# AlibabaResearch/recom

Hardware: AMD Instinct MI355X
Metric: inference QPS + p50 latency, 1000-col synth model, batch 512, 1×MI355X (higher is better)
Workload: dtype f32

## Files before the change

include/fcp_hip.h:

```cpp
#ifndef FCP_HIP_H_
#define FCP_HIP_H_

#include <stddef.h>
#include <stdint.h>

#ifdef __cplusplus
extern "C" {
#endif

#define FCP_ABI_VERSION 2

enum {
  FCP_OK = 0,
  FCP_ERR_INVALID_ARGUMENT = 1,
  FCP_ERR_SHAPE_MISMATCH = 2,
  FCP_ERR_ALLOC = 3,
  FCP_ERR_HIP = 4,
  FCP_ERR_UNSUPPORTED = 5,
  FCP_ERR_NO_DEVICE = 6
};

enum {
  FCP_FORM_GATHER = 1,
  FCP_FORM_SEGMENT_REDUCE = 2,
// ... 138 lines not shown
                            int64_t *blob_bytes, int32_t *rank_sum);
int fcp_concat_inputs(const fcp_host_tensor_t *inputs, int32_t n_inputs,
                      void *blob, int64_t blob_capacity, int32_t *offsets,
                      int32_t *shapes);

int fcp_plan_create(const fcp_plan_desc_t *desc, fcp_plan_t **plan);

#define FCP_SEG_MAP_MAX 4
typedef struct fcp_column_ext {
  int32_t seg_map_n;
  int32_t seg_map_sym;
  int32_t seg_map_sym_slot;
  int32_t weights_input1;
  int64_t seg_map_mul[FCP_SEG_MAP_MAX];
  int64_t seg_map_div;
  int32_t table_kind1;
  int32_t reserved0;
  int64_t reserved1[1];
} fcp_column_ext_t;
int fcp_plan_create_ex(const fcp_plan_desc_t *desc, const fcp_column_ext_t *ext, fcp_plan_t **plan);
int fcp_plan_create_from_file(const char *path, int32_t device, uint32_t flags,
                              fcp_plan_t **plan);
int fcp_plan_destroy(fcp_plan_t *plan);
int fcp_plan_counts(const fcp_plan_t *plan, int32_t *n_columns, int32_t *n_groups,
                    int32_t *n_host_inputs, int32_t *n_device_inputs,
                    int32_t *n_symbols);
int fcp_plan_output_columns(const fcp_plan_t *plan, int32_t *n, int32_t *indices,
                            int32_t capacity);
int fcp_plan_out_dtype(const fcp_plan_t *plan, int32_t *out);
int fcp_plan_table_dtype(const fcp_plan_t *plan, int32_t *out);
int fcp_plan_table_kinds(const fcp_plan_t *plan, int32_t *kinds, int32_t capacity, int32_t *n);
int fcp_plan_table_bytes(const fcp_plan_t *plan, int64_t *shard_bytes,
                         int64_t *max_table_bytes_unsharded);

int64_t fcp_table_row_bytes(int32_t kind, int32_t dim);
int fcp_table_convert(void *dst, int32_t dst_kind, int64_t dst_row0, const void *src, int32_t src_kind, int64_t rows,
                      int32_t dim, int32_t device, void *stream);
int fcp_table_update_rows(void *table, int32_t kind, int64_t table_rows, int32_t dim, const int64_t *row_ids, const float *rows,
                          int64_t n, int64_t *skipped, int32_t device, void *stream);
int fcp_table_read_rows(float *rows, const void *table, int32_t kind, int64_t table_rows, int32_t dim, const int64_t *row_ids,
                        int64_t n, int32_t device, void *stream);
typedef struct fcp_table_delta_report {
  int64_t n;
  int64_t distinct;
  int64_t duplicates;
  int64_t skipped;
} fcp_table_delta_report_t;
int64_t fcp_table_delta_workspace_bytes(int64_t n);
int fcp_table_delta_distinct(const void *row_ids, int32_t id_bytes, const float *rows, int32_t dim, int64_t n, int64_t table_rows,
                             int64_t *ids_out, float *rows_out, int64_t *pos_out, fcp_table_delta_report_t *report, void *workspace,
                             int32_t device, void *stream);
typedef struct fcp_table_audit_kind {
  int64_t rows_bad;
  int64_t first_bad_row;
  double sum_sq_err;
  float max_abs_err;
  int32_t reserved;
} fcp_table_audit_kind_t;
typedef struct fcp_table_audit {
  int64_t rows, rows_nonfinite, first_nonfinite_row;
  double sum_sq;
  fcp_table_audit_kind_t kind[4];
} fcp_table_audit_t;
int64_t fcp_table_audit_workspace_bytes(void);
int fcp_table_audit(const float *src, int64_t rows, int32_t dim, fcp_table_audit_t *out, void *workspace, int32_t device,
                    void *stream);
int fcp_table_audit_weighted(const float *src, int64_t rows, int32_t dim, const uint32_t *row_counts, fcp_table_audit_t *out,
                             void *workspace, int32_t device, void *stream);
int fcp_table_count_ids(uint32_t *counts, int64_t table_rows, const void *ids, int32_t id_bytes, int64_t n, int64_t *skipped,
                        int32_t device, void *stream);
int fcp_plan_table_rows(const fcp_plan_t *plan, int64_t *rows, int32_t capacity, int32_t *n);
int fcp_plan_traffic_bind(fcp_plan_t *plan, uint32_t *const *counts, int32_t n_counts, int64_t *skipped);
int fcp_plan_traffic_count(fcp_plan_t *plan, const fcp_process_args_t *args);
int fcp_table_formats_choose(const fcp_table_audit_t *audits, const int64_t *rows, const int32_t *dims, int32_t n_tables,
                             int64_t budget_bytes, uint32_t allowed_kinds, const double *table_weight, int32_t *kinds_out,
                             int64_t *bytes_out, double *error_out);
typedef struct fcp_table_digest {
  uint64_t sum;
  int64_t rows;
  int64_t skipped;
  int64_t reserved;
} fcp_table_digest_t;
int64_t fcp_table_digest_workspace_bytes(void);
int fcp_table_digest(const void *first_row, int32_t kind, int64_t rows, int32_t dim, int64_t row0, int64_t row_step,
                     fcp_table_digest_t *out, void *workspace, int32_t device, void *stream);
int fcp_table_digest_rows(const void *table, int32_t kind, int64_t table_rows, int32_t dim, int64_t row0, int64_t row_step,
                          const int64_t *row_ids, int64_t n, fcp_table_digest_t *out, void *workspace, int32_t device, void *stream);
uint64_t fcp_table_digest_host(const void *first_row, int32_t kind, int64_t rows, int32_t dim, int64_t row0, int64_t row_step);
typedef struct fcp_output_error {
  int64_t elems;
  int64_t differ;
  int64_t nonfinite;
  int64_t first_differ_row;
  double sum_sq_ref;
  double sum_sq_err;
  float max_abs_err;
  float max_abs_ref;
  int64_t reserved;
} fcp_output_error_t;
int64_t fcp_outputs_compare_workspace_bytes(int32_t n_columns);
int fcp_outputs_compare(const void *const *ptrs_a, const int64_t *row_strides_a, int32_t out_kind_a, const void *const *ptrs_b,
                        const int64_t *row_strides_b, int32_t out_kind_b,
                        const int32_t *shapes , int32_t n_columns,
                        fcp_output_error_t *out , void *workspace, int32_t device, void *stream);
enum {
  FCP_PLACE_REPLICATE = 0,
  FCP_PLACE_COLUMN_SHARD = 1,
  FCP_PLACE_ROW_SHARD = 2,
  FCP_PLACE_MIXED = 3
};
typedef struct fcp_placement {
  int32_t mode;
  int32_t min_world;
  int64_t bytes_per_gpu;
} fcp_placement_t;
int fcp_placement_decide(const int64_t *table_bytes, int32_t n_tables,
                         int64_t hbm_bytes, int64_t reserve_bytes, int32_t world,
                         int32_t prefer_mode, fcp_placement_t *out);
int fcp_placement_assign(const int64_t *table_bytes, int32_t n_tables,
                         int64_t hbm_bytes, int64_t reserve_bytes, int32_t world,
                         int32_t prefer_mode, int32_t *owner, fcp_placement_t *out);

int fcp_plan_group_width(const fcp_plan_t *plan, int32_t group, int32_t *width);
int fcp_plan_column_offset(const fcp_plan_t *plan, int32_t column,
                           int32_t *offset);
int fcp_plan_arena_bytes(fcp_plan_t *plan, const int32_t *concated_shapes,
                         const int32_t *symbols, int64_t *bytes);
int fcp_plan_read_bad_ids(fcp_plan_t *plan, void *stream, int64_t *count);

enum {
  FCP_LAUNCH_NONE = 0, FCP_LAUNCH_DENSE = 1, FCP_LAUNCH_RAGGED = 2, FCP_LAUNCH_HYBRID = 3,
  FCP_LAUNCH_RAGGED_WEIGHTED = 4,
  FCP_LAUNCH_DENSE_NARROW = 5, FCP_LAUNCH_RAGGED_NARROW = 6, FCP_LAUNCH_HYBRID_NARROW = 7,
  FCP_LAUNCH_DENSE_TAB16 = 8, FCP_LAUNCH_RAGGED_TAB16 = 9, FCP_LAUNCH_HYBRID_TAB16 = 10,
  FCP_LAUNCH_DENSE_TABQ8 = 11, FCP_LAUNCH_RAGGED_TABQ8 = 12, FCP_LAUNCH_HYBRID_TABQ8 = 13,
  FCP_LAUNCH_DENSE_TABMIX = 14, FCP_LAUNCH_RAGGED_TABMIX = 15, FCP_LAUNCH_HYBRID_TABMIX = 16
};
enum { FCP_LAUNCH_STORE_NT = 0, FCP_LAUNCH_STORE_SC1_NT = 1, FCP_LAUNCH_STORE_PLAIN = 4 };
enum { FCP_LAUNCH_SEG_NONE = 0, FCP_LAUNCH_SEG_PREPASS = 1, FCP_LAUNCH_SEG_SEARCH = 2 };
typedef struct fcp_launch_info {
  int32_t kernel;
  int32_t vec;
  int32_t rows_per_wave;
  int32_t store_policy;
  int32_t wide_rows;
  int32_t shard_world;
  int32_t dense_blocks;
  int32_t ragged_blocks;
  int32_t segment_offsets;
} fcp_launch_info_t;
int fcp_plan_last_launch(const fcp_plan_t *plan, fcp_launch_info_t *out);
enum { FCP_DENSE_FRONT_NONE = 0, FCP_DENSE_FRONT_GENERIC = 1, FCP_DENSE_FRONT_PLAIN = 2 };
int fcp_plan_last_dense_front(const fcp_plan_t *plan, int32_t *front);
int fcp_plan_last_csr(const fcp_plan_t *plan, int64_t *csr_arena_off, int32_t *csr_base, int32_t capacity);
enum {
  FCP_AUX_SEGMENT_OFFSETS = 0,
  FCP_AUX_SHARD_FINALIZE_V4 = 1, FCP_AUX_SHARD_FINALIZE_V2 = 2, FCP_AUX_SHARD_FINALIZE_V1 = 3,
  FCP_AUX_CONCAT_V4 = 4, FCP_AUX_CONCAT_V2 = 5, FCP_AUX_CONCAT_V1 = 6,
  FCP_AUX_UPLOAD = 7,
  FCP_AUX_H2D_COPY = 8,
  FCP_AUX_KERNELS = 9
};
int fcp_aux_launch_counts(int64_t *counts, int32_t capacity, int32_t reset);

int fcp_plan_release_captures(fcp_plan_t *plan);
int fcp_process_feature_columns(fcp_plan_t *plan,
                                const fcp_process_args_t *args,
                                fcp_process_result_t *result);

enum { FCP_PRIVATE_NO_CALLER_WAIT = 1u << 0, FCP_PRIVATE_ALWAYS = 1u << 1, FCP_PRIVATE_NO_VERIFY = 1u << 2 };
 int fcp_plan_set_private_streams(fcp_plan_t *plan, int32_t n_streams, uint32_t flags);

 int fcp_plan_probe_private_streams(fcp_plan_t *plan, void *stream, int32_t requests, int32_t spin_us, int32_t grid_blocks,
                                   double *serial_us, double *lanes_us);
 int fcp_plan_private_streams_verdict(fcp_plan_t *plan, void *stream, int32_t *verdict);
 int fcp_plan_verify_private_streams(fcp_plan_t *plan, void *stream, int32_t budget_ms, int32_t *verdict);
typedef struct fcp_private_streams_stats {
  void *supervised_stream;
  int64_t requests;
  int64_t lane_requests;
  int64_t evaluations;
  double stream_order_us_per_mib;
  double last_ratio;
  double worst_ratio;
  double keep_ratio;
  int32_t demoted;
  int32_t evaluation_in_progress;
} fcp_private_streams_stats_t;
 int fcp_plan_private_streams_stats(fcp_plan_t *plan, fcp_private_streams_stats_t *out);

enum { FCP_ORDER_STREAM = 0, FCP_ORDER_INPUTS_READY = 1 };
 int fcp_plan_set_request_order(fcp_plan_t *plan, int32_t order);
 int fcp_result_wait(const void *buffer, void *stream);
 int fcp_result_synchronize(const void *buffer);

int fcp_concat_outputs(const void *const *inputs, const int32_t *dims,
                       int32_t n, int64_t prefix_size, void *out, void *stream);

int fcp_concat_outputs_scatter(const void *const *inputs, const int32_t *dims,
                               const int32_t *col_offsets, int32_t n,
                               int64_t prefix_size, int32_t out_width, void *out,
                               void *stream);
int fcp_concat_outputs_scatter_strided(const void *const *inputs, const int32_t *dims,
                                       const int32_t *in_strides, const int32_t *col_offsets,
                                       int32_t n, int64_t prefix_size, int32_t out_width,
                                       void *out, void *stream);
int fcp_concat_outputs_host(const void *const *host_inputs, const int32_t *dims,
                            const int32_t *col_offsets, int32_t n,
                            int64_t prefix_size, int32_t out_width, void *out,
                            fcp_alloc_fn malloc_temp, void *malloc_temp_ctx,
                            int32_t device, void *stream);

typedef struct fcp_stager fcp_stager_t;
enum { FCP_STAGER_DEFAULT = 0, FCP_STAGER_ZERO_COPY = 1, FCP_STAGER_COPY_KERNEL = 2, FCP_STAGER_COPY_SDMA = 4 };
int fcp_stager_create(int32_t device, int64_t capacity_bytes, int32_t max_inputs,
                      int32_t max_rank_sum, int32_t depth, int32_t n_threads,
                      fcp_stager_t **stager);
int fcp_stager_create_ex(int32_t device, int64_t capacity_bytes, int32_t max_inputs,
                         int32_t max_rank_sum, int32_t depth, int32_t n_threads,
                         uint32_t flags, fcp_stager_t **stager);
int fcp_stager_stage(fcp_stager_t *stager, const fcp_host_tensor_t *inputs,
                     int32_t n_inputs, void *stream, const void **device_blob,
                     int64_t *blob_bytes, const int32_t **offsets,
                     const int32_t **shapes);
int fcp_stager_stage_narrow(fcp_stager_t *stager, const fcp_host_tensor_t *inputs,
                            int32_t n_inputs, const uint8_t *narrow_int64, void *stream,
                            const void **device_blob, int64_t *blob_bytes,
                            const int32_t **offsets, const int32_t **shapes);
enum { FCP_STAGE_COPY = 0, FCP_STAGE_NARROW_I64 = 1, FCP_STAGE_SEG_TO_CSR = 2 };
int fcp_stager_stage_ex(fcp_stager_t *stager, const fcp_host_tensor_t *inputs, int32_t n_inputs,
                        const uint8_t *modes, const int64_t *mode_args, void *stream,
                        const void **device_blob, int64_t *blob_bytes, const int32_t **offsets,
                        const int32_t **shapes);
int fcp_stager_destroy(fcp_stager_t *stager);
typedef struct fcp_stager_stats {
  int64_t calls, copy_calls, copy_calls_over_1ms, fallback_switches, requests_with_blocked_copy;
  double max_copy_call_us;
} fcp_stager_stats_t;
int fcp_stager_stats(fcp_stager_t *stager, fcp_stager_stats_t *out);

int fcp_concat_inputs_ex_sizes(const fcp_host_tensor_t *inputs, int32_t n_inputs,
                               const uint8_t *modes, const int64_t *mode_args,
                               int64_t *blob_bytes, int32_t *rank_sum);
int fcp_concat_inputs_ex(const fcp_host_tensor_t *inputs, int32_t n_inputs,
                         const uint8_t *modes, const int64_t *mode_args, void *blob,
                         int64_t blob_capacity, int32_t *offsets, int32_t *shapes);
typedef struct fcp_pack_pool fcp_pack_pool_t;
int fcp_pack_pool_create(int32_t n_threads, fcp_pack_pool_t **pool);
int fcp_pack_pool_destroy(fcp_pack_pool_t *pool);
int fcp_concat_inputs_ex_pool(fcp_pack_pool_t *pool ,
                              const fcp_host_tensor_t *inputs, int32_t n_inputs,
                              const uint8_t *modes, const int64_t *mode_args,
                              void *blob, int64_t blob_capacity, int32_t *offsets, int32_t *shapes);
int fcp_plan_file_stage_info(const char *path, int32_t *n_inputs, uint8_t *modes,
                             int32_t *rows_symbol, int32_t capacity, int32_t *symbols_input);

enum {
  FCP_GRAPH_HOST_CONCAT_EXTERNAL = 1u << 0,
  FCP_GRAPH_STAGED = 1u << 1,
  FCP_GRAPH_NO_PRUNE = 1u << 2
};
int fcp_graph_build(const void *graphdef, size_t n_bytes, uint32_t flags, const char *plan_path,
                    void **rewritten, size_t *rewritten_bytes, char **description);
void fcp_graph_free(void *p);

#define FCP_COMM_ID_BYTES 128
#define FCP_MAX_GROUPS_ABI 16
typedef struct fcp_comm fcp_comm_t;
int fcp_comm_unique_id(uint8_t *id );
int fcp_comm_create(const uint8_t *id, int32_t rank, int32_t world, int32_t device,
                    fcp_comm_t **comm);
int fcp_comm_destroy(fcp_comm_t *comm);
int fcp_comm_rank(const fcp_comm_t *comm, int32_t *rank, int32_t *world);
int fcp_shard_batch_slice(int64_t rows, int32_t world, int32_t rank, int64_t *begin,
                          int64_t *count);
int fcp_shard_exchange(fcp_comm_t *comm, const void *partial, int64_t rows,
                       int64_t width, void *slices, int64_t *row_begin,
                       int64_t *row_count, void *stream);
int fcp_shard_exchange_columns(fcp_comm_t *comm, const void *block, int64_t rows,
                               const int32_t *widths, void *recv, int64_t *row_begin,
                               int64_t *row_count, void *stream);
typedef struct fcp_shard_step fcp_shard_step_t;
int fcp_shard_step_create(fcp_plan_t *plan, fcp_comm_t *comm, int32_t mode,
                          int32_t group, int64_t max_rows, int64_t max_arena_bytes,
                          const int32_t *col_widths, fcp_shard_step_t **step);
int fcp_shard_step_run(fcp_shard_step_t *step, const fcp_process_args_t *args,
                       void **out, int64_t *row_begin, int64_t *row_count);
int fcp_shard_step_destroy(fcp_shard_step_t *step);

int fcp_shard_finalize(fcp_plan_t *plan, const fcp_process_args_t *args,
                       int32_t group, const void *partial_slices,
                       int32_t world, int64_t row_begin, int64_t row_count,
                       void *out, void *stream);

#ifdef __cplusplus
}
#endif
#endif
```

recom_amd/csrc/fcp_fused_bodies.h:

```cpp
#pragma once
#include <hip/hip_runtime.h>
#include <stdint.h>
#include <stdlib.h>

#include <type_traits>

#include "../../include/fcp_hip.h"
#include <hip/hip_ext.h>
#include "fcp_internal.h"

namespace {

#define FCP_GLOBAL __attribute__((address_space(1)))
template <typename T> __device__ __forceinline__ const FCP_GLOBAL T *as_global(const T *p) {
  return (const FCP_GLOBAL T *)(p);
}
template <typename T> __device__ __forceinline__ FCP_GLOBAL T *as_global(T *p) { return (FCP_GLOBAL T *)(p); }
#define FCP_CONST __attribute__((address_space(4)))
template <typename T> __device__ __forceinline__ const FCP_CONST T *as_const(const T *p) { return (const FCP_CONST T *)(p); }

template <int V> struct VecType;
template <> struct VecType<4> { typedef float __attribute__((ext_vector_type(4))) T; };
template <> struct VecType<2> { typedef float __attribute__((ext_vector_type(2))) T; };
template <> struct VecType<1> { typedef float T; };
// ... 755 lines not shown
    const int64_t below = lo > 0 ? seg_at(seg, is64, stride, lo - 1) : INT64_MIN;
    const int64_t above = hi < n ? seg_at(seg, is64, stride, hi) : INT64_MAX;
    int wa = lo, wz = hi;
    seg_narrow(seg, is64, stride, target, wa, wz);
    if (below < (int64_t)target && above >= (int64_t)target) {
      a = wa;
      z = wz;
    }
  }
  while (z > a) seg_narrow(seg, is64, stride, target, a, z);
  return a;
}

__device__ __forceinline__ void wave_lds_order() {
  __builtin_amdgcn_fence(__ATOMIC_RELEASE, "wavefront");
  __builtin_amdgcn_wave_barrier();
  __builtin_amdgcn_fence(__ATOMIC_ACQUIRE, "wavefront");
}

template <int V> __device__ __forceinline__ VF<V> ld_slot_or_zero(const float *tb, const float *zeros, uint32_t off, uint32_t spr) {
  typedef typename VecType<V>::T T;
  const FCP_GLOBAL T *g = is_row(off) ? as_global(reinterpret_cast<const T *>(tb)) + (uint64_t)off * spr : as_global(reinterpret_cast<const T *>(zeros));
  const T t = *g;
  VF<V> r;
  __builtin_memcpy(&r, &t, sizeof(T));
  return r;
}

template <int V>
__device__ __forceinline__ VF<V> ld_slot_or_zero16(const char *tb, const float *zeros, uint32_t off, uint32_t spr, int tab_kind) {
  typedef typename NarrowType<V>::T T;
  const FCP_GLOBAL T *g = is_row(off) ? as_global(reinterpret_cast<const T *>(tb)) + (uint64_t)off * spr : as_global(reinterpret_cast<const T *>(zeros));
  return widen16<V>(*g, tab_kind);
}

template <int V>
__device__ __forceinline__ Q8Raw ld_slot_or_zero_q8(const char *tb, const float *zeros, int tail, uint32_t off, uint32_t row_bytes) {
  const char *in_table = tb + (uint64_t)off * row_bytes, *in_zeros = reinterpret_cast<const char *>(zeros);
  const char *codes = is_row(off) ? in_table : in_zeros;
  return ld_q8_raw<V>(codes, codes + tail);
}

template <int V, int N, FcpVariant X = FCP_VAR_F32>
__device__ __forceinline__ void bag_walk_batch(const float *tb, const float *zeros, uint32_t spr, const uint32_t *s, int base, int n, VF<V> &acc,
                                               int tab_kind = 0, int q8_tail = 0) {
  constexpr bool TAB16 = X == FCP_VAR_TAB16, TABQ8 = X == FCP_VAR_TABQ8;
  uint32_t off[N];
#pragma unroll
  for (int k = 0; k < N; ++k) off[k] = base + k < n ? s[base + k] : kNoRow;
  if constexpr (TABQ8) {
    Q8Raw raw[N];
#pragma unroll
    for (int k = 0; k < N; ++k) raw[k] = ld_slot_or_zero_q8<V>(reinterpret_cast<const char *>(tb), zeros, q8_tail, off[k], spr);
#pragma unroll
    for (int k = 0; k < N; ++k)
#pragma unroll
      for (int t = 0; t < V; ++t) acc.v[t] = acc.v[t] + dequant_q8(raw[k], t);
    return;
  }
  VF<V> w[N];
#pragma unroll
  for (int k = 0; k < N; ++k) {
    if constexpr (TAB16)
      w[k] = ld_slot_or_zero16<V>(reinterpret_cast<const char *>(tb), zeros, off[k], spr, tab_kind);
    else
      w[k] = ld_slot_or_zero<V>(tb, zeros, off[k], spr);
  }
#pragma unroll
  for (int k = 0; k < N; ++k)
#pragma unroll
    for (int t = 0; t < V; ++t) acc.v[t] = acc.v[t] + w[k].v[t];
}

template <int V, int WALK, FcpVariant X = FCP_VAR_F32>
__device__ __forceinline__ void bag_walk_sum(const float *tb, const float *zeros, uint32_t spr, const uint32_t *s, int n, VF<V> &acc,
                                             int tab_kind = 0, int q8_tail = 0) {
  int base = WALK;
  if (WALK >= 8 && !__any(n > 4)) {
    bag_walk_batch<V, 4, X>(tb, zeros, spr, s, 0, n, acc, tab_kind, q8_tail);
    return;
  } else if (WALK >= 8 && kWalkFirst > WALK && __any(n > WALK)) {
    bag_walk_batch<V, kWalkFirst, X>(tb, zeros, spr, s, 0, n, acc, tab_kind, q8_tail);
    base = kWalkFirst;
  } else {
    bag_walk_batch<V, WALK, X>(tb, zeros, spr, s, 0, n, acc, tab_kind, q8_tail);
  }
  for (; __any(n > base);) {
    if (WALK > 4 && !__any(n > base + 4)) {
      bag_walk_batch<V, 4, X>(tb, zeros, spr, s, base, n, acc, tab_kind, q8_tail);
      base += 4;
    } else {
      bag_walk_batch<V, WALK, X>(tb, zeros, spr, s, base, n, acc, tab_kind, q8_tail);
      base += WALK;
    }
  }
}

__device__ __forceinline__ float weight_den_step(float den, float w, bool squares) {
#pragma clang fp contract(off)
  const float term = squares ? w * w : w;
  return den + term;
}

template <int V>
__device__ __forceinline__ void bag_walk_weighted(const float *tb, const float *zeros, uint32_t spr, const uint32_t *s, int n,
                                                  const float *w, bool want_den, bool squares, VF<V> &acc, float &den) {
#pragma clang fp contract(off)
  constexpr int N = 4;
  const FCP_GLOBAL float *gw = as_global(w);
#pragma unroll 1
  for (int base = 0; base < n; base += N) {
    uint32_t off[N];
    float wt[N];
    VF<V> x[N];
#pragma unroll
    for (int k = 0; k < N; ++k) off[k] = base + k < n ? s[base + k] : kNoRow;
#pragma unroll
    for (int k = 0; k < N; ++k) wt[k] = gw[min(base + k, n - 1)];
#pragma unroll
    for (int k = 0; k < N; ++k) x[k] = ld_slot_or_zero<V>(tb, zeros, off[k], spr);
#pragma unroll
    for (int k = 0; k < N; ++k) {
      const bool counts = off[k] <= kBadRow;
#pragma unroll
      for (int t = 0; t < V; ++t) {
        const float prod = wt[k] * x[k].v[t];
        const float sum = acc.v[t] + prod;
        acc.v[t] = counts ? sum : acc.v[t];
      }
      if (want_den && counts) den = weight_den_step(den, wt[k], squares);
    }
  }
}

__device__ __forceinline__ int wave_inclusive_sum(int x) {
  x += __builtin_amdgcn_update_dpp(0, x, 0x111, 0xf, 0xf, true);
  x += __builtin_amdgcn_update_dpp(0, x, 0x112, 0xf, 0xf, true);
  x += __builtin_amdgcn_update_dpp(0, x, 0x114, 0xf, 0xf, true);
  x += __builtin_amdgcn_update_dpp(0, x, 0x118, 0xf, 0xf, true);
  x += __builtin_amdgcn_update_dpp(0, x, 0x142, 0xa, 0xf, false);
  x += __builtin_amdgcn_update_dpp(0, x, 0x143, 0xc, 0xf, false);
  return x;
}

struct RaggedLds {
  static constexpr int RB = FCP_WAVES_PER_BLOCK;
  static constexpr int CAPW = 384;
  LdsCol col[FCP_WAVE];
  uint32_t ids[RB][CAPW];
  uint8_t owner[RB][CAPW];
  int32_t bound[FCP_WAVE * (FCP_WAVES_PER_BLOCK + 1)];
};

template <int V, bool SHARDED, FcpVariant X = FCP_VAR_F32>
__device__ __forceinline__ void ragged_body(const FcpLaunch &L, int bid, char *smem, const int64_t *wts = nullptr, int kind = 0) {
  constexpr bool WEIGHTED = X == FCP_VAR_WEIGHTED, NARROW = X == FCP_VAR_NARROW, TAB16 = X == FCP_VAR_TAB16, TABQ8 = X == FCP_VAR_TABQ8,
                 TABMIX = X == FCP_VAR_TABMIX;
  const int out_kind = kind, tab_kind = kind;
  constexpr int RB = RaggedLds::RB, CAPW = RaggedLds::CAPW;
  RaggedLds &S = *reinterpret_cast<RaggedLds *>(smem);
  LdsCol *s_col = S.col;

  BlockPos B;
  __builtin_amdgcn_s_setprio(3);
  const Hot H = load_hot(L);
  if (!locate_block<RB>(L, H, bid, B)) return;
  const int tid = threadIdx.x;
  const int lane = tid & (FCP_WAVE - 1);
  const int wave = tid >> 6;
  const int q = B.q0 + lane;
  const uint32_t my_col = B.map[min(q, B.nslots - 1)];
  const int world = H.world, rank = H.rank;

  int pre0 = 0, pre1 = 0;
  const int csr_reg_stride = H.g0.csr_reg_stride;
  if (csr_reg_stride && lane < B.ncols && B.row_blk + wave < B.rows) {
    const FCP_GLOBAL int32_t *cr = as_global(L.csr_reg) + (int64_t)(B.first_col + lane) * csr_reg_stride + (B.row_blk + wave);
    pre0 = cr[0];
    pre1 = cr[1];
  }
  if (tid < B.ncols) stage_col(H, &s_col[tid], H.cols + B.first_col + tid, H.dyn + B.first_col + tid);
  __syncthreads();

  if (H.seg_search) {
    for (int u = tid; u < B.ncols * (RB + 1); u += FCP_BLOCK_THREADS) {
      const LdsCol &c = s_col[u / (RB + 1)];
      const unsigned sk = FCP_F_SEGKIND(c.flags), f = FCP_F_FORM(c.flags);
      int v = 0;
      if ((sk == FCP_SEG_IDS_I32 || sk == FCP_SEG_IDS_I64) && (f == FCP_FORM_SEGMENT_REDUCE || f == FCP_FORM_GATHER_SCATTER))
        v = seg_lower_bound(reinterpret_cast<const char *>(c.csr), sk == FCP_SEG_IDS_I64, c.seg_stride, c.nnz,
                            min(B.row_blk + u % (RB + 1), B.rows), B.rows);
      S.bound[u] = v;
    }
    __syncthreads();
  }
  const int b = B.row_blk + wave;
  if (b >= B.rows) return;

  int lo = 0, cnt = 0;
  if (lane < B.ncols) {
    const unsigned form = FCP_F_FORM(s_col[lane].flags);
    if (form == FCP_FORM_GATHER) {
      lo = b;
      cnt = 1;
    } else if (form == FCP_FORM_SEGMENT_REDUCE || form == FCP_FORM_GATHER_SCATTER) {
      const int nnz = s_col[lane].nnz;
      int o0, o1;
      const unsigned sk = FCP_F_SEGKIND(s_col[lane].flags);
      if (form == FCP_FORM_GATHER_SCATTER && sk != FCP_SEG_CSR_I32) {
        const int t = as_global(s_col[lane].csr)[b];
        o0 = t - 1;
        o1 = t > 0 ? t : -1;
      } else if (H.seg_search && sk != FCP_SEG_CSR_I32) {
        o0 = S.bound[lane * (RB + 1) + wave];
        o1 = S.bound[lane * (RB + 1) + wave + 1];
      } else if (csr_reg_stride) {
        o0 = pre0;
        o1 = pre1;
      } else {
        const FCP_GLOBAL int32_t *csr = as_global(s_col[lane].csr);
        o0 = csr[b];
        o1 = csr[b + 1];
      }
      lo = min(max(o0, 0), nnz);
      const int hi = min(max(o1, lo), nnz);
      cnt = hi - lo;
      if (form == FCP_FORM_GATHER_SCATTER && cnt > 1 && (s_col[lane].xform & 3u) != FCP_XFORM_FILTER) {
        lo = hi - 1;
        cnt = 1;
      }
    }
  }

  const int j = (int)(my_col - B.first_col);
  const bool live = q < B.nslots;
  VF<V> acc = vzero<V>();
  int dropped = 0;

  uint8_t *ow = S.owner[wave];
  uint32_t *wi = S.ids[wave];
  const int want = min(cnt, CAPW);
  const int incl = wave_inclusive_sum(want);
  const int offx = incl - want;
  const int take = max(min(want, CAPW - offx), 0);
  const int limit = min(__shfl(incl, FCP_WAVE - 1), CAPW);
  if (take <= 16)
    for (int i = 0; i < take; ++i) ow[offx + i] = (uint8_t)lane;
  for (unsigned long long big = __ballot(take > 16); big; big &= big - 1) {
    const int p = __ffsll((long long)big) - 1;
    const int po = __shfl(offx, p), pt = __shfl(take, p);
    for (int i = lane; i < pt; i += FCP_WAVE) ow[po + i] = (uint8_t)p;
  }
  wave_lds_order();

  for (int base = 0; base < limit; base += FCP_WAVE) {
    const int k = base + lane;
    const int p = k < limit ? (int)ow[k] : 0;
    const int px = __shfl(offx, p), pl = __shfl(lo, p);
    if (k < limit) {
      bool bad;
      wi[k] = fetch_slot_offset<V, SHARDED>(s_col[p], L.xforms + B.first_col + p, pl + (k - px), nullptr, rank, world, bad);
      if (bad && H.bad_ids && s_col[p].out_off >= B.q0 * V && FCP_F_FORM(s_col[p].flags) != FCP_FORM_GATHER_SCATTER)
        atomicAdd(H.bad_ids, 1ull);
    }
  }
  wave_lds_order();

  __builtin_amdgcn_s_setprio(0);
  const float *wbase = nullptr;
  float den = 0.0f;
  if constexpr (WEIGHTED) {
    if (wts) {
      const int64_t wo = as_global(wts)[B.first_col + j];
      if (wo >= 0) wbase = reinterpret_cast<const float *>(H.blob + wo);
    }
  }
  auto consume = [&](auto walk_width, const uint32_t *s, int n, int wpos) __attribute__((always_inline)) {
    constexpr int WALK = decltype(walk_width)::value;
    const unsigned form = FCP_F_FORM(s_col[j].flags);
    const float *tb = s_col[j].table + (q * V - s_col[j].out_off);
    if constexpr (TAB16)
      tb = reinterpret_cast<const float *>(reinterpret_cast<const char *>(s_col[j].table) + 2 * (int64_t)(q * V - s_col[j].out_off));
    uint32_t spr = (uint32_t)(s_col[j].dim / V);
    int q8_tail = 0;
    if constexpr (TABQ8) {
      const int e = q * V - s_col[j].out_off;
      tb = reinterpret_cast<const float *>(reinterpret_cast<const char *>(s_col[j].table) + e);
      q8_tail = s_col[j].dim - e;
      spr = (uint32_t)s_col[j].dim + 8u;
    }
    int kind = 0;
    if constexpr (TABMIX) {
      kind = (int)FCP_F_TABKIND(s_col[j].flags);
      const int e = q * V - s_col[j].out_off;
      if (kind == FCP_TAB_Q8) {
        tb = reinterpret_cast<const float *>(reinterpret_cast<const char *>(s_col[j].table) + e);
        q8_tail = s_col[j].dim - e;
        spr = (uint32_t)s_col[j].dim + 8u;
      } else if (kind != FCP_TAB_F32) {
        tb = reinterpret_cast<const float *>(reinterpret_cast<const char *>(s_col[j].table) + 2 * (int64_t)e);
      }
    }
    if (form == FCP_FORM_SEGMENT_REDUCE) {
      if ((s_col[j].xform & 3u) == FCP_XFORM_FILTER && (FCP_F_COMBINER(s_col[j].flags) == FCP_COMBINER_MEAN ||
                                                        (WEIGHTED && FCP_F_COMBINER(s_col[j].flags) == FCP_COMBINER_SQRTN))) {
#pragma unroll 1
        for (int k = 0; k < n; ++k) dropped += s[k] == kFiltered;
      }
      if constexpr (WEIGHTED) {
        if (wbase) {
          const unsigned comb = FCP_F_COMBINER(s_col[j].flags);
          bag_walk_weighted<V>(tb, H.zeros, spr, s, n, wbase + wpos, !SHARDED && comb != FCP_COMBINER_SUM, comb == FCP_COMBINER_SQRTN,
                               acc, den);
        } else {
          bag_walk_sum<V, (WALK < kWalkLong ? WALK : kWalkLong)>(tb, H.zeros, spr, s, n, acc);
        }
      } else if constexpr (TABMIX) {
        auto walk = [&](int k) __attribute__((always_inline)) {
          if (k == FCP_TAB_F32)
            bag_walk_sum<V, WALK>(tb, H.zeros, spr, s, n, acc);
          else if (k == FCP_TAB_Q8)
            bag_walk_sum<V, WALK, FCP_VAR_TABQ8>(tb, H.zeros, spr, s, n, acc, 0, q8_tail);
          else
            bag_walk_sum<V, WALK, FCP_VAR_TAB16>(tb, H.zeros, spr, s, n, acc, k);
        };
        const int k0 = __builtin_amdgcn_readfirstlane(kind);
        if (__ballot(kind != k0) == 0ull)
          walk(k0);
        else
          walk(kind);
      } else if constexpr (TABQ8) {
        bag_walk_sum<V, WALK, FCP_VAR_TABQ8>(tb, H.zeros, spr, s, n, acc, 0, q8_tail);
      } else if constexpr (TAB16) {
        bag_walk_sum<V, WALK, FCP_VAR_TAB16>(tb, H.zeros, spr, s, n, acc, tab_kind);
      } else {
        bag_walk_sum<V, WALK>(tb, H.zeros, spr, s, n, acc);
      }
    } else if (form == FCP_FORM_GATHER || form == FCP_FORM_GATHER_SCATTER) {
      int k = n - 1;
      while (k > 0 && s[k] == kFiltered) --k;
      const uint32_t off = s[k];
      if (off != kFiltered) {
        acc = vzero<V>();
        if constexpr (TABMIX) {
          if (is_row(off)) {
            if (kind == FCP_TAB_F32)
              acc = ld_slot<V>(tb, off, spr);
            else if (kind == FCP_TAB_Q8)
              acc = ld_slot_q8<V>(reinterpret_cast<const char *>(tb), q8_tail, off, spr);
            else
              acc = ld_slot16<V>(reinterpret_cast<const char *>(tb), off, spr, kind);
          }
        } else if constexpr (TABQ8) {
          if (is_row(off)) acc = ld_slot_q8<V>(reinterpret_cast<const char *>(tb), q8_tail, off, spr);
        } else if constexpr (TAB16) {
          if (is_row(off)) acc = ld_slot16<V>(reinterpret_cast<const char *>(tb), off, spr, tab_kind);
        } else {
          if (is_row(off)) acc = ld_slot<V>(tb, off, spr);
        }
        if (form == FCP_FORM_GATHER_SCATTER && off == kBadRow && H.bad_ids && q * V == s_col[j].out_off) atomicAdd(H.bad_ids, 1ull);
      }
    }
  };
  {
    const int ptake = __shfl(take, j), poff = __shfl(offx, j);
    int wpos = 0;
    if constexpr (WEIGHTED) wpos = __shfl(lo, j);
    if (live && ptake > 0) consume(std::integral_constant<int, kWalk>(), wi + poff, ptake, wpos);
  }

  for (int done = take;;) {
    const int rem = cnt - done;
    const unsigned long long act = __ballot(rem > 0);
    if (!act) break;
    const int nact = __popcll(act);
    const int sh_log2 = 31 - __clz(CAPW / nact);
    const int share = 1 << sh_log2;
    const int my_rank = __popcll(act & ((1ull << lane) - 1ull));
    const int tk = rem > 0 ? min(rem, share) : 0;
    wave_lds_order();
    if (rem > 0) ow[my_rank] = (uint8_t)lane;
    wave_lds_order();
    const int limit = nact << sh_log2;
    const int from = lo + done;
    for (int base = 0; base < limit; base += FCP_WAVE) {
      const int k = base + lane;
      const int p = k < limit ? (int)ow[k >> sh_log2] : 0;
      const int i = k & (share - 1);
      const int ptk = __shfl(tk, p), pf = __shfl(from, p);
      if (k < limit && i < ptk) {
        bool bad;
        wi[k] = fetch_slot_offset<V, SHARDED>(s_col[p], L.xforms + B.first_col + p, pf + i, nullptr, rank, world, bad);
        if (bad && H.bad_ids && s_col[p].out_off >= B.q0 * V && FCP_F_FORM(s_col[p].flags) != FCP_FORM_GATHER_SCATTER)
          atomicAdd(H.bad_ids, 1ull);
      }
    }
    wave_lds_order();
    const int ptake = __shfl(tk, j), prank = __shfl(my_rank, j);
    int wpos = 0;
    if constexpr (WEIGHTED) wpos = __shfl(from, j);
    if (live && ptake > 0) consume(std::integral_constant<int, kWalkLong>(), wi + (prank << sh_log2), ptake, wpos);
    done += tk;
  }
  const int pcnt = __shfl(cnt, j);
  const LdsCol &C = s_col[j];
  const unsigned form = FCP_F_FORM(C.flags);
  if (!live || form == FCP_FORM_EXTERNAL) return;

  const int dim = C.dim;
  const int e = q * V - C.out_off;
  if (form == FCP_FORM_PASSTHROUGH) {
    if (rank == 0) acc = ld_blob_f32<V>(C.ids + 4 * ((int64_t)b * dim + e));
  } else if (form == FCP_FORM_BATCH_COL_REDUCTION) {
    const int inner = rank == 0 ? C.inner : 0;
    for (int rr = 0; rr < inner; ++rr) {
      const VF<V> x = ld_blob_f32<V>(C.ids + 4 * (((int64_t)b * inner + rr) * dim + e));
#pragma unroll
      for (int t = 0; t < V; ++t) acc.v[t] = acc.v[t] + x.v[t];
    }
  } else if (WEIGHTED && form == FCP_FORM_SEGMENT_REDUCE && !SHARDED && FCP_F_COMBINER(C.flags) != FCP_COMBINER_SUM) {
    float d = wbase ? den : (float)(pcnt - dropped);
    if (FCP_F_COMBINER(C.flags) == FCP_COMBINER_SQRTN) d = sqrtf(d);
    if (d == 0.0f) {
      acc = vzero<V>();
    } else {
#pragma unroll
      for (int t = 0; t < V; ++t) acc.v[t] = acc.v[t] / d;
    }
  } else if (!WEIGHTED && form == FCP_FORM_SEGMENT_REDUCE && !SHARDED && FCP_F_COMBINER(C.flags) == FCP_COMBINER_MEAN && pcnt > dropped) {
    const float fc = (float)(pcnt - dropped);
#pragma unroll
    for (int t = 0; t < V; ++t) acc.v[t] = acc.v[t] / fc;
  }
  if constexpr (NARROW) {
    st_out_narrow<V>(H.arena + C.out_base + 2 * (e + (int64_t)b * C.out_stride), acc, H.store_through, out_kind);
    return;
  }
  st_out<V>(reinterpret_cast<float *>(H.arena + C.out_base) + e + (int64_t)b * C.out_stride, acc, H.store_through);
}

}
```

recom_amd/csrc/fcp_host.h:

```cpp
#pragma once
#include <hip/hip_runtime.h>
#include <hip/hip_ext.h>

#include <algorithm>
#include <atomic>
#include <chrono>
#include <cmath>
#include <cstdio>
#include <cstdlib>
#include <cstring>
#include <functional>
#include <map>
#include <memory>
#include <mutex>
#include <new>
#include <string>
#include <thread>
#include <vector>

#include "../../include/fcp_hip.h"
#include "fcp_internal.h"
#include "fcp_env.h"
#include "fcp_formats.h"
#include "fcp_plan_desc.h"

namespace fcph {

int hip_fail(const char *what, hipError_t e);

#define HIP_TRY(expr)                                   \
  do {                                                  \
    hipError_t e_ = (expr);                             \
    if (e_ != hipSuccess) return hip_fail(#expr, e_);   \
  } while (0)

inline int64_t align128(int64_t x) { return (x + 127) / 128 * 128; }

constexpr int kSlots = 32;
constexpr uint32_t kFlagHostOnly = FCP_FLAG_HOST_ONLY;

struct HostColumn {
  fcp_column_desc_t d;
  fcp_column_ext_t ext = {};
  std::vector<float> boundaries;
  int32_t weights_input = -1;
  std::vector<int64_t> xf_lo, xf_hi;
  int64_t xf_const_off = -1;
  int32_t out_off = 0;
  int64_t const_off = -1;
};

constexpr int kAllSlotsBusy = -2;
constexpr int kNeedsInstall = -3;

struct DynMeta {
  std::vector<int32_t> group_rows;
  std::vector<int64_t> group_base;
  int64_t arena_bytes = 0;
  int64_t csr_arena_off = 0;
  int32_t max_seg_nnz = 0;
  int32_t max_lookup_nnz = 0;
  int64_t seg_pairs = 0;
  bool seg_search = false;
  bool plain = false;
  int64_t work_bytes = 0;
  int32_t csr_reg_mode = 0, csr_reg_stride = 0;
  int64_t csr_reg_base = 0;
  struct Geo {
    int32_t grid_blocks = 0;
    int32_t rows_per_wave = 1;
    FcpGroupLaunch groups[FCP_MAX_GROUPS];
  } geo[2];
};

struct DynSlot {
  bool valid = false;
  std::vector<int32_t> key;
  FcpColDyn *h_dyn = nullptr;
  void *h_dyn_dev = nullptr;
  FcpColDyn *d_dyn = nullptr;
  hipEvent_t uploaded = nullptr;
  uint64_t done_gen = 0;
  hipEvent_t done = nullptr;
  std::vector<std::pair<void *, hipEvent_t>> done_pool;
  bool done_valid = false;
  void *stream = nullptr;
  uint64_t tick = 0;
  int users = 0;
  int uses = 0;
  bool captured = false;
  bool img_built = false;
  bool was_valid = false;
  DynMeta meta;
};

constexpr int kLaneEvents = 8;
constexpr int kMaxPoolLanes = 16;
struct PrivateLane {
  hipStream_t stream = nullptr;
  std::mutex mu;
  hipEvent_t in[kLaneEvents] = {};
  hipEvent_t out[kLaneEvents] = {};
  uint32_t next = 0;
};

extern std::atomic<uint64_t> g_lane_generation;
extern thread_local hipEvent_t tl_lane_done;
extern thread_local uint64_t tl_lane_done_gen;

struct LaneDep {
  hipEvent_t in;
  hipStream_t caller, lane;
};
extern thread_local const LaneDep *tl_lane_dep;
extern thread_local int64_t tl_work_bytes;

constexpr int kSupWindow = 48;
struct LaneSupervisor {
  std::mutex mu;
  bool on = true;
  uint32_t period = 8192, first_gap = 256;
  double keep_ratio = 0.97;
  void *caller = nullptr;
  bool use_lanes = true;
  uint64_t seq = 0;
  uint64_t next_eval = 1, gap = 256;
  int phase = 0;
  hipEvent_t b0 = nullptr, b1 = nullptr;
  hipEvent_t w0 = nullptr, w1 = nullptr;
  PrivateLane *w_lane = nullptr;
  int so_count = 0, w_count = 0;
  int64_t so_bytes = 0, w_bytes = 0;
  int strikes = 0;
  uint64_t evaluations = 0, lane_requests = 0;
  double so_ns_per_byte = 0, last_ratio = 0, worst_ratio = 0;
  bool demoted = false;
};

struct LanePool {
  std::mutex cal_mu;
  std::vector<std::unique_ptr<PrivateLane>> lanes;
  std::vector<hipStream_t> spacers;
  std::atomic<int> n_relying{0};
  std::atomic<uint32_t> rr{0};
  std::atomic<int> fault_us{0};
  std::atomic<hipEvent_t> last_out{nullptr};
};
void sup_reset(LaneSupervisor &S, const fcp::Env &env);
LanePool *lane_pool_for(int device);

struct PendingResult {
  uintptr_t end;
  hipEvent_t done;
  const void *owner;
};
void pending_register(const void *owner, void *arena, int64_t bytes, const void *blob, int64_t blob_bytes, hipEvent_t done);
void pending_clear_range(void *arena, int64_t bytes);
void pending_forget(const void *owner);
int stager_input_wait(const void *base, int64_t bytes, hipStream_t stream);
int stager_input_synchronize(const void *base, int64_t bytes);
int wait_for_inputs(const void *const *inputs, int32_t n, void *stream);

}
using namespace fcph;

struct fcp_plan {
  fcp::Env env;
  fcp_plan_desc_t desc;
  std::vector<HostColumn> cols;
  std::vector<int32_t> ranks, elem_sizes, shape_off;
  std::vector<int32_t> group_width, group_nslots, group_map_off;
  std::vector<int32_t> seg_cols;
  int32_t n_seg_plain = 0;
  bool seg_search = false;
  bool has_inverse = false;
  bool csr_by_pos = false;
  std::vector<int32_t> order, pos_of;
  struct FastCol {
    int32_t ids_input, seg_input, rows_arg, dim, seg_stride;
    int64_t out_off_bytes;
    uint8_t form, rows_source, seg_kind, group;
  };
  std::vector<FastCol> fast_cols;
  std::vector<int32_t> group_rep;
  int vec = 1;
  bool dense_only = true;
  std::vector<uint32_t> span_list;
  std::vector<int32_t> list_off[2], list_n[2];
  uint32_t *d_span_list = nullptr;
  bool host_only = false;
  int32_t rank_sum = 0;

  uint32_t *d_slot_map = nullptr;
  FcpColStatic *d_cols = nullptr;
  FcpXform *d_xforms = nullptr;
  FcpSegMap *d_segmaps = nullptr;
  bool has_seg_map = false;
  bool has_weights = false, weighted_kernel = false;
  FcpVariant variant = FCP_VAR_F32;
  bool plain_dense = false;
  int32_t plain_stride = 0, plain_spans = 0, plain_cols_off = 0;
  std::vector<char> plain_tmpl;
  std::vector<std::pair<uint32_t, int32_t>> plain_entries;
  std::atomic<int32_t> last_dense_front{0};
  bool wide_rows = false;
  int out_kind = FCP_OUT_F32, out_elem = 4;
  int tab_kind = FCP_TAB_F32, tab_elem = 4;
  int tab_row_tail = 0;
  std::vector<int8_t> col_kind;
  bool tab_mixed() const { return !col_kind.empty(); }
  int col_tab_kind(size_t k) const { return col_kind.empty() ? tab_kind : col_kind[k]; }
  int64_t col_row_bytes(size_t k, int dim) const {
    return fcpf::row_bytes(col_tab_kind(k), dim);
  }
  std::vector<FcpColStatic> h_cols;
  char *d_const = nullptr;
  int32_t *d_seg_cols = nullptr;
  unsigned long long *d_bad = nullptr;
  float *d_zeros = nullptr;
  std::vector<const void *> bound_tables;
  bool tables_bound = false;
  FcpTrafficCol *d_traffic = nullptr;
  int32_t traffic_n = 0;
  unsigned long long *traffic_skipped = nullptr;

  bool host_writes_dyn = false;
  std::mutex mu;
  DynSlot slots[kSlots];
  uint64_t tick = 0;

  LanePool *pool = nullptr;
  uint32_t lane_flags = 0;
  std::vector<std::pair<void *, bool>> lane_verdicts;
  std::atomic<void *> lane_good_caller{nullptr};
  int32_t lane_count = 0;
  std::atomic<bool> lane_relies{false};
  std::atomic<int64_t> last_work_bytes{0};
  int64_t lane_min_work = 0;
  int32_t request_order = FCP_ORDER_STREAM;
  std::atomic<uintptr_t> recent_arena[2] = {};
  struct LastLaunch {
    std::atomic<int32_t> kernel{0}, rows_per_wave{0}, store_policy{0}, dense_blocks{0}, ragged_blocks{0}, segment_offsets{0};
    std::atomic<int64_t> csr_arena_off{-1};
    std::unique_ptr<std::atomic<int32_t>[]> csr_base;
  } last_launch;
  std::atomic<bool> lane_demoted{false};
  LaneSupervisor sup;
  std::atomic<bool> sup_window{false};
};

namespace fcph {

struct DeviceGuard {
  int prev = -1;
  bool changed = false;
  int enter(int dev) {
    hipError_t e = hipGetDevice(&prev);
    if (e != hipSuccess) return hip_fail("hipGetDevice", e);
    if (prev != dev) {
      e = hipSetDevice(dev);
      if (e != hipSuccess) return hip_fail("hipSetDevice", e);
      changed = true;
    }
    return FCP_OK;
  }
  ~DeviceGuard() {
    if (changed) (void)hipSetDevice(prev);
  }
};

template <class F> int on_device(const char *who, int32_t device, void *stream, F enqueue) {
  DeviceGuard guard;
  const int rc = guard.enter(device);
  if (rc) return rc;
  enqueue(static_cast<hipStream_t>(stream));
  const hipError_t e = hipGetLastError();
  return e == hipSuccess ? FCP_OK : hip_fail((std::string(who) + ": kernel launch").c_str(), e);
}

int compute_dyn(const fcp_plan *p, const int32_t *offsets, const int32_t *shapes, const int32_t *symbols, int64_t blob_bytes,
                FcpColDyn *dyn, DynMeta *m);
int compute_weights(const fcp_plan *p, const int32_t *offsets, const int32_t *shapes, int64_t *wts);
inline size_t slot_dyn_bytes(const fcp_plan *p) {
  return p->cols.size() * sizeof(FcpColDyn) + (p->has_weights ? p->cols.size() * sizeof(int64_t) : 0) +
         (p->plain_dense ? p->plain_tmpl.size() : 0);
}
inline size_t slot_image_off(const fcp_plan *p) { return p->cols.size() * sizeof(FcpColDyn); }
inline const int64_t *slot_weights(const fcp_plan *p, const FcpColDyn *dyn) {
  return p->has_weights ? reinterpret_cast<const int64_t *>(dyn + p->cols.size()) : nullptr;
}
void build_plain_template(fcp_plan *p);
bool stream_is_capturing(hipStream_t stream);
int bind_tables(fcp_plan *p, const void *const *input_ptrs, bool capturing);
void build_key(const fcp_plan *p, const fcp_process_args_t *a, std::vector<int32_t> &key);
int find_or_reserve(fcp_plan *p, const std::vector<int32_t> &key, DynSlot **out, bool *install, bool capturing);
int install_slot(fcp_plan *p, const fcp_process_args_t *a, DynSlot &s);
void publish_slot(fcp_plan *p, DynSlot &s, const std::vector<int32_t> &key, void *stream);
void fill_launch(const fcp_plan *p, const DynSlot &s, int kind, const void *blob, void *arena, int store_policy, FcpLaunch *L);
void destroy_lanes(LanePool *pool);
int create_lanes(LanePool *pool, int n, int prio);
int process_on_private_streams(fcp_plan_t *p, const fcp_process_args_t *a, fcp_process_result_t *r);

struct SlotUnpin {
  fcp_plan *p;
  DynSlot *s;
  bool recorded;
  ~SlotUnpin() {
    std::lock_guard<std::mutex> lock(p->mu);
    if (recorded) s->done_valid = s->uses == 1;
    --s->users;
  }
};

}

extern "C" int fcp_internal_process(fcp_plan_t *p, const fcp_process_args_t *a, fcp_process_result_t *r);
```

recom_amd/csrc/fcp_internal.h:

```cpp
#pragma once
#include <stddef.h>
#include <stdint.h>

#ifndef FCP_MAX_GROUPS
#define FCP_MAX_GROUPS 16
#endif
#define FCP_BLOCK_THREADS 256
#define FCP_WAVES_PER_BLOCK 4
#define FCP_WAVE 64

#define FCP_F_FORM(f) ((f) & 0xFu)
#define FCP_F_COMBINER(f) (((f) >> 4) & 0xFu)
#define FCP_F_IDSRC(f) (((f) >> 8) & 0xFu)
#define FCP_F_SEGKIND(f) (((f) >> 12) & 0xFu)
#define FCP_F_TABKIND(f) (((f) >> 16) & 0x3u)
#define FCP_F_PACK(form, comb, idsrc, segkind) \
  ((uint32_t)(form) | ((uint32_t)(comb) << 4) | ((uint32_t)(idsrc) << 8) | ((uint32_t)(segkind) << 12))

struct FcpColStatic {
  const float *table;
  const float *boundaries;
  int64_t vocab;
  int32_t dim;
  int32_t out_off;
  uint32_t flags;
  int32_t n_boundaries;
  int32_t seg_stride;
  float bnd_b0, bnd_inv, bnd_step;
  uint32_t xform;
  int32_t bnd_off;
};

struct FcpXform {
  int64_t lo0, hi0;
  int64_t sub;
  const int64_t *extra;
  int64_t hash_buckets;
  int64_t pad_;
};
#define FCP_XFORM_HASH_BIT 0x80000000u

struct FcpColDyn {
  int64_t ids_off;
  int64_t seg_off;
  int64_t out_base;
  int32_t out_stride;
  int32_t nnz;
  int32_t csr_base;
  int32_t inner;
  int32_t rows;
  int32_t seg_sym;
};

struct FcpSegMap {
  int64_t mul[4];
  int64_t div;
  int32_t n;
  int32_t sym_slot;
};

struct FcpGroupLaunch {
  int32_t rows;
  int32_t nslots;
  int32_t nsp8;
  int32_t block_begin;
  int32_t slot_map_off;
  int32_t span_list_off;
  int32_t nlist;
  int32_t csr_reg_stride;
};

struct FcpLaunch {
  const uint32_t *slot_map;
  const uint32_t *span_list;
  const FcpColStatic *cols;
  const FcpColDyn *dyn;
  const char *blob;
  char *arena;
  unsigned long long *bad_ids;
  int64_t csr_arena_off;
  int32_t n_groups;
  int32_t rows_per_wave;
  int32_t shard_rank, shard_world;
  int32_t seg_search;
  int32_t store_through;
  const int32_t *csr_reg;
  FcpGroupLaunch groups[FCP_MAX_GROUPS];
  const FcpXform *xforms;
  const float *zeros;
};

struct FcpPlainCol {
  const float *table;
  int64_t ids_off;
  uint32_t vocab;
  uint32_t spr;
  int32_t out_off;
  uint32_t kind;
  int32_t n_boundaries;
  float bnd_b0, bnd_inv, bnd_step;
};
constexpr uint32_t FCP_PLAIN_FACT_NONE = 0, FCP_PLAIN_FACT_I32 = 1, FCP_PLAIN_FACT_I64 = 2, FCP_PLAIN_FACT_F32 = 3;
constexpr int FCP_PLAIN_FACTS_OFF = 80;
constexpr int FCP_PLAIN_FACTS_PER_PASS = 16;
constexpr int fcp_plain_facts_bytes(int max_cols) {
  return (max_cols + FCP_PLAIN_FACTS_PER_PASS - 1) / FCP_PLAIN_FACTS_PER_PASS * FCP_PLAIN_FACTS_PER_PASS * 4;
}
struct FcpPlainSpan {
  int32_t ncols;
  int32_t cols_off;
  int32_t pad_[2];
  uint8_t lane_col[FCP_WAVE];
};
struct FcpPlainLaunch {
  const char *img;
  const char *blob;
  float *out;
  unsigned long long *bad_ids;
  int32_t rows, nslots, nsp8, nlist;
  int32_t img_stride;
  int32_t out_stride;
  int32_t store_policy;
};

struct FcpSegLaunch {
  const int32_t *seg_cols;
  const FcpColStatic *cols;
  const FcpColDyn *dyn;
  const char *blob;
  char *arena;
  int64_t csr_arena_off;
  unsigned long long *bad_ids;
  const FcpXform *xforms;
  const FcpSegMap *segmaps;
  int32_t skip_inverse;
};

struct FcpTrafficCol {
  uint32_t *counts;
  int32_t pos;
  int32_t pad_;
};
struct FcpTrafficLaunch {
  const FcpTrafficCol *list;
  const FcpColStatic *cols;
  const FcpColDyn *dyn;
  const FcpXform *xforms;
  const char *blob;
  unsigned long long *skipped;
};
struct ihipStream_t;
int fcp_launch_plan_traffic(const FcpTrafficLaunch &T, int n_list, int max_nnz, ihipStream_t *s);

enum FcpVariant {
  FCP_VAR_F32 = 0,
  FCP_VAR_WEIGHTED,
  FCP_VAR_NARROW,
  FCP_VAR_TAB16,
  FCP_VAR_TABQ8,
  FCP_VAR_TABMIX,
  FCP_VARIANTS
};

struct ihipStream_t;
void fcp_set_stop_event(void *event);
bool fcp_stop_event_pending();
void fcp_set_any_order(bool on);
struct FcpFusedWork {
  const FcpLaunch *dense;
  int dense_blocks;
  const FcpLaunch *ragged;
  int ragged_blocks;
  int vec;
  int kind;
  const int64_t *wts;
};
typedef int FcpFusedLauncher(const FcpFusedWork &W, ihipStream_t *s);
FcpFusedLauncher fcp_launch_f32, fcp_launch_weighted, fcp_launch_narrow, fcp_launch_tab16, fcp_launch_tabq8, fcp_launch_tabmix;
int fcp_launch_dense_plain(const FcpPlainLaunch &P, int grid_blocks, ihipStream_t *s);
void fcp_take_launch_extras(void **stop_event, int *flags);
int fcp_launch_upload(const void *host_mapped_src, void *dst, size_t bytes, ihipStream_t *s);
int fcp_launch_h2d_copy(const void *host_mapped_src, void *dst, size_t bytes, ihipStream_t *s);
int fcp_launch_segment_offsets(const FcpSegLaunch &L, int n_seg_cols, int max_nnz, ihipStream_t *s, bool any_order = false);
int fcp_launch_concat_outputs(const void *const *inputs, const int32_t *dims, const int32_t *col_offsets, const int32_t *in_strides,
                              int32_t n, int64_t prefix, int32_t width, int32_t first_off, void *out,
                              ihipStream_t *s);
int fcp_launch_shard_finalize(const FcpLaunch &L, int group, const float *partials, int world,
                              int64_t row_begin, int64_t row_count, float *out, int vec,
                              ihipStream_t *s, const int64_t *wts = nullptr);
```

recom_amd/csrc/fcp_plan.hip:

```cpp
#include "fcp_host.h"

namespace fcph {

int hip_fail(const char *what, hipError_t e) {
  return fail((e == hipErrorNoDevice || e == hipErrorInvalidDevice || e == hipErrorNoBinaryForGpu || e == hipErrorInsufficientDriver)
                  ? FCP_ERR_NO_DEVICE
                  : FCP_ERR_HIP,
              std::string(what) + ": " + hipGetErrorString(e));
}

int finish_geometry(const fcp_plan *p, DynMeta *m);
void find_regular_csr(const fcp_plan *p, const FcpColDyn *dyn, DynMeta *m);

int compute_dyn_slow(const fcp_plan *p, const int32_t *offsets, const int32_t *shapes,
                     const int32_t *symbols, int64_t blob_bytes, FcpColDyn *dyn, DynMeta *m) {
  const int nc = (int)p->cols.size();
  const int ng = p->desc.n_groups;
  const int nh = (int)p->ranks.size();
  thread_local std::vector<int64_t> numel_v, col_rows;
  numel_v.resize(nh);
  col_rows.resize(nc);
  for (int i = 0; i < nh; ++i) {
    int64_t n = 1;
    const int32_t *d = shapes + p->shape_off[i];
// ... 283 lines not shown
  m->csr_arena_off = cursor;
  int64_t csr_cursor = 0;
  if (p->csr_by_pos) {
    const int64_t stride = ((int64_t)m->group_rows[0] + 1 + 31) / 32 * 32;
    for (int k : p->seg_cols) dyn[p->pos_of[k]].csr_base = (int32_t)(p->pos_of[k] * stride);
    csr_cursor = stride * nc;
    if (csr_cursor > 0x7fffffff) return -1;
  } else {
    for (int k : p->seg_cols) {
      FcpColDyn &d = dyn[p->pos_of[k]];
      d.csr_base = (int32_t)csr_cursor;
      csr_cursor += ((int64_t)d.rows + 1 + 31) / 32 * 32;
      if (csr_cursor > 0x7fffffff) return -1;
    }
  }
  m->arena_bytes = cursor + csr_cursor * 4;
  find_regular_csr(p, dyn, m);
  return finish_geometry(p, m);
}

int compute_weights(const fcp_plan *p, const int32_t *offsets, const int32_t *shapes, int64_t *wts) {
  auto numel = [&](int i) {
    int64_t n = 1;
    for (int j = 0; j < p->ranks[i]; ++j) n *= shapes[p->shape_off[i] + j];
    return n;
  };
  for (size_t pos = 0; pos < p->cols.size(); ++pos) {
    const HostColumn &hc = p->cols[p->order[pos]];
    wts[pos] = -1;
    if (hc.weights_input < 0) continue;
    if (numel(hc.weights_input) != numel(hc.d.ids_input))
      return fail(FCP_ERR_SHAPE_MISMATCH, "column " + std::to_string(p->order[pos]) + ": the weights tensor does not hold one weight per id");
    if (offsets[hc.weights_input] % 4) return fail(FCP_ERR_UNSUPPORTED, "blob tensor not 4-byte aligned");
    wts[pos] = offsets[hc.weights_input];
  }
  return FCP_OK;
}

int compute_dyn(const fcp_plan *p, const int32_t *offsets, const int32_t *shapes, const int32_t *symbols,
                int64_t blob_bytes, FcpColDyn *dyn, DynMeta *m) {
  const bool slow_only = fcp::diag_on("dyn_general");
  if (!slow_only && !p->fast_cols.empty()) {
    const int rc = compute_dyn_fast(p, offsets, shapes, symbols, blob_bytes, dyn, m);
    if (rc >= 0) return rc;
  }
  const int rc = compute_dyn_slow(p, offsets, shapes, symbols, blob_bytes, dyn, m);
  if (rc == FCP_OK) {
    int64_t gathered = 0;
    for (size_t i = 0; i < p->cols.size(); ++i) gathered += (int64_t)dyn[i].nnz * p->cols[p->order[i]].d.dim;
    m->work_bytes = gathered * 4 + m->csr_arena_off;
  }
  return rc;
}

void uniform_boundaries(const std::vector<float> &b, float *b0, float *inv, float *step_out) {
  const int n = (int)b.size();
  if (n < 2 || !(b[n - 1] > b[0])) return;
  const float lo = b[0];
  const float scale = (float)((double)(n - 1) / ((double)b[n - 1] - (double)b[0]));
  if (!(scale > 0.0f) || !std::isfinite(scale)) return;
  auto guess = [&](float x) {
    float t = (x - lo) * scale;
    t = std::fmin(std::fmax(t, -1.0f), (float)n);
    int g = (int)std::floor(t) + 1;
    return std::min(std::max(g, 0), n);
  };
  auto exact = [&](float x) { return (int)(std::upper_bound(b.begin(), b.end(), x) - b.begin()); };
  int misses = 0;
  for (int i = 0; i < n; ++i) {
    if (i && !(b[i] > b[i - 1])) return;
    const float below = std::nextafter(b[i], -INFINITY);
    misses += guess(b[i]) != exact(b[i]);
    misses += guess(below) != exact(below);
  }
  if (misses * 8 > n) return;
  *b0 = lo;
  *inv = scale;
  const float step = b[1] - b[0];
  if (!(step > 0.0f) || !std::isfinite(step)) return;
  for (int i = 0; i < n; ++i)
    if (std::fmaf((float)i, step, lo) != b[i]) return;
  *step_out = step;
}

void build_plain_template(fcp_plan *p) {
  p->plain_dense = false;
  if (fcp::diag_ll("dense_generic", 0) != 0) return;
  const fcp_plan_desc_t &d = p->desc;
  if (p->out_elem != 4 || p->tab_elem != 4 || d.layout != FCP_LAYOUT_CONCAT || d.n_groups != 1 || d.shard_world > 1 || p->vec != 4 || p->wide_rows ||
      p->weighted_kernel || !p->dense_only || p->cols.empty())
    return;
  const int nc = (int)p->cols.size();
  for (int pos = 0; pos < nc; ++pos) {
    const HostColumn &hc = p->cols[p->order[pos]];
    const FcpColStatic &s = p->h_cols[pos];
    if (hc.d.form != FCP_FORM_GATHER || s.xform != 0 || hc.d.vocab < 0 || hc.d.vocab >= 0xFFFFFFFDLL) return;
    if (hc.d.id_source == FCP_IDS_F32_BUCKETIZE) {
      if (s.bnd_step == 0.0f) return;
    } else if (hc.d.id_source != FCP_IDS_I32 && hc.d.id_source != FCP_IDS_I64) {
      return;
    }
  }
  const int nslots = p->group_nslots[0];
  const int nspans = (nslots + FCP_WAVE - 1) / FCP_WAVE;
  if (p->list_n[0][0] != nspans) return;
  std::vector<int> first(nspans, nc), last(nspans, -1);
  for (int pos = 0; pos < nc; ++pos) {
    const FcpColStatic &s = p->h_cols[pos];
    const int s0 = s.out_off / 4 / FCP_WAVE, s1 = (s.out_off + s.dim - 1) / 4 / FCP_WAVE;
    for (int sp = s0; sp <= s1; ++sp) {
      first[sp] = std::min(first[sp], pos);
      last[sp] = std::max(last[sp], pos);
    }
  }
  int max_cols = 1;
  for (int sp = 0; sp < nspans; ++sp) max_cols = std::max(max_cols, last[sp] - first[sp] + 1);
  if (max_cols > FCP_WAVE) return;
  p->plain_cols_off = FCP_PLAIN_FACTS_OFF + fcp_plain_facts_bytes(max_cols);
  p->plain_stride = (int32_t)(p->plain_cols_off + (size_t)max_cols * sizeof(FcpPlainCol));
  p->plain_spans = nspans;
  p->plain_tmpl.assign((size_t)nspans * p->plain_stride, 0);
  p->plain_entries.clear();
  for (int sp = 0; sp < nspans; ++sp) {
    char *rec = p->plain_tmpl.data() + (size_t)sp * p->plain_stride;
    FcpPlainSpan head;
    std::memset(&head, 0, sizeof(head));
    head.ncols = last[sp] - first[sp] + 1;
    head.cols_off = p->plain_cols_off;
    for (int pos = first[sp]; pos <= last[sp]; ++pos) {
      const FcpColStatic &s = p->h_cols[pos];
      FcpPlainCol c;
      std::memset(&c, 0, sizeof(c));
      c.table = nullptr;
      c.ids_off = 0;
      c.vocab = (uint32_t)s.vocab;
      c.spr = (uint32_t)(s.dim / 4);
      c.out_off = s.out_off;
      c.kind = FCP_F_IDSRC(s.flags);
      c.n_boundaries = s.n_boundaries;
      c.bnd_b0 = s.bnd_b0;
      c.bnd_inv = s.bnd_inv;
      c.bnd_step = s.bnd_step;
      const size_t at = (size_t)sp * p->plain_stride + p->plain_cols_off + (size_t)(pos - first[sp]) * sizeof(FcpPlainCol);
      std::memcpy(p->plain_tmpl.data() + at, &c, sizeof(c));
      p->plain_entries.emplace_back((uint32_t)at, pos);
      for (int q = std::max(s.out_off / 4, sp * FCP_WAVE); q < std::min((s.out_off + s.dim) / 4, (sp + 1) * FCP_WAVE); ++q)
        head.lane_col[q - sp * FCP_WAVE] = (uint8_t)(pos - first[sp]);
    }
    std::memcpy(rec, &head, sizeof(head));
  }
  p->plain_dense = true;
}

void destroy_device(fcp_plan *p) {
  if (p->host_only) return;
  for (auto &s : p->slots) {
    if (s.h_dyn) (void)hipHostFree(s.h_dyn);
    if (s.d_dyn) (void)hipFree(s.d_dyn);
    if (s.uploaded) (void)hipEventDestroy(s.uploaded);
    for (auto &e : s.done_pool) (void)hipEventDestroy(e.second);
  }
  if (p->d_slot_map) (void)hipFree(p->d_slot_map);
  if (p->d_span_list) (void)hipFree(p->d_span_list);
  if (p->d_cols) (void)hipFree(p->d_cols);
  if (p->d_xforms) (void)hipFree(p->d_xforms);
  if (p->d_segmaps) (void)hipFree(p->d_segmaps);
  if (p->d_const) (void)hipFree(p->d_const);
  if (p->d_seg_cols) (void)hipFree(p->d_seg_cols);
  if (p->d_bad) (void)hipFree(p->d_bad);
  if (p->d_zeros) (void)hipFree(p->d_zeros);
  if (p->d_traffic) (void)hipFree(p->d_traffic);
}

int init_device(fcp_plan *p) {
  DeviceGuard guard;
  int rc = guard.enter(p->desc.device);
  if (rc) return rc;
  const int nc = (int)p->cols.size();
  std::vector<uint32_t> map;
  for (int g = 0; g < p->desc.n_groups; ++g) {
    p->group_map_off[g] = (int32_t)map.size();
    for (int pos = 0; pos < nc; ++pos) {
      const HostColumn &hc = p->cols[p->order[pos]];
      if (hc.d.concat_group != g) continue;
      for (int s = 0; s < hc.d.dim / p->vec; ++s) map.push_back((uint32_t)pos);
    }
  }
  HIP_TRY(hipMalloc(&p->d_span_list, std::max<size_t>(p->span_list.size(), 1) * sizeof(uint32_t)));
  HIP_TRY(hipMemcpy(p->d_span_list, p->span_list.data(), p->span_list.size() * sizeof(uint32_t), hipMemcpyHostToDevice));
  HIP_TRY(hipMalloc(&p->d_slot_map, std::max<size_t>(map.size(), 1) * sizeof(uint32_t)));
  HIP_TRY(hipMemcpy(p->d_slot_map, map.data(), map.size() * sizeof(uint32_t), hipMemcpyHostToDevice));
  int64_t const_bytes = 0;
  std::vector<int> owners;
  for (size_t k = 0; k < p->cols.size(); ++k) {
    HostColumn &hc = p->cols[k];
    if (hc.boundaries.empty()) continue;
    for (int o : owners)
      if (p->cols[o].boundaries == hc.boundaries) {
        hc.const_off = p->cols[o].const_off;
        break;
      }
    if (hc.const_off < 0) {
      hc.const_off = const_bytes;
      const_bytes += align128((int64_t)hc.boundaries.size() * 4);
      owners.push_back((int)k);
    }
  }
  for (HostColumn &hc : p->cols) {
    if (hc.xf_lo.size() <= 1) continue;
    hc.xf_const_off = const_bytes;
    const_bytes += align128((int64_t)(hc.xf_lo.size() - 1) * 16);
  }
  if (const_bytes) {
    HIP_TRY(hipMalloc(&p->d_const, const_bytes));
    for (const HostColumn &hc : p->cols) {
      if (hc.xf_const_off < 0) continue;
      std::vector<int64_t> pairs;
      for (size_t i = 1; i < hc.xf_lo.size(); ++i) {
        pairs.push_back(hc.xf_lo[i]);
        pairs.push_back(hc.xf_hi[i]);
      }
      HIP_TRY(hipMemcpy(p->d_const + hc.xf_const_off, pairs.data(), pairs.size() * 8, hipMemcpyHostToDevice));
    }
    for (int o : owners)
      HIP_TRY(hipMemcpy(p->d_const + p->cols[o].const_off, p->cols[o].boundaries.data(),
                        p->cols[o].boundaries.size() * 4, hipMemcpyHostToDevice));
  }
  std::vector<FcpXform> h_xforms;
  p->h_cols.resize(nc);
  for (int pos = 0; pos < nc; ++pos) {
    const HostColumn &hc = p->cols[p->order[pos]];
    FcpColStatic &s = p->h_cols[pos];
    s.table = nullptr;
    s.boundaries = hc.const_off >= 0 ? reinterpret_cast<const float *>(p->d_const + hc.const_off) : nullptr;
    s.vocab = hc.d.vocab;
    s.dim = hc.d.dim;
    s.out_off = hc.out_off;
    s.flags = FCP_F_PACK(hc.d.form, hc.d.combiner, hc.d.id_source, hc.d.seg_kind);
    if (p->tab_mixed()) s.flags |= (uint32_t)p->col_kind[p->order[pos]] << 16;
    s.n_boundaries = (int32_t)hc.boundaries.size();
    s.seg_stride = hc.d.seg_stride < 1 ? 1 : hc.d.seg_stride;
    s.bnd_b0 = 0.0f;
    s.bnd_inv = 0.0f;
    s.bnd_step = 0.0f;
    uniform_boundaries(hc.boundaries, &s.bnd_b0, &s.bnd_inv, &s.bnd_step);
    s.bnd_off = -1;
    s.xform = 0;
    if (hc.d.xform_mode != FCP_XFORM_NONE || hc.d.hash_buckets > 0) {
      if (h_xforms.empty()) {
        FcpXform none;
        none.lo0 = 1;
        none.hi0 = 0;
        none.sub = 0;
        none.extra = nullptr;
        none.hash_buckets = 0;
        none.pad_ = 0;
        h_xforms.assign(nc, none);
      }
      FcpXform &x = h_xforms[pos];
      if (hc.d.hash_buckets > 0) {
        s.xform |= FCP_XFORM_HASH_BIT;
        x.hash_buckets = hc.d.hash_buckets;
      }
      if (hc.d.xform_mode != FCP_XFORM_NONE) {
        const uint32_t n = (uint32_t)std::max<size_t>(hc.xf_lo.size(), 1);
        s.xform |= (n << 2) | (uint32_t)hc.d.xform_mode;
        x.sub = hc.d.xform_substitute;
        if (!hc.xf_lo.empty()) {
          x.lo0 = hc.xf_lo[0];
          x.hi0 = hc.xf_hi[0];
        }
        if (hc.xf_const_off >= 0) x.extra = reinterpret_cast<const int64_t *>(p->d_const + hc.xf_const_off);
      }
    }
  }
  build_plain_template(p);
  HIP_TRY(hipMalloc(&p->d_cols, nc * sizeof(FcpColStatic)));
  HIP_TRY(hipMemcpy(p->d_cols, p->h_cols.data(), nc * sizeof(FcpColStatic), hipMemcpyHostToDevice));
  if (!h_xforms.empty()) {
    HIP_TRY(hipMalloc(&p->d_xforms, nc * sizeof(FcpXform)));
    HIP_TRY(hipMemcpy(p->d_xforms, h_xforms.data(), nc * sizeof(FcpXform), hipMemcpyHostToDevice));
  }
  if (p->has_seg_map) {
    std::vector<FcpSegMap> h_maps(nc);
    for (int pos = 0; pos < nc; ++pos) {
      const fcp_column_ext_t &e = p->cols[p->order[pos]].ext;
      FcpSegMap &sm = h_maps[pos];
      for (int i = 0; i < 4; ++i) sm.mul[i] = i < e.seg_map_n ? e.seg_map_mul[i] : 0;
      sm.div = e.seg_map_n > 0 ? e.seg_map_div : 1;
      sm.n = e.seg_map_n;
      sm.sym_slot = e.seg_map_n > 0 && e.seg_map_sym >= 0 ? e.seg_map_sym_slot : -1;
    }
    HIP_TRY(hipMalloc(&p->d_segmaps, nc * sizeof(FcpSegMap)));
    HIP_TRY(hipMemcpy(p->d_segmaps, h_maps.data(), nc * sizeof(FcpSegMap), hipMemcpyHostToDevice));
  }
  if (!p->seg_cols.empty()) {
    std::vector<int32_t> seg_pos;
    for (int k : p->seg_cols) seg_pos.push_back(p->pos_of[k]);
    HIP_TRY(hipMalloc(&p->d_seg_cols, seg_pos.size() * sizeof(int32_t)));
    HIP_TRY(hipMemcpy(p->d_seg_cols, seg_pos.data(), seg_pos.size() * sizeof(int32_t), hipMemcpyHostToDevice));
  }
  size_t zero_bytes = 256;
  for (size_t k = 0; k < p->cols.size(); ++k)
    if (fcpf::kTab[p->col_tab_kind(k)].row_tail) zero_bytes = std::max(zero_bytes, (size_t)((p->col_row_bytes(k, p->cols[k].d.dim) + 255) / 256 * 256));
  HIP_TRY(hipMalloc(&p->d_zeros, zero_bytes));
  HIP_TRY(hipMemset(p->d_zeros, 0, zero_bytes));
  if (p->desc.flags & FCP_FLAG_COUNT_BAD_IDS) {
    HIP_TRY(hipMalloc(&p->d_bad, sizeof(unsigned long long)));
    HIP_TRY(hipMemset(p->d_bad, 0, sizeof(unsigned long long)));
  }
  {
    int large_bar = 0;
    (void)hipDeviceGetAttribute(&large_bar, hipDeviceAttributeIsLargeBar, p->desc.device);
    p->host_writes_dyn = large_bar != 0 && !p->env.dyn_upload_kernel;
  }
  for (auto &s : p->slots) {
    const size_t dyn_bytes = (slot_dyn_bytes(p) + 15) / 16 * 16;
    HIP_TRY(hipHostMalloc(reinterpret_cast<void **>(&s.h_dyn), dyn_bytes, hipHostMallocMapped));
    HIP_TRY(hipHostGetDevicePointer(&s.h_dyn_dev, s.h_dyn, 0));
    if (p->host_writes_dyn) {
      if (hipExtMallocWithFlags(reinterpret_cast<void **>(&s.d_dyn), dyn_bytes, hipDeviceMallocFinegrained) != hipSuccess) {
        (void)hipGetLastError();
        p->host_writes_dyn = false;
        for (auto &t : p->slots)
          if (t.d_dyn) {
            (void)hipFree(t.d_dyn);
            t.d_dyn = nullptr;
          }
      }
    }
  }
  for (auto &s : p->slots) {
    const size_t dyn_bytes = (slot_dyn_bytes(p) + 15) / 16 * 16;
    if (!s.d_dyn) HIP_TRY(hipMalloc(&s.d_dyn, dyn_bytes));
    HIP_TRY(hipEventCreateWithFlags(&s.uploaded, hipEventDisableTiming));
    s.done = nullptr;
  }
  p->bound_tables.assign(p->desc.n_device_inputs, nullptr);
  {
    int64_t shard_bytes = 0;
    (void)fcp_plan_table_bytes(p, &shard_bytes, nullptr);
    size_t free_b = 0, total_b = 0;
    if (hipMemGetInfo(&free_b, &total_b) == hipSuccess && total_b > 0 && (uint64_t)shard_bytes > total_b)
      return fail(FCP_ERR_UNSUPPORTED, "this plan's tables need " + std::to_string(shard_bytes) + " bytes on a device with " +
                                           std::to_string(total_b) + ": shard them over more GPUs (fcp_placement_decide)");
  }
  return FCP_OK;
}

}

extern "C" {

int fcp_plan_create(const fcp_plan_desc_t *desc, fcp_plan_t **out) { return fcp_plan_create_ex(desc, nullptr, out); }

int fcp_plan_create_ex(const fcp_plan_desc_t *desc, const fcp_column_ext_t *ext, fcp_plan_t **out) {
  if (!out) return fail(FCP_ERR_INVALID_ARGUMENT, "null plan out pointer");
  *out = nullptr;
  PlanFacts facts;
  int rc = check_desc(desc, ext, &facts);
  if (rc) return rc;
  fcp_plan_desc_t canonical = *desc;
  canonical.flags = facts.flags;
  desc = &canonical;
  fcp_plan *p = new (std::nothrow) fcp_plan();
  if (!p) return fail(FCP_ERR_ALLOC, "out of host memory");
  p->out_kind = facts.out_kind;
  p->out_elem = fcpf::kOut[facts.out_kind].elem;
  p->tab_kind = facts.tab_kind;
  p->col_kind.swap(facts.col_kind);
  p->tab_elem = p->tab_mixed() ? 0 : fcpf::kTab[facts.tab_kind].elem;
  p->tab_row_tail = p->tab_mixed() ? 0 : fcpf::kTab[facts.tab_kind].row_tail;
  p->variant = facts.variant;
  p->weighted_kernel = facts.variant == FCP_VAR_WEIGHTED;
  p->env = fcp::read_env();
  p->desc = *desc;
  p->desc.columns = nullptr;
  p->desc.host_input_ranks = nullptr;
  p->desc.host_input_elem_sizes = nullptr;
  p->host_only = (desc->flags & kFlagHostOnly) != 0;
  p->ranks.assign(desc->host_input_ranks, desc->host_input_ranks + desc->n_host_inputs);
  p->elem_sizes.assign(desc->host_input_elem_sizes, desc->host_input_elem_sizes + desc->n_host_inputs);
  p->shape_off.resize(desc->n_host_inputs);
  int32_t acc = 0;
  for (int i = 0; i < desc->n_host_inputs; ++i) {
    p->shape_off[i] = acc;
    acc += p->ranks[i];
  }
  p->rank_sum = acc;
  p->cols.resize(desc->n_columns);
  int gcd4 = 4;
  for (int k = 0; k < desc->n_columns; ++k) {
    HostColumn &hc = p->cols[k];
    hc.d = desc->columns[k];
    if (hc.d.id_source == FCP_IDS_F32_BUCKETIZE && hc.d.boundaries && hc.d.n_boundaries > 0 &&
        hc.d.form != FCP_FORM_PASSTHROUGH && hc.d.form != FCP_FORM_BATCH_COL_REDUCTION && hc.d.form != FCP_FORM_EXTERNAL)
      hc.boundaries.assign(hc.d.boundaries, hc.d.boundaries + hc.d.n_boundaries);
    hc.d.boundaries = nullptr;
    if (hc.d.xform_mode != FCP_XFORM_NONE && hc.d.xform_n > 0) {
      hc.xf_lo.assign(hc.d.xform_lo, hc.d.xform_lo + hc.d.xform_n);
      hc.xf_hi.assign(hc.d.xform_hi, hc.d.xform_hi + hc.d.xform_n);
    }
    hc.d.xform_lo = hc.d.xform_hi = nullptr;
    if (ext && ext[k].seg_map_n > 0) {
      hc.ext = ext[k];
      p->has_seg_map = true;
    }
    if (ext && ext[k].weights_input1 > 0) {
      hc.weights_input = ext[k].weights_input1 - 1;
      p->has_weights = true;
    }
    if (hc.d.dim % 4) gcd4 = (hc.d.dim % 2) ? 1 : std::min(gcd4, 2);
    const int f = hc.d.form;
    if ((f == FCP_FORM_SEGMENT_REDUCE || f == FCP_FORM_GATHER_SCATTER) && hc.d.seg_kind != FCP_SEG_CSR_I32)
      p->seg_cols.push_back(k);
  }
  p->vec = gcd4;
  std::stable_partition(p->seg_cols.begin(), p->seg_cols.end(), [&](int32_t k) { return p->cols[k].d.form != FCP_FORM_GATHER_SCATTER; });
  p->n_seg_plain = 0;
  for (int32_t k : p->seg_cols) p->n_seg_plain += p->cols[k].d.form != FCP_FORM_GATHER_SCATTER;
  p->last_launch.csr_base.reset(new std::atomic<int32_t>[p->cols.size() > 0 ? p->cols.size() : 1]);
  for (size_t k = 0; k < p->cols.size(); ++k) p->last_launch.csr_base[k].store(-1, std::memory_order_relaxed);
  p->seg_search = desc->shard_world <= 1 && !p->env.seg_prepass;
  if (p->has_seg_map) p->seg_search = false;
  for (const HostColumn &hc : p->cols) {
    if (hc.d.seg_kind != FCP_SEG_NONE && hc.d.seg_stride > 0xffff) p->seg_search = false;
    if (hc.d.form == FCP_FORM_GATHER_SCATTER && hc.d.seg_kind != FCP_SEG_CSR_I32) {
      p->has_inverse = true;
      p->seg_search = false;
// ... 137 lines not shown
  *out = p->tab_kind;
  return FCP_OK;
}

int fcp_plan_table_kinds(const fcp_plan_t *p, int32_t *kinds, int32_t capacity, int32_t *n) {
  if (!p) return fail(FCP_ERR_INVALID_ARGUMENT, "null plan");
  std::vector<int32_t> in_kind(p->desc.n_device_inputs, -1);
  for (size_t k = 0; k < p->cols.size(); ++k) {
    const int f = p->cols[k].d.form;
    if (f == FCP_FORM_GATHER || f == FCP_FORM_SEGMENT_REDUCE || f == FCP_FORM_GATHER_SCATTER) in_kind[p->cols[k].d.table_input] = p->col_tab_kind(k);
  }
  for (int32_t t = 0; t < p->desc.n_device_inputs && t < capacity; ++t)
    if (kinds) kinds[t] = in_kind[t];
  if (n) *n = p->desc.n_device_inputs;
  return FCP_OK;
}

int fcp_plan_table_rows(const fcp_plan_t *p, int64_t *rows, int32_t capacity, int32_t *n) {
  if (!p) return fail(FCP_ERR_INVALID_ARGUMENT, "null plan");
  std::vector<int64_t> in_rows(p->desc.n_device_inputs, -1);
  for (size_t k = 0; k < p->cols.size(); ++k) {
    const int f = p->cols[k].d.form;
    if (f != FCP_FORM_GATHER && f != FCP_FORM_SEGMENT_REDUCE && f != FCP_FORM_GATHER_SCATTER) continue;
    int64_t &r = in_rows[p->cols[k].d.table_input];
    r = std::max(r, p->cols[k].d.vocab);
  }
  for (int32_t t = 0; t < p->desc.n_device_inputs && t < capacity; ++t)
    if (rows) rows[t] = in_rows[t];
  if (n) *n = p->desc.n_device_inputs;
  return FCP_OK;
}

int fcp_plan_table_bytes(const fcp_plan_t *p, int64_t *shard_bytes, int64_t *max_table_bytes_unsharded) {
  if (!p) return fail(FCP_ERR_INVALID_ARGUMENT, "null plan");
  std::vector<int64_t> local(p->desc.n_device_inputs, 0), whole(p->desc.n_device_inputs, 0);
  for (size_t k = 0; k < p->cols.size(); ++k) {
    const HostColumn &hc = p->cols[k];
    const int f = hc.d.form;
    if (f != FCP_FORM_GATHER && f != FCP_FORM_SEGMENT_REDUCE && f != FCP_FORM_GATHER_SCATTER) continue;
    const int64_t local_vocab =
        (hc.d.vocab - p->desc.shard_rank + p->desc.shard_world - 1) / p->desc.shard_world;
    const int64_t row_bytes = p->col_row_bytes(k, hc.d.dim);
    local[hc.d.table_input] = std::max(local[hc.d.table_input], local_vocab * row_bytes);
    whole[hc.d.table_input] = std::max(whole[hc.d.table_input], hc.d.vocab * row_bytes);
  }
  int64_t sum = 0, mx = 0;
  for (int t = 0; t < p->desc.n_device_inputs; ++t) {
    sum += local[t];
    mx = std::max(mx, whole[t]);
  }
  if (shard_bytes) *shard_bytes = sum;
  if (max_table_bytes_unsharded) *max_table_bytes_unsharded = mx;
  return FCP_OK;
}

int fcp_plan_release_captures(fcp_plan_t *p) {
  if (!p) return fail(FCP_ERR_INVALID_ARGUMENT, "null plan");
  std::lock_guard<std::mutex> lock(p->mu);
  for (auto &s : p->slots) {
    if (!s.captured) continue;
    s.captured = false;
    s.done_valid = false;
  }
  return FCP_OK;
}

int fcp_plan_destroy(fcp_plan_t *p) {
  if (!p) return FCP_OK;
  if (!p->host_only) {
    DeviceGuard guard;
    if (guard.enter(p->desc.device) == FCP_OK) {
      (void)hipDeviceSynchronize();
      pending_forget(p);
      if (p->pool && p->lane_relies.exchange(false)) p->pool->n_relying.fetch_sub(1, std::memory_order_acq_rel);
      for (hipEvent_t *ev : {&p->sup.b0, &p->sup.b1, &p->sup.w0, &p->sup.w1})
        if (*ev) {
          (void)hipEventDestroy(*ev);
          *ev = nullptr;
        }
      destroy_device(p);
    }
  }
  delete p;
  return FCP_OK;
}

int fcp_plan_group_width(const fcp_plan_t *p, int32_t group, int32_t *width) {
  if (!p || !width || group < 0 || group >= p->desc.n_groups)
    return fail(FCP_ERR_INVALID_ARGUMENT, "bad group");
  *width = p->group_width[group];
  return FCP_OK;
}

int fcp_plan_column_offset(const fcp_plan_t *p, int32_t column, int32_t *offset) {
  if (!p || !offset || column < 0 || column >= (int32_t)p->cols.size())
    return fail(FCP_ERR_INVALID_ARGUMENT, "bad column");
  *offset = p->cols[column].out_off;
  return FCP_OK;
}

int fcp_plan_arena_bytes(fcp_plan_t *p, const int32_t *concated_shapes, const int32_t *symbols,
                         int64_t *bytes) {
  if (!p || !concated_shapes || !bytes) return fail(FCP_ERR_INVALID_ARGUMENT, "null argument");
  std::vector<FcpColDyn> dyn(p->cols.size());
  std::vector<int32_t> offsets(p->ranks.size(), 0);
  DynMeta m;
  int rc = compute_dyn(p, offsets.data(), concated_shapes, symbols, -1, dyn.data(), &m);
  if (rc) return rc;
  *bytes = m.arena_bytes;
  return FCP_OK;
}

int fcp_plan_read_bad_ids(fcp_plan_t *p, void *stream, int64_t *count) {
  if (!p || !count) return fail(FCP_ERR_INVALID_ARGUMENT, "null argument");
  *count = 0;
  if (p->host_only) return fail(FCP_ERR_NO_DEVICE, "host-only plan");
  if (!p->d_bad) return FCP_OK;
  DeviceGuard guard;
  int rc = guard.enter(p->desc.device);
  if (rc) return rc;
  unsigned long long v = 0;
  HIP_TRY(hipStreamSynchronize(static_cast<hipStream_t>(stream)));
  if (p->pool && p->lane_count > 0) {
    std::lock_guard<std::mutex> cal_lock(p->pool->cal_mu);
    for (auto &l : p->pool->lanes)
      if (l->stream) HIP_TRY(hipStreamSynchronize(l->stream));
  }
  HIP_TRY(hipMemcpy(&v, p->d_bad, sizeof(v), hipMemcpyDeviceToHost));
  *count = (int64_t)v;
  return FCP_OK;
}

int fcp_plan_last_launch(const fcp_plan_t *p, fcp_launch_info_t *out) {
  if (!p || !out) return fail(FCP_ERR_INVALID_ARGUMENT, "null argument");
  const fcp_plan::LastLaunch &ll = p->last_launch;
  out->kernel = ll.kernel.load(std::memory_order_relaxed);
  out->vec = p->vec;
  out->rows_per_wave = ll.rows_per_wave.load(std::memory_order_relaxed);
  out->store_policy = ll.store_policy.load(std::memory_order_relaxed);
  out->wide_rows = p->wide_rows ? 1 : 0;
  out->shard_world = p->desc.shard_world > 1 ? p->desc.shard_world : 1;
  out->dense_blocks = ll.dense_blocks.load(std::memory_order_relaxed);
  out->ragged_blocks = ll.ragged_blocks.load(std::memory_order_relaxed);
  out->segment_offsets = ll.segment_offsets.load(std::memory_order_relaxed);
  return FCP_OK;
}

int fcp_plan_last_dense_front(const fcp_plan_t *p, int32_t *front) {
  if (!p || !front) return fail(FCP_ERR_INVALID_ARGUMENT, "null argument");
  *front = p->last_dense_front.load(std::memory_order_relaxed);
  return FCP_OK;
}

int fcp_plan_last_csr(const fcp_plan_t *p, int64_t *csr_arena_off, int32_t *csr_base, int32_t capacity) {
  if (!p || capacity < 0 || (capacity > 0 && !csr_base)) return fail(FCP_ERR_INVALID_ARGUMENT, "null plan / bad capacity");
  const fcp_plan::LastLaunch &ll = p->last_launch;
  if (csr_arena_off) *csr_arena_off = ll.csr_arena_off.load(std::memory_order_relaxed);
  for (int32_t k = 0; k < capacity && k < (int32_t)p->cols.size(); ++k)
    csr_base[k] = ll.csr_base ? ll.csr_base[k].load(std::memory_order_relaxed) : -1;
  return FCP_OK;
}

}
```

recom_amd/csrc/fcp_plan_desc.cc:

```cpp
#include "fcp_plan_desc.h"

#include <algorithm>
#include <cmath>
#include <cstdio>
#include <cstring>
#include <utility>

namespace fcph {
namespace {
thread_local std::string g_last_error;
}

int fail(int code, const std::string &msg) {
  g_last_error = msg;
  return code;
}

namespace {

int validate_desc(const fcp_plan_desc_t *d) {
  if (!d) return fail(FCP_ERR_INVALID_ARGUMENT, "null plan descriptor");
  if (d->abi_version != FCP_ABI_VERSION) return fail(FCP_ERR_INVALID_ARGUMENT, "abi_version mismatch");
  if (d->n_columns <= 0 || !d->columns) return fail(FCP_ERR_INVALID_ARGUMENT, "plan has no columns");
  if (d->n_host_inputs < 0 || (d->n_host_inputs > 0 && (!d->host_input_ranks || !d->host_input_elem_sizes)))
// ... 263 lines not shown
    fcp_column_desc_t &c = P.cols[k];
    std::memset(&c, 0, sizeof(c));
    long long vocab = 0;
    if (std::fscanf(f, "%d %d %d %d %lld %d %d %d %d %d %d %d %d %d %d", &c.form, &c.combiner, &c.dim, &c.id_source, &vocab,
                    &c.table_input, &c.ids_input, &c.seg_input, &c.seg_kind, &c.seg_stride, &c.rows_source, &c.rows_arg,
                    &c.concat_group, &c.concat_slot, &c.n_boundaries) != 15 ||
        c.n_boundaries < 0 || c.n_boundaries > (1 << 24))
      return fail(FCP_ERR_INVALID_ARGUMENT, where + "truncated or malformed column " + std::to_string(k));
    c.vocab = vocab;
    P.bnd[k].resize(c.n_boundaries);
    for (int b = 0; b < c.n_boundaries; ++b)
      if (std::fscanf(f, "%f", &P.bnd[k][b]) != 1) return fail(FCP_ERR_INVALID_ARGUMENT, where + "truncated boundary list");
    c.boundaries = c.n_boundaries ? P.bnd[k].data() : nullptr;
    if (version >= 2) {
      long long sub = 0, hb = 0;
      if (std::fscanf(f, "%d %d %lld %lld", &c.xform_mode, &c.xform_n, &sub, &hb) != 4 || c.xform_n < 0 || c.xform_n > (1 << 20))
        return fail(FCP_ERR_INVALID_ARGUMENT, where + "truncated or malformed id transform of column " + std::to_string(k));
      c.xform_substitute = sub;
      c.hash_buckets = hb;
      P.xlo[k].resize(c.xform_n);
      P.xhi[k].resize(c.xform_n);
      for (int i = 0; i < c.xform_n; ++i) {
        long long lo = 0, hi = 0;
        if (std::fscanf(f, "%lld %lld", &lo, &hi) != 2) return fail(FCP_ERR_INVALID_ARGUMENT, where + "truncated interval list");
        P.xlo[k][i] = lo;
        P.xhi[k][i] = hi;
      }
      c.xform_lo = c.xform_n ? P.xlo[k].data() : nullptr;
      c.xform_hi = c.xform_n ? P.xhi[k].data() : nullptr;
    }
  }
  bool seen_maps = false, seen_weights = false;
  for (;;) {
    int count = 0;
    const int got = std::fscanf(f, "%31s %d", tag, &count);
    if (got == EOF || got == 0) break;
    if (got != 2) return fail(FCP_ERR_INVALID_ARGUMENT, where + "malformed trailing section");
    if (version >= 5 && !std::strcmp(tag, "weights") && !seen_weights && !seen_maps && !P.has_stage) {
      if (count < 0 || count > n_cols) return fail(FCP_ERR_INVALID_ARGUMENT, where + "bad 'weights M'");
      seen_weights = true;
      if (count > 0) P.ext.assign(n_cols, fcp_column_ext_t{});
      for (int i = 0; i < count; ++i) {
        int col = -1, input = -1;
        if (std::fscanf(f, "%d %d", &col, &input) != 2 || col < 0 || col >= n_cols || input < 0 || input >= n_host ||
            P.ext[col].weights_input1 != 0)
          return fail(FCP_ERR_INVALID_ARGUMENT, where + "malformed weights entry " + std::to_string(i));
        P.ext[col].weights_input1 = input + 1;
      }
    } else if (version >= 4 && !std::strcmp(tag, "segmaps") && !seen_maps && !P.has_stage) {
      if (count < 0 || count > n_cols) return fail(FCP_ERR_INVALID_ARGUMENT, where + "bad 'segmaps M'");
      seen_maps = true;
      if (P.ext.empty()) P.ext.assign(n_cols, fcp_column_ext_t{});
      for (int i = 0; i < count; ++i) {
        int col = -1, n = 0, sym = -1, slot = 0;
        long long mul[4] = {0, 0, 0, 0}, div = 1;
        if (std::fscanf(f, "%d %d %d %d %lld %lld %lld %lld %lld", &col, &n, &sym, &slot, &mul[0], &mul[1], &mul[2], &mul[3], &div) != 9 ||
            col < 0 || col >= n_cols || n < 1 || n > FCP_SEG_MAP_MAX || P.ext[col].seg_map_n != 0)
          return fail(FCP_ERR_INVALID_ARGUMENT, where + "malformed segmaps entry " + std::to_string(i));
        fcp_column_ext_t &e = P.ext[col];
        e.seg_map_n = n;
        e.seg_map_sym = sym;
        e.seg_map_sym_slot = slot;
        for (int j = 0; j < 4; ++j) e.seg_map_mul[j] = mul[j];
        e.seg_map_div = div;
      }
    } else if (version >= 3 && !std::strcmp(tag, "stage") && !P.has_stage) {
      const int n_stage = count;
      int sym_in = -1;
      if (std::fscanf(f, "%31s %d", t2, &sym_in) != 2 || std::strcmp(t2, "symbols_input") || n_stage < 0 || n_stage > (1 << 24) ||
          sym_in < -1 || sym_in >= n_stage)
        return fail(FCP_ERR_INVALID_ARGUMENT, where + "expected 'stage N symbols_input K'");
      P.stage_modes.resize(n_stage);
      P.stage_rows_symbol.resize(n_stage);
      for (int i = 0; i < n_stage; ++i) {
        int mode = 0, sym = -1;
        if (std::fscanf(f, "%d %d", &mode, &sym) != 2 || mode < FCP_STAGE_COPY || mode > FCP_STAGE_SEG_TO_CSR || sym < -1 ||
            sym >= d.n_symbols || (mode == FCP_STAGE_SEG_TO_CSR && (sym < 0 || sym_in < 0)))
          return fail(FCP_ERR_INVALID_ARGUMENT, where + "malformed stage entry " + std::to_string(i));
        P.stage_modes[i] = (uint8_t)mode;
        P.stage_rows_symbol[i] = sym;
      }
      P.stage_symbols_input = sym_in;
      P.has_stage = true;
    } else {
      return fail(FCP_ERR_INVALID_ARGUMENT, where + "unexpected section '" + tag + "'");
    }
  }
  if (version >= 8) {
    if (P.ext.empty()) P.ext.assign(n_cols, fcp_column_ext_t{});
    std::vector<char> read(P.in_kinds.size(), 0);
    int first = -1;
    bool differ = false;
    for (int k = 0; k < n_cols; ++k) {
      const fcp_column_desc_t &c = P.cols[k];
      if (c.form != FCP_FORM_GATHER && c.form != FCP_FORM_SEGMENT_REDUCE && c.form != FCP_FORM_GATHER_SCATTER) continue;
      if (c.table_input < 0 || c.table_input >= (int)P.in_kinds.size() || P.in_kinds[c.table_input] < 0)
        return fail(FCP_ERR_INVALID_ARGUMENT, where + "column " + std::to_string(k) + " reads a table the table_dtypes line gives no dtype");
      read[c.table_input] = 1;
      const int kind = P.in_kinds[c.table_input];
      P.ext[k].table_kind1 = 1 + kind;
      differ = differ || (first >= 0 && kind != first);
      if (first < 0) first = kind;
    }
    for (size_t t = 0; t < read.size(); ++t)
      if (!read[t] && P.in_kinds[t] >= 0)
        return fail(FCP_ERR_INVALID_ARGUMENT, where + "the table_dtypes line gives device input " + std::to_string(t) + ", which no lookup column reads, a dtype");
    if (!differ) return fail(FCP_ERR_INVALID_ARGUMENT, where + "version 8 is for plans whose tables have more than one dtype; this one is a version <= 7 plan");
  }
  d.abi_version = FCP_ABI_VERSION;
  d.n_columns = n_cols;
  d.columns = P.cols.data();
  d.n_host_inputs = n_host;
  d.host_input_ranks = P.ranks.data();
  d.host_input_elem_sizes = P.esz.data();
  d.shard_rank = 0;
  d.shard_world = 1;
  return FCP_OK;
}

}

int check_desc(const fcp_plan_desc_t *desc, const fcp_column_ext_t *ext, PlanFacts *facts) {
  int rc = validate_desc(desc);
  if (rc) return rc;
  if (ext && (rc = validate_ext(desc, ext))) return rc;
  fcp_plan_desc_t d = *desc;
  facts->col_kind.clear();
  if (d.flags & FCP_FLAG_TABLES_PER_INPUT) {
    int uniform = -1;
    if ((rc = resolve_table_kinds(desc, ext, &facts->col_kind, &uniform))) return rc;
    d.flags &= ~(uint32_t)FCP_FLAG_TABLES_PER_INPUT;
    if (uniform >= 0) {
      facts->col_kind.clear();
      d.flags |= fcpf::kTab[uniform].flag;
    }
  }
  const bool mixed = !facts->col_kind.empty();
  const unsigned families = ((d.flags & fcpf::kOutFlags) ? NARROW : 0) | (mixed ? MIXED : 0) | ((d.flags & FCP_FLAG_TABLES_Q8) ? Q8 : 0) | ((d.flags & kTab16Flags) ? TAB16 : 0);
  if ((rc = run_refusals(d, ext, families))) return rc;
  facts->flags = d.flags;
  facts->out_kind = fcpf::out_kind_of_flags(d.flags);
  facts->tab_kind = mixed ? FCP_TAB_MIXED : fcpf::tab_kind_of_flags(d.flags);
  bool weighted = false;
  for (int k = 0; k < d.n_columns; ++k) weighted = weighted || (ext && ext[k].weights_input1 > 0) || d.columns[k].combiner == FCP_COMBINER_SQRTN;
  facts->variant = weighted                           ? FCP_VAR_WEIGHTED
                   : facts->out_kind != FCP_OUT_F32   ? FCP_VAR_NARROW
                   : mixed                            ? FCP_VAR_TABMIX
                   : facts->tab_kind == FCP_TAB_Q8    ? FCP_VAR_TABQ8
                   : facts->tab_kind != FCP_TAB_F32   ? FCP_VAR_TAB16
                                                      : FCP_VAR_F32;
  return FCP_OK;
}

}

using namespace fcph;

int fcp_internal_fail(int code, const std::string &msg) { return fail(code, msg); }

extern "C" {

int fcp_abi_version(void) { return FCP_ABI_VERSION; }

const char *fcp_status_string(int status) {
  switch (status) {
  case FCP_OK: return "ok";
  case FCP_ERR_INVALID_ARGUMENT: return "invalid argument";
  case FCP_ERR_SHAPE_MISMATCH: return "run-time shapes do not match the plan";
  case FCP_ERR_ALLOC: return "allocator callback failed";
  case FCP_ERR_HIP: return "HIP runtime error";
  case FCP_ERR_UNSUPPORTED: return "unsupported";
  case FCP_ERR_NO_DEVICE: return "no usable gfx950 device";
  default: return "unknown status";
  }
}

const char *fcp_last_error(void) { return g_last_error.c_str(); }

int fcp_plan_create_from_file(const char *path, int32_t device, uint32_t flags, fcp_plan_t **out) {
  if (!path || !out) return fail(FCP_ERR_INVALID_ARGUMENT, "null argument");
  *out = nullptr;
  ParsedPlanFile P;
  const int rc = parse_plan_file(path, P);
  if (rc) return rc;
  const std::string where = std::string("column plan ") + path + ": ";
  if (P.has_stage && (int32_t)P.stage_modes.size() != P.d.n_host_inputs)
    return fail(FCP_ERR_INVALID_ARGUMENT, where + "the stage section lists " + std::to_string(P.stage_modes.size()) + " inputs, the plan has " +
                                              std::to_string(P.d.n_host_inputs) + " host inputs");
  P.d.device = device;
  if (P.out_kind != FCP_OUT_F32 && (flags & fcpf::kOutFlags & ~fcpf::kOut[P.out_kind].flag))
    return fail(FCP_ERR_INVALID_ARGUMENT, where + "flags ask for another output dtype than the file's out_dtype line");
  if (P.tab_kind != FCP_TAB_F32 && (flags & fcpf::kTabFlags & ~fcpf::kTab[P.tab_kind].flag))
    return fail(FCP_ERR_INVALID_ARGUMENT, where + "flags ask for another table dtype than the file's table_dtype line");
  if (!P.in_kinds.empty() && (flags & fcpf::kTabFlags))
    return fail(FCP_ERR_INVALID_ARGUMENT, where + "plan-wide table dtype flags with a file that carries a table_dtypes line");
  P.d.flags = flags | fcpf::kOut[P.out_kind].flag | fcpf::kTab[P.tab_kind].flag | (P.in_kinds.empty() ? 0u : FCP_FLAG_TABLES_PER_INPUT);
  return fcp_plan_create_ex(&P.d, P.ext.empty() ? nullptr : P.ext.data(), out);
}

int fcp_plan_file_stage_info(const char *path, int32_t *n_inputs, uint8_t *modes, int32_t *rows_symbol, int32_t capacity,
                             int32_t *symbols_input) {
  if (!path) return fail(FCP_ERR_INVALID_ARGUMENT, "null argument");
  ParsedPlanFile P;
  const int rc = parse_plan_file(path, P);
  if (rc) return rc;
  const int32_t n = P.has_stage ? (int32_t)P.stage_modes.size() : 0;
  if (n_inputs) *n_inputs = n;
  if (symbols_input) *symbols_input = P.has_stage ? P.stage_symbols_input : -1;
  for (int32_t i = 0; i < n && i < capacity; ++i) {
    if (modes) modes[i] = P.stage_modes[i];
    if (rows_symbol) rows_symbol[i] = P.stage_rows_symbol[i];
  }
  return FCP_OK;
}

int fcp_placement_assign(const int64_t *table_bytes, int32_t n_tables, int64_t hbm_bytes, int64_t reserve_bytes, int32_t world,
                         int32_t prefer_mode, int32_t *owner, fcp_placement_t *out) {
  if (!out || n_tables < 0 || (n_tables > 0 && !table_bytes) || hbm_bytes <= 0 || reserve_bytes < 0 || world < 1)
    return fail(FCP_ERR_INVALID_ARGUMENT, "bad placement arguments");
  if (prefer_mode != FCP_PLACE_COLUMN_SHARD && prefer_mode != FCP_PLACE_ROW_SHARD && prefer_mode != FCP_PLACE_MIXED)
    return fail(FCP_ERR_INVALID_ARGUMENT, "prefer_mode must be column sharding, row sharding or mixed");
  const int64_t budget = hbm_bytes - reserve_bytes;
  if (budget <= 0) return fail(FCP_ERR_INVALID_ARGUMENT, "reserve_bytes leaves no room for tables");
  int64_t total = 0, largest = 0;
  for (int32_t t = 0; t < n_tables; ++t) {
    if (table_bytes[t] < 0) return fail(FCP_ERR_INVALID_ARGUMENT, "negative table size");
    total += table_bytes[t];
    largest = std::max(largest, table_bytes[t]);
  }
  out->min_world = (int32_t)std::max<int64_t>(1, (total + budget - 1) / budget);
  out->mode = FCP_PLACE_REPLICATE;
  out->bytes_per_gpu = total;
  if (owner)
    for (int32_t t = 0; t < n_tables; ++t) owner[t] = 0;
  if (total <= budget) return FCP_OK;
  const int64_t row_share = (total + world - 1) / world;
  const bool row_ok = world > 1 && row_share <= budget;
  std::vector<int32_t> assign(n_tables, -1);
  int32_t n_whole = 0;
  auto pack = [&](int64_t spread_over, int64_t *share) {
    int64_t spread = 0;
    std::vector<int32_t> order;
    for (int32_t t = 0; t < n_tables; ++t) {
      if (table_bytes[t] > spread_over) {
        spread += table_bytes[t];
        assign[t] = -1;
      } else {
        order.push_back(t);
      }
    }
    std::vector<int64_t> load(world, (spread + world - 1) / world);
    std::stable_sort(order.begin(), order.end(), [&](int32_t a, int32_t b) { return table_bytes[a] > table_bytes[b]; });
    for (int32_t t : order) {
      const int32_t r = (int32_t)(std::min_element(load.begin(), load.end()) - load.begin());
      load[r] += table_bytes[t];
      assign[t] = r;
    }
    *share = *std::max_element(load.begin(), load.end());
    n_whole = (int32_t)order.size();
    return *share <= budget;
  };
  int64_t col_share = 0, mixed_share = 0;
  const bool col_ok = world > 1 && largest <= budget && pack(INT64_MAX, &col_share);
  int mode;
  if (prefer_mode == FCP_PLACE_MIXED) {
    if (col_ok) mode = FCP_PLACE_COLUMN_SHARD;
    else if (world > 1 && largest > budget && pack(budget, &mixed_share) && n_whole >= world) mode = FCP_PLACE_MIXED;
    else if (row_ok) mode = FCP_PLACE_ROW_SHARD;
    else mode = -1;
  } else {
    if (!row_ok && !col_ok) mode = -1;
    else mode = (col_ok && (prefer_mode == FCP_PLACE_COLUMN_SHARD || !row_ok)) ? FCP_PLACE_COLUMN_SHARD : FCP_PLACE_ROW_SHARD;
  }
  if (mode < 0)
    return fail(FCP_ERR_UNSUPPORTED, "tables of " + std::to_string(total) + " bytes do not fit " + std::to_string(world) +
                                         " GPU(s) with " + std::to_string(budget) + " bytes each: needs at least " +
                                         std::to_string(out->min_world));
  out->mode = mode;
  if (mode == FCP_PLACE_COLUMN_SHARD) {
    (void)pack(INT64_MAX, &col_share);
    out->bytes_per_gpu = col_share;
  } else if (mode == FCP_PLACE_MIXED) {
    out->bytes_per_gpu = mixed_share;
  } else {
    out->bytes_per_gpu = row_share;
    std::fill(assign.begin(), assign.end(), -1);
  }
  if (owner)
    for (int32_t t = 0; t < n_tables; ++t) owner[t] = assign[t];
  return FCP_OK;
}

int fcp_placement_decide(const int64_t *table_bytes, int32_t n_tables, int64_t hbm_bytes, int64_t reserve_bytes,
                         int32_t world, int32_t prefer_mode, fcp_placement_t *out) {
  return fcp_placement_assign(table_bytes, n_tables, hbm_bytes, reserve_bytes, world, prefer_mode, nullptr, out);
}

int fcp_table_formats_choose(const fcp_table_audit_t *audits, const int64_t *rows, const int32_t *dims, int32_t n_tables,
                             int64_t budget_bytes, uint32_t allowed_kinds, const double *table_weight, int32_t *kinds_out,
                             int64_t *bytes_out, double *error_out) {
  const char *who = "fcp_table_formats_choose: ";
  if (n_tables < 0) return fail(FCP_ERR_INVALID_ARGUMENT, std::string(who) + "n_tables is negative");
  if (n_tables > 0 && (!audits || !rows || !dims || !kinds_out))
    return fail(FCP_ERR_INVALID_ARGUMENT, std::string(who) + "audits, rows, dims or kinds_out is null");
  if (budget_bytes < 0) return fail(FCP_ERR_INVALID_ARGUMENT, std::string(who) + "budget_bytes is negative");
  struct Point {
// ... 70 lines not shown
```

recom_amd/csrc/fcp_plan_desc.h:

```cpp
#pragma once
#include <cstdint>
#include <string>
#include <vector>

#include "../../include/fcp_hip.h"
#include "fcp_formats.h"
#include "fcp_internal.h"

namespace fcph {

int fail(int code, const std::string &msg);

struct PlanFacts {
  uint32_t flags = 0;
  int out_kind = FCP_OUT_F32;
  int tab_kind = FCP_TAB_F32;
  std::vector<int8_t> col_kind;
  FcpVariant variant = FCP_VAR_F32;
};

int check_desc(const fcp_plan_desc_t *d, const fcp_column_ext_t *ext, PlanFacts *facts);

}
```

recom_amd/csrc/fcp_process.hip:

```cpp
#include "fcp_host.h"

namespace fcph {

bool stream_is_capturing(hipStream_t stream) {
  hipStreamCaptureStatus st = hipStreamCaptureStatusNone;
  if (stream && hipStreamIsCapturing(stream, &st) == hipSuccess) return st == hipStreamCaptureStatusActive;
  (void)hipGetLastError();
  return false;
}

static bool fill_plain_image(const fcp_plan *p, const FcpColStatic *cols, FcpColDyn *h_dyn) {
  char *img = reinterpret_cast<char *>(h_dyn) + slot_image_off(p);
  std::memcpy(img, p->plain_tmpl.data(), p->plain_tmpl.size());
  for (const auto &e : p->plain_entries) {
    FcpPlainCol *c = reinterpret_cast<FcpPlainCol *>(img + e.first);
    c->table = cols[e.second].table;
    c->ids_off = h_dyn[e.second].ids_off;
    const uint64_t off = (uint64_t)c->ids_off;
    if ((off & 3) || (off >> 32)) return false;
    const uint32_t rec = e.first / (uint32_t)p->plain_stride * (uint32_t)p->plain_stride;
    const uint32_t j = (e.first - rec - (uint32_t)p->plain_cols_off) / (uint32_t)sizeof(FcpPlainCol);
    const uint32_t kind = c->kind == FCP_IDS_I64 ? FCP_PLAIN_FACT_I64 : c->kind == FCP_IDS_I32 ? FCP_PLAIN_FACT_I32 : FCP_PLAIN_FACT_F32;
    reinterpret_cast<uint32_t *>(img + rec + FCP_PLAIN_FACTS_OFF)[j] = (uint32_t)(off >> 2) | kind << 30;
  }
  return true;
}

int bind_tables(fcp_plan *p, const void *const *input_ptrs, bool capturing) {
  const int nt = p->desc.n_device_inputs;
  if (p->tables_bound && std::memcmp(p->bound_tables.data(), input_ptrs, nt * sizeof(void *)) == 0)
    return FCP_OK;
  if (capturing)
    return fail(FCP_ERR_UNSUPPORTED, "stream capture of a request whose tables are not bound to the plan yet (or have moved): run it "
                                     "once on this stream before capturing");
  std::vector<FcpColStatic> cols = p->h_cols;
  for (size_t k = 0; k < p->cols.size(); ++k) {
    const int t = p->cols[k].d.table_input;
    const bool lookup = p->cols[k].d.form == FCP_FORM_GATHER || p->cols[k].d.form == FCP_FORM_SEGMENT_REDUCE ||
                        p->cols[k].d.form == FCP_FORM_GATHER_SCATTER;
    if (lookup) {
      const bool empty_shard = p->desc.shard_world > 1 && p->cols[k].d.vocab <= p->desc.shard_rank;
      if (!input_ptrs[t] && !empty_shard) return fail(FCP_ERR_INVALID_ARGUMENT, "null table pointer");
      cols[p->pos_of[k]].table = static_cast<const float *>(input_ptrs[t]);
    }
  }
  if (p->tables_bound) HIP_TRY(hipDeviceSynchronize());
  p->tables_bound = false;
  HIP_TRY(hipMemcpy(p->d_cols, cols.data(), cols.size() * sizeof(FcpColStatic), hipMemcpyHostToDevice));
  p->h_cols.swap(cols);
  if (p->plain_dense) {
    for (auto &s : p->slots) {
      if (!s.img_built) continue;
      (void)fill_plain_image(p, p->h_cols.data(), s.h_dyn);
      const size_t off = slot_image_off(p);
      HIP_TRY(hipMemcpy(reinterpret_cast<char *>(s.d_dyn) + off, reinterpret_cast<const char *>(s.h_dyn) + off, p->plain_tmpl.size(),
                        hipMemcpyHostToDevice));
    }
  }
  for (int t = 0; t < nt; ++t) p->bound_tables[t] = input_ptrs[t];
  p->tables_bound = true;
  return FCP_OK;
}

int done_event_for(DynSlot &s, void *stream) {
  s.done_gen = 0;
  for (auto &e : s.done_pool)
    if (e.first == stream) {
      s.done = e.second;
      return FCP_OK;
    }
  hipEvent_t ev = nullptr;
  HIP_TRY(hipEventCreateWithFlags(&ev, hipEventDisableTiming | hipEventDisableSystemFence));
  s.done_pool.emplace_back(stream, ev);
  s.done = ev;
  return FCP_OK;
}

void build_key(const fcp_plan *p, const fcp_process_args_t *a, std::vector<int32_t> &key) {
  const int nh = (int)p->ranks.size();
  const int nsym = a->symbols ? p->desc.n_symbols : 0;
  const size_t key_len = (size_t)nh + p->rank_sum + nsym + 3;
  key.resize(key_len);
  std::memcpy(key.data(), a->concated_offsets, nh * sizeof(int32_t));
  std::memcpy(key.data() + nh, a->concated_shapes, p->rank_sum * sizeof(int32_t));
  if (nsym) std::memcpy(key.data() + nh + p->rank_sum, a->symbols, nsym * sizeof(int32_t));
  key[key_len - 3] = (int32_t)std::min<int64_t>(a->concated_bytes, 0x7fffffff);
  const uint64_t stream_bits = (uint64_t)reinterpret_cast<uintptr_t>(a->stream);
  key[key_len - 2] = (int32_t)(uint32_t)stream_bits;
  key[key_len - 1] = (int32_t)(uint32_t)(stream_bits >> 32);
}

int find_or_reserve(fcp_plan *p, const std::vector<int32_t> &key, DynSlot **out, bool *install, bool capturing) {
  ++p->tick;
  DynSlot *victim = nullptr;
  int pinned = 0;
  for (auto &s : p->slots) {
    if (s.valid && s.key == key) {
      s.tick = p->tick;
      ++s.users;
      ++s.uses;
      s.done_valid = false;
      if (capturing) s.captured = true;
      *out = &s;
      *install = false;
      return FCP_OK;
    }
    if (s.captured) {
      ++pinned;
      continue;
    }
    if (s.users > 0) continue;
    auto rank = [](const DynSlot &x) { return !x.valid ? 0 : (x.done_valid ? 1 : 2); };
    if (!victim || rank(s) < rank(*victim) || (rank(s) == rank(*victim) && s.tick < victim->tick)) victim = &s;
  }
  if (capturing) return kNeedsInstall;
  if (!victim)
    return pinned == kSlots ? fail(FCP_ERR_UNSUPPORTED, "every descriptor slot belongs to a captured graph: fcp_plan_release_captures")
                            : kAllSlotsBusy;
  victim->was_valid = victim->valid;
  victim->img_built = false;
  victim->valid = false;
  victim->users = 1;
  *out = victim;
  *install = true;
  return FCP_OK;
}

int install_slot(fcp_plan *p, const fcp_process_args_t *a, DynSlot &s) {
  hipStream_t stream = static_cast<hipStream_t>(a->stream);
  if (s.was_valid) {
    if (!s.done_valid) {
      if (s.stream == a->stream) {
        HIP_TRY(hipStreamSynchronize(stream));
      } else {
        HIP_TRY(hipDeviceSynchronize());
      }
    } else if (s.done_gen != 0 && s.done_gen != g_lane_generation.load(std::memory_order_acquire)) {
    } else if (hipEventQuery(s.done) != hipSuccess) {
      HIP_TRY(hipEventSynchronize(s.done));
    }
    if (!p->host_writes_dyn && hipEventQuery(s.uploaded) != hipSuccess) HIP_TRY(hipEventSynchronize(s.uploaded));
  }
  int rc = compute_dyn(p, a->concated_offsets, a->concated_shapes, a->symbols, a->concated_bytes, s.h_dyn, &s.meta);
  if (rc) return rc;
  if (p->has_weights) {
    rc = compute_weights(p, a->concated_offsets, a->concated_shapes, reinterpret_cast<int64_t *>(s.h_dyn + p->cols.size()));
    if (rc) return rc;
  }
  p->last_work_bytes.store(s.meta.work_bytes, std::memory_order_relaxed);
  s.meta.plain = p->plain_dense && s.meta.geo[0].rows_per_wave == 4 && s.meta.geo[1].grid_blocks == 0 &&
                 s.meta.geo[0].groups[0].span_list_off < 0 && s.meta.geo[0].groups[0].nlist == p->plain_spans;
  std::unique_lock<std::mutex> image_lock(p->mu, std::defer_lock);
  if (s.meta.plain) {
    image_lock.lock();
    s.meta.plain = fill_plain_image(p, p->h_cols.data(), s.h_dyn);
    s.img_built = s.meta.plain;
    if (!s.meta.plain) image_lock.unlock();
  }
  const size_t dyn_bytes = s.meta.plain ? slot_dyn_bytes(p) : (slot_dyn_bytes(p) - (p->plain_dense ? p->plain_tmpl.size() : 0));
  if (p->host_writes_dyn) {
    std::memcpy(s.d_dyn, s.h_dyn, dyn_bytes);
    __builtin_ia32_sfence();
  } else {
    const int e = fcp_launch_upload(s.h_dyn_dev, s.d_dyn, dyn_bytes, stream);
    if (e) return hip_fail("descriptor upload launch", (hipError_t)e);
    HIP_TRY(hipEventRecord(s.uploaded, stream));
  }
  return done_event_for(s, a->stream);
}

void publish_slot(fcp_plan *p, DynSlot &s, const std::vector<int32_t> &key, void *stream) {
  s.done_valid = false;
  s.uses = 1;
  s.key = key;
  s.stream = stream;
  s.tick = p->tick;
  s.valid = true;
}

int store_policy_for(fcp_plan *p, const void *arena, int64_t out_bytes) {
  const int64_t through_bytes = p->env.store_through_bytes;
  const uintptr_t ar = reinterpret_cast<uintptr_t>(arena);
  const uintptr_t a0 = p->recent_arena[0].load(std::memory_order_relaxed), a1 = p->recent_arena[1].load(std::memory_order_relaxed);
  const bool reused = ar == a0 || ar == a1;
  if (ar != a0) {
    p->recent_arena[1].store(a0, std::memory_order_relaxed);
    p->recent_arena[0].store(ar, std::memory_order_relaxed);
  }
  constexpr int64_t kPlainMaxBytes = (int64_t)160 << 20;
  if (out_bytes < through_bytes) return 0;
  return (reused && out_bytes <= kPlainMaxBytes) ? 4 : 1;
}

void fill_launch(const fcp_plan *p, const DynSlot &s, int kind, const void *blob, void *arena, int store_policy, FcpLaunch *L) {
  L->slot_map = p->d_slot_map;
  L->span_list = p->d_span_list;
  L->cols = p->d_cols;
  L->xforms = p->d_xforms;
  L->zeros = p->d_zeros;
  L->dyn = s.d_dyn;
  L->blob = static_cast<const char *>(blob);
  L->arena = static_cast<char *>(arena);
  L->bad_ids = p->d_bad;
  L->csr_arena_off = s.meta.csr_arena_off;
  L->shard_rank = p->desc.shard_rank;
  L->shard_world = p->desc.shard_world;
  L->n_groups = p->desc.n_groups;
  L->rows_per_wave = s.meta.geo[kind].rows_per_wave;
  L->seg_search = s.meta.seg_search ? 1 : 0;
  L->store_through = store_policy | (p->wide_rows ? 2 : 0);
  L->csr_reg = s.meta.csr_reg_mode == 1   ? reinterpret_cast<const int32_t *>(static_cast<const char *>(arena) + s.meta.csr_arena_off)
               : s.meta.csr_reg_mode == 2 ? reinterpret_cast<const int32_t *>(static_cast<const char *>(blob) + s.meta.csr_reg_base)
                                          : nullptr;
  for (int g = 0; g < p->desc.n_groups; ++g) L->groups[g] = s.meta.geo[kind].groups[g];
  L->groups[0].csr_reg_stride = (s.meta.csr_reg_mode && L->csr_reg) ? s.meta.csr_reg_stride : 0;
}

}

struct VariantEntry {
  FcpFusedLauncher *launch;
  const char *what;
  int32_t launch_base;
};
static const VariantEntry kVariants[FCP_VARIANTS] = {
    {fcp_launch_f32, nullptr , 0},
    {fcp_launch_weighted, "weighted ragged kernel launch", FCP_LAUNCH_RAGGED_WEIGHTED - FCP_LAUNCH_RAGGED},
    {fcp_launch_narrow, "narrow-output kernel launch", FCP_LAUNCH_DENSE_NARROW - FCP_LAUNCH_DENSE},
    {fcp_launch_tab16, "16-bit-table kernel launch", FCP_LAUNCH_DENSE_TAB16 - FCP_LAUNCH_DENSE},
    {fcp_launch_tabq8, "8-bit-table kernel launch", FCP_LAUNCH_DENSE_TABQ8 - FCP_LAUNCH_DENSE},
    {fcp_launch_tabmix, "mixed-table kernel launch", FCP_LAUNCH_DENSE_TABMIX - FCP_LAUNCH_DENSE},
};
static const char *const kF32What[4] = {"", "dense kernel launch", "ragged kernel launch", "hybrid kernel launch"};

extern "C" {

int fcp_internal_process(fcp_plan_t *p, const fcp_process_args_t *a, fcp_process_result_t *r) {
  if (!p || !a) return fail(FCP_ERR_INVALID_ARGUMENT, "null plan / args");
  if (p->host_only) return fail(FCP_ERR_NO_DEVICE, "host-only plan cannot run");
  if (!a->concated_offsets || !a->concated_shapes) {
    if (!p->ranks.empty()) return fail(FCP_ERR_INVALID_ARGUMENT, "null offsets / shapes");
  }
  if (!a->malloc_buff) return fail(FCP_ERR_INVALID_ARGUMENT, "malloc_buff callback is required");
  if (p->desc.n_device_inputs > 0 && !a->input_ptrs) return fail(FCP_ERR_INVALID_ARGUMENT, "null input_ptrs");
  if (p->desc.n_symbols > 0 && !a->symbols) return fail(FCP_ERR_INVALID_ARGUMENT, "plan needs symbols");
  if (a->input_shapes) {
    for (size_t k = 0; k < p->cols.size(); ++k) {
      const HostColumn &hc = p->cols[k];
      const int f = hc.d.form;
      if (f == FCP_FORM_PASSTHROUGH || f == FCP_FORM_BATCH_COL_REDUCTION || f == FCP_FORM_EXTERNAL) continue;
      const int32_t *s = a->input_shapes + 2 * hc.d.table_input;
      const int64_t local_vocab = p->desc.shard_world > 1
                                      ? (hc.d.vocab - p->desc.shard_rank + p->desc.shard_world - 1) / p->desc.shard_world
                                      : hc.d.vocab;
      if (s[0] != local_vocab || s[1] != hc.d.dim + fcpf::kTab[p->col_tab_kind(k)].row_tail)
        return fail(FCP_ERR_SHAPE_MISMATCH, "table shape does not match the plan");
    }
  }
  DeviceGuard guard;
  int rc = guard.enter(p->desc.device);
  if (rc) return rc;
  hipStream_t stream = static_cast<hipStream_t>(a->stream);

  DynSlot *slot = nullptr;
  bool install = false;
  thread_local std::vector<int32_t> key;
  build_key(p, a, key);
  const bool capturing = stream_is_capturing(stream);
  {
    std::unique_lock<std::mutex> lock(p->mu);
    if (p->desc.n_device_inputs > 0) {
      rc = bind_tables(p, a->input_ptrs, capturing);
      if (rc) return rc;
    }
    while ((rc = find_or_reserve(p, key, &slot, &install, capturing)) == kAllSlotsBusy) {
      lock.unlock();
      std::this_thread::yield();
      lock.lock();
    }
    if (rc == kNeedsInstall)
      return fail(FCP_ERR_UNSUPPORTED, "stream capture of a request whose shapes are not resident: run it once on this stream "
                                       "before capturing (descriptors cannot be installed inside a capture)");
    if (rc) return rc;
  }
  SlotUnpin unpin{p, slot, false};
  if (install) {
    rc = install_slot(p, a, *slot);
    if (rc) return rc;
    std::lock_guard<std::mutex> lock(p->mu);
    publish_slot(p, *slot, key, a->stream);
  }
  const DynMeta &m = slot->meta;
  tl_work_bytes = m.work_bytes;
  if (m.arena_bytes > 0 && !a->concated_inputs && !p->ranks.empty() && a->concated_bytes != 0)
    return fail(FCP_ERR_INVALID_ARGUMENT, "null blob");

  void *arena = a->malloc_buff(a->malloc_buff_ctx, (size_t)std::max<int64_t>(m.arena_bytes, 128));
  if (!arena) return fail(FCP_ERR_ALLOC, "malloc_buff returned NULL");
  if (const LaneDep *dep = tl_lane_dep) {
    tl_lane_dep = nullptr;
    HIP_TRY(hipEventRecord(dep->in, dep->caller));
    HIP_TRY(hipStreamWaitEvent(dep->lane, dep->in, 0));
  }

  FcpLaunch L;
  const int store_policy = store_policy_for(p, arena, m.csr_arena_off);
  fill_launch(p, *slot, 1, a->concated_inputs, arena, store_policy, &L);
  {
    fcp_plan::LastLaunch &ll = p->last_launch;
    const int32_t fused = (int32_t)(m.geo[0].grid_blocks > 0) | (int32_t)(m.geo[1].grid_blocks > 0) << 1;
    const int32_t mine = p->variant == FCP_VAR_WEIGHTED ? fused & FCP_LAUNCH_RAGGED : fused;
    ll.kernel.store(mine ? mine + kVariants[p->variant].launch_base : FCP_LAUNCH_NONE, std::memory_order_relaxed);
    p->last_dense_front.store(m.geo[0].grid_blocks <= 0 || p->weighted_kernel ? FCP_DENSE_FRONT_NONE
                              : m.plain                                       ? FCP_DENSE_FRONT_PLAIN
                                                                              : FCP_DENSE_FRONT_GENERIC,
                              std::memory_order_relaxed);
    ll.rows_per_wave.store(m.geo[0].rows_per_wave, std::memory_order_relaxed);
    ll.store_policy.store(store_policy, std::memory_order_relaxed);
    ll.dense_blocks.store(m.geo[0].grid_blocks, std::memory_order_relaxed);
    ll.ragged_blocks.store(m.geo[1].grid_blocks, std::memory_order_relaxed);
    ll.segment_offsets.store(p->seg_cols.empty() ? 0 : (m.seg_search ? 2 : 1), std::memory_order_relaxed);
    ll.csr_arena_off.store(m.csr_arena_off, std::memory_order_relaxed);
    for (int k : p->seg_cols) ll.csr_base[k].store(slot->h_dyn[p->pos_of[k]].csr_base, std::memory_order_relaxed);
  }
  if (!p->seg_cols.empty() && !m.seg_search) {
    FcpSegLaunch S;
    S.seg_cols = p->d_seg_cols;
    S.cols = p->d_cols;
    S.dyn = slot->d_dyn;
    S.blob = L.blob;
    S.arena = L.arena;
    S.bad_ids = p->d_bad;
    S.xforms = p->d_xforms;
    S.segmaps = p->d_segmaps;
    S.skip_inverse = 0;
    S.csr_arena_off = m.csr_arena_off;
    if (p->has_inverse) {
      const int64_t first = m.csr_arena_off + 4 * (int64_t)slot->h_dyn[p->pos_of[p->seg_cols[p->n_seg_plain]]].csr_base;
      if (m.arena_bytes > first) HIP_TRY(hipMemsetAsync(static_cast<char *>(arena) + first, 0, (size_t)(m.arena_bytes - first), stream));
    }
    const bool prepass_any_order = p->request_order == FCP_ORDER_INPUTS_READY && !capturing && !p->has_inverse &&
                                   !(install && !p->host_writes_dyn);
    const int e = fcp_launch_segment_offsets(S, (int)p->seg_cols.size(), m.max_seg_nnz, stream, prepass_any_order);
    if (e) return hip_fail("segment-offsets launch", (hipError_t)e);
  }
  const bool attach_done = install && !fcp_stop_event_pending() && !capturing;
  if (attach_done) fcp_set_stop_event(slot->done);
  struct ClearStop {
    bool armed;
    ~ClearStop() {
      if (armed) fcp_set_stop_event(nullptr);
    }
  } clear_stop{attach_done};
  const bool queued_before = (!p->seg_cols.empty() && !m.seg_search) || (install && !p->host_writes_dyn);
  struct ClearAnyOrder {
    ~ClearAnyOrder() { fcp_set_any_order(false); }
  } clear_any_order;
  if (p->request_order == FCP_ORDER_INPUTS_READY && !queued_before && !capturing) fcp_set_any_order(true);
  const int dense_blocks = p->variant == FCP_VAR_WEIGHTED ? 0 : m.geo[0].grid_blocks, ragged_blocks = m.geo[1].grid_blocks;
  if (dense_blocks > 0 && m.plain) {
    const FcpGroupLaunch &G = m.geo[0].groups[0];
    FcpPlainLaunch P;
    P.img = reinterpret_cast<const char *>(slot->d_dyn) + slot_image_off(p);
    P.blob = static_cast<const char *>(a->concated_inputs);
    P.out = reinterpret_cast<float *>(static_cast<char *>(arena) + m.group_base[0]);
    P.bad_ids = p->d_bad;
    P.rows = G.rows;
    P.nslots = G.nslots;
    P.nsp8 = G.nsp8;
    P.nlist = G.nlist;
    P.img_stride = p->plain_stride;
    P.out_stride = p->group_width[0];
    P.store_policy = store_policy;
    const int e = fcp_launch_dense_plain(P, dense_blocks, stream);
    if (e) return hip_fail("plain dense kernel launch", (hipError_t)e);
  } else {
    FcpLaunch Ld;
    FcpLaunch *dense = ragged_blocks > 0 ? &Ld : &L;
    if (dense_blocks > 0) fill_launch(p, *slot, 0, a->concated_inputs, arena, store_policy, dense);
    const VariantEntry &V = kVariants[p->variant];
    const FcpFusedWork W = {dense, dense_blocks, &L, ragged_blocks, p->vec, p->variant == FCP_VAR_NARROW ? p->out_kind : p->tab_kind,
                            slot_weights(p, slot->d_dyn)};
    const int e = V.launch(W, stream);
    if (e) return hip_fail(p->variant == FCP_VAR_F32 ? kF32What[(dense_blocks > 0) | (ragged_blocks > 0) << 1] : V.what, (hipError_t)e);
  }
  if (install) {
    const bool taken = attach_done && !fcp_stop_event_pending();
    clear_stop.armed = false;
    if (attach_done && !taken) fcp_set_stop_event(nullptr);
    if (tl_lane_done) {
      slot->done = tl_lane_done;
      slot->done_gen = tl_lane_done_gen;
    } else if (!taken) {
      HIP_TRY(hipEventRecord(slot->done, stream));
    }
    unpin.recorded = true;
  }

  if (r) {
    const int nc = (int)p->cols.size();
    for (int k = 0; k < nc; ++k) {
      const FcpColDyn &d = slot->h_dyn[p->pos_of[k]];
      if (r->output_ptrs) r->output_ptrs[k] = static_cast<char *>(arena) + d.out_base;
      if (r->output_shapes) {
        r->output_shapes[2 * k] = d.rows;
        r->output_shapes[2 * k + 1] = p->cols[k].d.dim;
      }
      if (r->output_row_strides) r->output_row_strides[k] = d.out_stride;
    }
    for (int g = 0; g < p->desc.n_groups; ++g) {
      if (r->group_ptrs)
        r->group_ptrs[g] = p->desc.layout == FCP_LAYOUT_CONCAT ? static_cast<char *>(arena) + m.group_base[g] : nullptr;
      if (r->group_shapes) {
        r->group_shapes[2 * g] = m.group_rows[g];
        r->group_shapes[2 * g + 1] = p->group_width[g];
      }
    }
    r->buffer = arena;
    r->buffer_bytes = m.arena_bytes;
  }
  return FCP_OK;
}

int fcp_process_feature_columns(fcp_plan_t *p, const fcp_process_args_t *a, fcp_process_result_t *r) {
  if (!p || !a) return fail(FCP_ERR_INVALID_ARGUMENT, "null plan / args");
  if (!p->pool || p->lane_count == 0) return fcp_internal_process(p, a, r);
  return process_on_private_streams(p, a, r);
}

int fcp_plan_traffic_bind(fcp_plan_t *p, uint32_t *const *counts, int32_t n_counts, int64_t *skipped) {
  const std::string w = "fcp_plan_traffic_bind: ";
  if (!p) return fail(FCP_ERR_INVALID_ARGUMENT, w + "null plan");
  if (n_counts < 0) return fail(FCP_ERR_INVALID_ARGUMENT, w + "`n_counts` is negative");
  if (n_counts != 0 && n_counts != p->desc.n_device_inputs)
    return fail(FCP_ERR_INVALID_ARGUMENT, w + "`n_counts` must be the plan's number of device inputs (" +
                                              std::to_string(p->desc.n_device_inputs) + "), or 0 to unbind");
  if (n_counts > 0 && !counts) return fail(FCP_ERR_INVALID_ARGUMENT, w + "`counts` is null");
  for (int32_t t = 0; t < n_counts; ++t)
    if ((uintptr_t)counts[t] % 4) return fail(FCP_ERR_INVALID_ARGUMENT, w + "`counts[" + std::to_string(t) + "]` is not 4-byte aligned");
  if ((uintptr_t)skipped % 8) return fail(FCP_ERR_INVALID_ARGUMENT, w + "`skipped` is not 8-byte aligned");
  std::vector<FcpTrafficCol> list;
  for (size_t pos = 0; pos < p->cols.size() && n_counts > 0; ++pos) {
    const fcp_column_desc_t &c = p->cols[p->order[pos]].d;
    if (c.form != FCP_FORM_GATHER && c.form != FCP_FORM_SEGMENT_REDUCE && c.form != FCP_FORM_GATHER_SCATTER) continue;
    if (counts[c.table_input]) list.push_back({counts[c.table_input], (int32_t)pos, 0});
  }
  if (p->host_only) {
    if (list.empty()) return FCP_OK;
    return fail(FCP_ERR_NO_DEVICE, w + "host-only plan cannot count");
  }
  DeviceGuard guard;
  const int rc = guard.enter(p->desc.device);
  if (rc) return rc;
  std::lock_guard<std::mutex> lock(p->mu);
  if (p->traffic_n > 0) HIP_TRY(hipDeviceSynchronize());
  p->traffic_n = 0;
  p->traffic_skipped = nullptr;
  if (list.empty()) return FCP_OK;
  if (!p->d_traffic) HIP_TRY(hipMalloc(&p->d_traffic, p->cols.size() * sizeof(FcpTrafficCol)));
  HIP_TRY(hipMemcpy(p->d_traffic, list.data(), list.size() * sizeof(FcpTrafficCol), hipMemcpyHostToDevice));
  p->traffic_n = (int32_t)list.size();
  p->traffic_skipped = reinterpret_cast<unsigned long long *>(skipped);
  return FCP_OK;
}

int fcp_plan_traffic_count(fcp_plan_t *p, const fcp_process_args_t *a) {
  const std::string w = "fcp_plan_traffic_count: ";
  if (!p || !a) return fail(FCP_ERR_INVALID_ARGUMENT, w + "null plan / args");
  if ((!a->concated_offsets || !a->concated_shapes) && !p->ranks.empty())
    return fail(FCP_ERR_INVALID_ARGUMENT, w + "null offsets / shapes");
  if (p->desc.n_symbols > 0 && !a->symbols) return fail(FCP_ERR_INVALID_ARGUMENT, w + "plan needs symbols");
  if (p->host_only) return fail(FCP_ERR_INVALID_ARGUMENT, w + "no counts are bound (a host-only plan cannot bind any): `fcp_plan_traffic_bind`");
  DeviceGuard guard;
  int rc = guard.enter(p->desc.device);
  if (rc) return rc;
  hipStream_t stream = static_cast<hipStream_t>(a->stream);
  DynSlot *slot = nullptr;
  bool install = false;
  thread_local std::vector<int32_t> key;
  build_key(p, a, key);
  const bool capturing = stream_is_capturing(stream);
  FcpTrafficLaunch T;
  int32_t n_list = 0;
  {
    std::unique_lock<std::mutex> lock(p->mu);
    if (p->traffic_n == 0) return fail(FCP_ERR_INVALID_ARGUMENT, w + "no counts are bound: `fcp_plan_traffic_bind` first");
    n_list = p->traffic_n;
    T.list = p->d_traffic;
    T.skipped = p->traffic_skipped;
    while ((rc = find_or_reserve(p, key, &slot, &install, capturing)) == kAllSlotsBusy) {
      lock.unlock();
      std::this_thread::yield();
      lock.lock();
    }
    if (rc == kNeedsInstall)
      return fail(FCP_ERR_UNSUPPORTED, "stream capture of a request whose shapes are not resident: run it once on this stream "
                                       "before capturing (descriptors cannot be installed inside a capture)");
    if (rc) return rc;
  }
  SlotUnpin unpin{p, slot, false};
  if (install) {
    rc = install_slot(p, a, *slot);
    if (rc) return rc;
    std::lock_guard<std::mutex> lock(p->mu);
    publish_slot(p, *slot, key, a->stream);
  }
  const DynMeta &m = slot->meta;
  if (m.max_lookup_nnz > 0 && !a->concated_inputs) return fail(FCP_ERR_INVALID_ARGUMENT, w + "null blob");
  T.cols = p->d_cols;
  T.dyn = slot->d_dyn;
  T.xforms = p->d_xforms;
  T.blob = static_cast<const char *>(a->concated_inputs);
  const int e = fcp_launch_plan_traffic(T, n_list, m.max_lookup_nnz, stream);
  if (e) return hip_fail("traffic count kernel launch", (hipError_t)e);
  if (install) {
    HIP_TRY(hipEventRecord(slot->done, stream));
    unpin.recorded = true;
  }
  return FCP_OK;
}

}
```

recom_amd/lib.py:

```python
from __future__ import annotations

import ctypes as C
import os

from .plan import (FLAG_OUT_BF16, FLAG_OUT_F16, FLAG_TABLES_BF16, FLAG_TABLES_F16, FLAG_TABLES_PER_INPUT, FLAG_TABLES_Q8,
                   OUT_FORMATS, TABLE_FORMATS)

_HERE = os.path.dirname(os.path.abspath(__file__))
LIB_PATH = os.path.join(os.environ.get("FCP_LIB_DIR", _HERE), "libfcp_hip.so")

FCP_ABI_VERSION = 2
FCP_OK = 0
FCP_ERR_INVALID_ARGUMENT = 1
FCP_ERR_SHAPE_MISMATCH = 2
FCP_ERR_ALLOC = 3
FCP_ERR_HIP = 4
FCP_ERR_UNSUPPORTED = 5
FCP_ERR_NO_DEVICE = 6
FLAG_HOST_ONLY = 1 << 31
OUT_DTYPES = dict(enumerate(OUT_FORMATS))
OUT_DTYPE_FLAGS = {name: f.flag for name, f in OUT_FORMATS.items()}
ALL_TABLE_DTYPES = dict(enumerate(TABLE_FORMATS))
ALL_TABLE_DTYPE_FLAGS = {name: f.flag for name, f in TABLE_FORMATS.items()}
TAB_Q8 = 3
TABLE_DTYPES = {k: n for k, n in ALL_TABLE_DTYPES.items() if k != TAB_Q8}
TABLE_DTYPE_FLAGS = {n: ALL_TABLE_DTYPE_FLAGS[n] for n in TABLE_DTYPES.values()}
TAB_MIXED = 255
PLAN_TABLE_DTYPES = {**ALL_TABLE_DTYPES, TAB_MIXED: "mixed"}
TABLE_KINDS = {name: kind for kind, name in ALL_TABLE_DTYPES.items()}
LAUNCH_KERNELS = {0: "none", 1: "dense", 2: "ragged", 3: "hybrid", 4: "ragged_weighted",
                  5: "dense_narrow", 6: "ragged_narrow", 7: "hybrid_narrow",
                  8: "dense_tab16", 9: "ragged_tab16", 10: "hybrid_tab16",
                  11: "dense_tabq8", 12: "ragged_tabq8", 13: "hybrid_tabq8",
                  14: "dense_tabmix", 15: "ragged_tabmix", 16: "hybrid_tabmix"}
DENSE_FRONTS = {0: "none", 1: "generic", 2: "plain"}
LAUNCH_STORES = {0: "nt", 1: "sc1_nt", 4: "plain"}
LAUNCH_SEGMENT_OFFSETS = {0: "none", 1: "prepass", 2: "search"}
AUX_KERNELS = ("segment_offsets", "shard_finalize_v4", "shard_finalize_v2", "shard_finalize_v1",
               "concat_v4", "concat_v2", "concat_v1", "upload", "h2d_copy")


class FcpError(RuntimeError):
    def __init__(self, status: int, what: str, detail: str = "") -> None:
        self.status = status
        super().__init__(f"{what}: status {status}" + (f" ({detail})" if detail else ""))


class ColumnDesc(C.Structure):
    _fields_ = [
        ("form", C.c_int32), ("combiner", C.c_int32), ("dim", C.c_int32), ("id_source", C.c_int32),
        ("vocab", C.c_int64),
        ("table_input", C.c_int32), ("ids_input", C.c_int32), ("seg_input", C.c_int32),
        ("seg_kind", C.c_int32), ("seg_stride", C.c_int32),
        ("rows_source", C.c_int32), ("rows_arg", C.c_int32),
        ("n_boundaries", C.c_int32),
        ("boundaries", C.POINTER(C.c_float)),
        ("concat_group", C.c_int32), ("concat_slot", C.c_int32),
        ("xform_mode", C.c_int32), ("xform_n", C.c_int32),
        ("xform_lo", C.POINTER(C.c_int64)), ("xform_hi", C.POINTER(C.c_int64)),
        ("xform_substitute", C.c_int64), ("hash_buckets", C.c_int64),
    ]


class ColumnExt(C.Structure):
    _fields_ = [
        ("seg_map_n", C.c_int32), ("seg_map_sym", C.c_int32), ("seg_map_sym_slot", C.c_int32), ("weights_input1", C.c_int32),
        ("seg_map_mul", C.c_int64 * 4), ("seg_map_div", C.c_int64),
        ("table_kind1", C.c_int32), ("reserved0", C.c_int32), ("reserved1", C.c_int64 * 1),
    ]


class PlanDesc(C.Structure):
    _fields_ = [
        ("abi_version", C.c_int32), ("n_columns", C.c_int32),
        ("columns", C.POINTER(ColumnDesc)),
        ("n_host_inputs", C.c_int32),
        ("host_input_ranks", C.POINTER(C.c_int32)),
        ("host_input_elem_sizes", C.POINTER(C.c_int32)),
        ("n_device_inputs", C.c_int32), ("n_groups", C.c_int32), ("n_symbols", C.c_int32),
        ("layout", C.c_int32), ("device", C.c_int32),
        ("shard_rank", C.c_int32), ("shard_world", C.c_int32),
        ("flags", C.c_uint32),
    ]


ALLOC_FN = C.CFUNCTYPE(C.c_void_p, C.c_void_p, C.c_size_t)


class ProcessArgs(C.Structure):
    _fields_ = [
        ("concated_inputs", C.c_void_p), ("concated_bytes", C.c_int64),
        ("concated_offsets", C.POINTER(C.c_int32)), ("concated_shapes", C.POINTER(C.c_int32)),
        ("input_ptrs", C.POINTER(C.c_void_p)), ("input_shapes", C.POINTER(C.c_int32)),
        ("symbols", C.POINTER(C.c_int32)),
        ("stream", C.c_void_p),
        ("malloc_temp", ALLOC_FN), ("malloc_temp_ctx", C.c_void_p),
        ("malloc_buff", ALLOC_FN), ("malloc_buff_ctx", C.c_void_p),
    ]


class ProcessResult(C.Structure):
    _fields_ = [
        ("output_ptrs", C.POINTER(C.c_void_p)), ("output_shapes", C.POINTER(C.c_int32)),
        ("output_row_strides", C.POINTER(C.c_int64)),
        ("group_ptrs", C.POINTER(C.c_void_p)), ("group_shapes", C.POINTER(C.c_int32)),
        ("buffer", C.c_void_p), ("buffer_bytes", C.c_int64),
    ]


class Placement(C.Structure):
    _fields_ = [("mode", C.c_int32), ("min_world", C.c_int32), ("bytes_per_gpu", C.c_int64)]


class TableAuditKind(C.Structure):
    _fields_ = [("rows_bad", C.c_int64), ("first_bad_row", C.c_int64), ("sum_sq_err", C.c_double), ("max_abs_err", C.c_float),
                ("reserved", C.c_int32)]


class TableAudit(C.Structure):
    _fields_ = [("rows", C.c_int64), ("rows_nonfinite", C.c_int64), ("first_nonfinite_row", C.c_int64), ("sum_sq", C.c_double),
                ("kind", TableAuditKind * 4)]


class TableDigest(C.Structure):
    _fields_ = [("sum", C.c_uint64), ("rows", C.c_int64), ("skipped", C.c_int64), ("reserved", C.c_int64)]


class TableDeltaReport(C.Structure):
    _fields_ = [("n", C.c_int64), ("distinct", C.c_int64), ("duplicates", C.c_int64), ("skipped", C.c_int64)]


class OutputError(C.Structure):
    _fields_ = [("elems", C.c_int64), ("differ", C.c_int64), ("nonfinite", C.c_int64), ("first_differ_row", C.c_int64),
                ("sum_sq_ref", C.c_double), ("sum_sq_err", C.c_double), ("max_abs_err", C.c_float), ("max_abs_ref", C.c_float),
                ("reserved", C.c_int64)]


class PrivateStreamsStats(C.Structure):
    _fields_ = [("supervised_stream", C.c_void_p), ("requests", C.c_int64), ("lane_requests", C.c_int64), ("evaluations", C.c_int64),
                ("stream_order_us_per_mib", C.c_double), ("last_ratio", C.c_double), ("worst_ratio", C.c_double),
                ("keep_ratio", C.c_double), ("demoted", C.c_int32), ("evaluation_in_progress", C.c_int32)]


class LaunchInfo(C.Structure):
    _fields_ = [("kernel", C.c_int32), ("vec", C.c_int32), ("rows_per_wave", C.c_int32), ("store_policy", C.c_int32),
                ("wide_rows", C.c_int32), ("shard_world", C.c_int32), ("dense_blocks", C.c_int32), ("ragged_blocks", C.c_int32),
                ("segment_offsets", C.c_int32)]


class StagerStats(C.Structure):
    _fields_ = [("calls", C.c_int64), ("copy_calls", C.c_int64), ("copy_calls_over_1ms", C.c_int64), ("fallback_switches", C.c_int64),
                ("requests_with_blocked_copy", C.c_int64), ("max_copy_call_us", C.c_double)]


class HostTensor(C.Structure):
    _fields_ = [("data", C.c_void_p), ("elem_size", C.c_int32), ("rank", C.c_int32),
                ("dims", C.POINTER(C.c_int64))]


EXPORTS = [
    "fcp_abi_version", "fcp_status_string", "fcp_last_error",
    "fcp_concat_inputs_sizes", "fcp_concat_inputs",
    "fcp_plan_create", "fcp_plan_create_ex", "fcp_plan_create_from_file", "fcp_plan_counts", "fcp_plan_destroy", "fcp_plan_group_width",
    "fcp_plan_column_offset",
    "fcp_plan_arena_bytes", "fcp_plan_read_bad_ids", "fcp_plan_output_columns", "fcp_plan_table_bytes",
    "fcp_placement_decide", "fcp_plan_release_captures",
    "fcp_process_feature_columns", "fcp_concat_outputs", "fcp_concat_outputs_scatter", "fcp_concat_outputs_host",
    "fcp_shard_finalize", "fcp_comm_unique_id", "fcp_comm_create", "fcp_comm_destroy", "fcp_comm_rank",
    "fcp_shard_batch_slice", "fcp_shard_exchange", "fcp_shard_exchange_columns",
    "fcp_shard_step_create", "fcp_shard_step_run", "fcp_shard_step_destroy",
    "fcp_stager_create", "fcp_stager_create_ex", "fcp_stager_stage", "fcp_stager_stage_ex", "fcp_stager_stage_narrow", "fcp_stager_destroy", "fcp_stager_stats",
    "fcp_concat_inputs_ex_sizes", "fcp_concat_inputs_ex", "fcp_plan_file_stage_info",
    "fcp_pack_pool_create", "fcp_pack_pool_destroy", "fcp_concat_inputs_ex_pool",
    "fcp_graph_build", "fcp_graph_free", "fcp_placement_assign", "fcp_concat_outputs_scatter_strided",
    "fcp_plan_set_private_streams", "fcp_result_wait", "fcp_result_synchronize", "fcp_plan_set_request_order",
    "fcp_plan_probe_private_streams", "fcp_plan_private_streams_verdict", "fcp_plan_verify_private_streams",
    "fcp_plan_private_streams_stats", "fcp_plan_last_launch", "fcp_plan_last_csr", "fcp_aux_launch_counts",
    "fcp_plan_out_dtype", "fcp_plan_last_dense_front", "fcp_plan_table_dtype",
    "fcp_table_row_bytes", "fcp_table_convert", "fcp_table_update_rows", "fcp_table_read_rows",
    "fcp_plan_table_kinds",
    "fcp_table_audit_workspace_bytes", "fcp_table_audit", "fcp_table_formats_choose",
    "fcp_table_audit_weighted", "fcp_table_count_ids",
    "fcp_plan_table_rows", "fcp_plan_traffic_bind", "fcp_plan_traffic_count",
    "fcp_table_digest_workspace_bytes", "fcp_table_digest", "fcp_table_digest_rows", "fcp_table_digest_host",
    "fcp_table_delta_workspace_bytes", "fcp_table_delta_distinct",
    "fcp_outputs_compare_workspace_bytes", "fcp_outputs_compare",
]

_lib = None


def _build_in_tree() -> None:
    import shutil
    import subprocess
    hipcc = os.environ.get("HIPCC", "/opt/rocm/bin/hipcc")
    if not (os.path.exists(hipcc) or shutil.which("hipcc")) or not shutil.which("make"):
        return
    import fcntl
    try:
        with open(os.path.join(_HERE, "csrc", ".build.lock"), "w") as lock:
            fcntl.flock(lock, fcntl.LOCK_EX)
            if not os.path.exists(LIB_PATH):
                subprocess.check_call(["make", "-C", os.path.join(_HERE, "csrc")], stdout=subprocess.DEVNULL)
    except (subprocess.CalledProcessError, OSError):
        pass


def load() -> C.CDLL:
    global _lib
    if _lib is not None:
        return _lib
    try:
        import torch
    except ImportError:
        pass
    if not os.path.exists(LIB_PATH) and "FCP_LIB_DIR" not in os.environ:
        _build_in_tree()
    if not os.path.exists(LIB_PATH):
        raise ImportError(
            f"{LIB_PATH} not found: build it with `python -c 'import __graft_entry__ as g; g.build()'` "
            "(hipcc --offload-arch=gfx950). There is no CPU fallback for the product path.")
    L = C.CDLL(LIB_PATH)
    L.fcp_abi_version.restype = C.c_int
    L.fcp_status_string.restype = C.c_char_p
    L.fcp_status_string.argtypes = [C.c_int]
    L.fcp_last_error.restype = C.c_char_p
    L.fcp_concat_inputs_sizes.argtypes = [C.POINTER(HostTensor), C.c_int32, C.POINTER(C.c_int64),
                                          C.POINTER(C.c_int32)]
    L.fcp_concat_inputs.argtypes = [C.POINTER(HostTensor), C.c_int32, C.c_void_p, C.c_int64,
                                    C.c_void_p, C.c_void_p]
    L.fcp_plan_create.argtypes = [C.POINTER(PlanDesc), C.POINTER(C.c_void_p)]
    if hasattr(L, "fcp_plan_create_ex"):
        L.fcp_plan_create_ex.argtypes = [C.POINTER(PlanDesc), C.POINTER(ColumnExt), C.POINTER(C.c_void_p)]
    L.fcp_plan_create_from_file.argtypes = [C.c_char_p, C.c_int32, C.c_uint32, C.POINTER(C.c_void_p)]
    L.fcp_plan_counts.argtypes = [C.c_void_p] + [C.POINTER(C.c_int32)] * 5
    L.fcp_plan_destroy.argtypes = [C.c_void_p]
    L.fcp_plan_group_width.argtypes = [C.c_void_p, C.c_int32, C.POINTER(C.c_int32)]
    L.fcp_plan_column_offset.argtypes = [C.c_void_p, C.c_int32, C.POINTER(C.c_int32)]
    L.fcp_plan_arena_bytes.argtypes = [C.c_void_p, C.c_void_p, C.c_void_p, C.POINTER(C.c_int64)]
    L.fcp_plan_read_bad_ids.argtypes = [C.c_void_p, C.c_void_p, C.POINTER(C.c_int64)]
    L.fcp_process_feature_columns.argtypes = [C.c_void_p, C.POINTER(ProcessArgs), C.POINTER(ProcessResult)]
    L.fcp_concat_outputs.argtypes = [C.POINTER(C.c_void_p), C.c_void_p, C.c_int32, C.c_int64, C.c_void_p,
                                     C.c_void_p]
    L.fcp_plan_output_columns.argtypes = [C.c_void_p, C.POINTER(C.c_int32), C.c_void_p, C.c_int32]
    L.fcp_plan_table_bytes.argtypes = [C.c_void_p, C.POINTER(C.c_int64), C.POINTER(C.c_int64)]
    L.fcp_plan_out_dtype.argtypes = [C.c_void_p, C.POINTER(C.c_int32)]
    L.fcp_plan_table_dtype.argtypes = [C.c_void_p, C.POINTER(C.c_int32)]
    L.fcp_plan_table_kinds.argtypes = [C.c_void_p, C.POINTER(C.c_int32), C.c_int32, C.POINTER(C.c_int32)]
    L.fcp_plan_release_captures.argtypes = [C.c_void_p]
    L.fcp_placement_decide.argtypes = [C.c_void_p, C.c_int32, C.c_int64, C.c_int64, C.c_int32, C.c_int32,
                                       C.POINTER(Placement)]
    L.fcp_concat_outputs_scatter.argtypes = [C.POINTER(C.c_void_p), C.c_void_p, C.c_void_p, C.c_int32, C.c_int64,
                                             C.c_int32, C.c_void_p, C.c_void_p]
    L.fcp_concat_outputs_host.argtypes = [C.POINTER(C.c_void_p), C.c_void_p, C.c_void_p, C.c_int32, C.c_int64,
                                          C.c_int32, C.c_void_p, ALLOC_FN, C.c_void_p, C.c_int32, C.c_void_p]
    L.fcp_shard_finalize.argtypes = [C.c_void_p, C.POINTER(ProcessArgs), C.c_int32, C.c_void_p, C.c_int32,
                                     C.c_int64, C.c_int64, C.c_void_p, C.c_void_p]
    L.fcp_comm_unique_id.argtypes = [C.c_void_p]
    L.fcp_comm_create.argtypes = [C.c_void_p, C.c_int32, C.c_int32, C.c_int32, C.POINTER(C.c_void_p)]
    L.fcp_comm_destroy.argtypes = [C.c_void_p]
    L.fcp_comm_rank.argtypes = [C.c_void_p, C.POINTER(C.c_int32), C.POINTER(C.c_int32)]
    L.fcp_shard_batch_slice.argtypes = [C.c_int64, C.c_int32, C.c_int32, C.POINTER(C.c_int64), C.POINTER(C.c_int64)]
    L.fcp_shard_exchange.argtypes = [C.c_void_p, C.c_void_p, C.c_int64, C.c_int64, C.c_void_p, C.POINTER(C.c_int64),
                                     C.POINTER(C.c_int64), C.c_void_p]
    L.fcp_shard_exchange_columns.argtypes = [C.c_void_p, C.c_void_p, C.c_int64, C.c_void_p, C.c_void_p,
                                             C.POINTER(C.c_int64), C.POINTER(C.c_int64), C.c_void_p]
    L.fcp_shard_step_create.argtypes = [C.c_void_p, C.c_void_p, C.c_int32, C.c_int32, C.c_int64, C.c_int64, C.c_void_p,
                                        C.POINTER(C.c_void_p)]
    L.fcp_shard_step_run.argtypes = [C.c_void_p, C.POINTER(ProcessArgs), C.POINTER(C.c_void_p), C.POINTER(C.c_int64),
                                     C.POINTER(C.c_int64)]
    L.fcp_shard_step_destroy.argtypes = [C.c_void_p]
    L.fcp_stager_stage_ex.argtypes = [C.c_void_p, C.POINTER(HostTensor), C.c_int32, C.c_void_p, C.c_void_p, C.c_void_p,
                                      C.POINTER(C.c_void_p), C.POINTER(C.c_int64), C.POINTER(C.POINTER(C.c_int32)),
                                      C.POINTER(C.POINTER(C.c_int32))]
    L.fcp_stager_create_ex.argtypes = [C.c_int32, C.c_int64, C.c_int32, C.c_int32, C.c_int32, C.c_int32, C.c_uint32,
                                       C.POINTER(C.c_void_p)]
    L.fcp_stager_create.argtypes = [C.c_int32, C.c_int64, C.c_int32, C.c_int32, C.c_int32, C.c_int32,
                                    C.POINTER(C.c_void_p)]
    L.fcp_stager_stage.argtypes = [C.c_void_p, C.POINTER(HostTensor), C.c_int32, C.c_void_p, C.POINTER(C.c_void_p),
                                   C.POINTER(C.c_int64), C.POINTER(C.POINTER(C.c_int32)),
                                   C.POINTER(C.POINTER(C.c_int32))]
    L.fcp_stager_stage_narrow.argtypes = [C.c_void_p, C.POINTER(HostTensor), C.c_int32, C.POINTER(C.c_uint8),
                                          C.c_void_p, C.POINTER(C.c_void_p), C.POINTER(C.c_int64),
                                          C.POINTER(C.POINTER(C.c_int32)), C.POINTER(C.POINTER(C.c_int32))]
    L.fcp_stager_destroy.argtypes = [C.c_void_p]
    if hasattr(L, "fcp_stager_stats"):
        L.fcp_stager_stats.argtypes = [C.c_void_p, C.POINTER(StagerStats)]
    if hasattr(L, "fcp_pack_pool_create"):
        L.fcp_pack_pool_create.argtypes = [C.c_int32, C.POINTER(C.c_void_p)]
        L.fcp_pack_pool_destroy.argtypes = [C.c_void_p]
        L.fcp_concat_inputs_ex_pool.argtypes = [C.c_void_p, C.POINTER(HostTensor), C.c_int32, C.c_void_p, C.c_void_p, C.c_void_p,
                                                C.c_int64, C.c_void_p, C.c_void_p]
    if "FCP_LIB_DIR" not in os.environ or hasattr(L, "fcp_concat_inputs_ex"):
        L.fcp_concat_inputs_ex_sizes.argtypes = [C.POINTER(HostTensor), C.c_int32, C.c_void_p, C.c_void_p, C.POINTER(C.c_int64),
                                                 C.POINTER(C.c_int32)]
        L.fcp_concat_inputs_ex.argtypes = [C.POINTER(HostTensor), C.c_int32, C.c_void_p, C.c_void_p, C.c_void_p, C.c_int64,
                                           C.c_void_p, C.c_void_p]
        L.fcp_plan_file_stage_info.argtypes = [C.c_char_p, C.POINTER(C.c_int32), C.c_void_p, C.c_void_p, C.c_int32,
                                               C.POINTER(C.c_int32)]
        L.fcp_graph_build.argtypes = [C.c_char_p, C.c_size_t, C.c_uint32, C.c_char_p, C.POINTER(C.c_void_p), C.POINTER(C.c_size_t),
                                      C.POINTER(C.c_char_p)]
        L.fcp_graph_free.argtypes = [C.c_void_p]
        L.fcp_graph_free.restype = None
        L.fcp_placement_assign.argtypes = [C.c_void_p, C.c_int32, C.c_int64, C.c_int64, C.c_int32, C.c_int32, C.c_void_p,
                                           C.POINTER(Placement)]
        L.fcp_concat_outputs_scatter_strided.argtypes = [C.POINTER(C.c_void_p), C.c_void_p, C.c_void_p, C.c_void_p, C.c_int32,
                                                         C.c_int64, C.c_int32, C.c_void_p, C.c_void_p]
    if hasattr(L, "fcp_plan_set_private_streams"):
        L.fcp_plan_set_private_streams.argtypes = [C.c_void_p, C.c_int32, C.c_uint32]
        L.fcp_result_wait.argtypes = [C.c_void_p, C.c_void_p]
        L.fcp_result_synchronize.argtypes = [C.c_void_p]
    if hasattr(L, "fcp_plan_probe_private_streams"):
        L.fcp_plan_probe_private_streams.argtypes = [C.c_void_p, C.c_void_p, C.c_int32, C.c_int32, C.c_int32,
                                                     C.POINTER(C.c_double), C.POINTER(C.c_double)]
        L.fcp_plan_private_streams_verdict.argtypes = [C.c_void_p, C.c_void_p, C.POINTER(C.c_int32)]
    if hasattr(L, "fcp_plan_verify_private_streams"):
        L.fcp_plan_verify_private_streams.argtypes = [C.c_void_p, C.c_void_p, C.c_int32, C.POINTER(C.c_int32)]
        L.fcp_plan_private_streams_stats.argtypes = [C.c_void_p, C.POINTER(PrivateStreamsStats)]
    if hasattr(L, "fcp_plan_set_request_order"):
        L.fcp_plan_set_request_order.argtypes = [C.c_void_p, C.c_int32]
    if hasattr(L, "fcp_plan_last_launch"):
        L.fcp_plan_last_launch.argtypes = [C.c_void_p, C.POINTER(LaunchInfo)]
    if hasattr(L, "fcp_aux_launch_counts"):
        L.fcp_plan_last_csr.argtypes = [C.c_void_p, C.POINTER(C.c_int64), C.c_void_p, C.c_int32]
        L.fcp_aux_launch_counts.argtypes = [C.c_void_p, C.c_int32, C.c_int32]
    if hasattr(L, "fcp_plan_last_dense_front"):
        L.fcp_plan_last_dense_front.argtypes = [C.c_void_p, C.POINTER(C.c_int32)]
    if hasattr(L, "fcp_table_convert"):
        L.fcp_table_row_bytes.restype = C.c_int64
        L.fcp_table_row_bytes.argtypes = [C.c_int32, C.c_int32]
        L.fcp_table_convert.argtypes = [C.c_void_p, C.c_int32, C.c_int64, C.c_void_p, C.c_int32, C.c_int64, C.c_int32, C.c_int32,
                                        C.c_void_p]
    if hasattr(L, "fcp_table_update_rows"):
        L.fcp_table_update_rows.argtypes = [C.c_void_p, C.c_int32, C.c_int64, C.c_int32, C.c_void_p, C.c_void_p, C.c_int64,
                                            C.c_void_p, C.c_int32, C.c_void_p]
        L.fcp_table_read_rows.argtypes = [C.c_void_p, C.c_void_p, C.c_int32, C.c_int64, C.c_int32, C.c_void_p, C.c_int64,
                                          C.c_int32, C.c_void_p]
    if hasattr(L, "fcp_table_audit"):
        L.fcp_table_audit_workspace_bytes.restype = C.c_int64
        L.fcp_table_audit_workspace_bytes.argtypes = []
        L.fcp_table_audit.argtypes = [C.c_void_p, C.c_int64, C.c_int32, C.c_void_p, C.c_void_p, C.c_int32, C.c_void_p]
        L.fcp_table_formats_choose.argtypes = [C.POINTER(TableAudit), C.POINTER(C.c_int64), C.POINTER(C.c_int32), C.c_int32, C.c_int64,
                                               C.c_uint32, C.POINTER(C.c_double), C.POINTER(C.c_int32), C.POINTER(C.c_int64),
                                               C.POINTER(C.c_double)]
    if hasattr(L, "fcp_table_count_ids"):
        L.fcp_table_audit_weighted.argtypes = [C.c_void_p, C.c_int64, C.c_int32, C.c_void_p, C.c_void_p, C.c_void_p, C.c_int32, C.c_void_p]
        L.fcp_table_count_ids.argtypes = [C.c_void_p, C.c_int64, C.c_void_p, C.c_int32, C.c_int64, C.c_void_p, C.c_int32, C.c_void_p]
    if hasattr(L, "fcp_plan_traffic_count"):
        L.fcp_plan_table_rows.argtypes = [C.c_void_p, C.POINTER(C.c_int64), C.c_int32, C.POINTER(C.c_int32)]
        L.fcp_plan_traffic_bind.argtypes = [C.c_void_p, C.POINTER(C.c_void_p), C.c_int32, C.c_void_p]
        L.fcp_plan_traffic_count.argtypes = [C.c_void_p, C.POINTER(ProcessArgs)]
    if hasattr(L, "fcp_table_digest"):
        L.fcp_table_digest_workspace_bytes.restype = C.c_int64
        L.fcp_table_digest_workspace_bytes.argtypes = []
        L.fcp_table_digest.argtypes = [C.c_void_p, C.c_int32, C.c_int64, C.c_int32, C.c_int64, C.c_int64, C.c_void_p, C.c_void_p,
                                       C.c_int32, C.c_void_p]
        L.fcp_table_digest_rows.argtypes = [C.c_void_p, C.c_int32, C.c_int64, C.c_int32, C.c_int64, C.c_int64, C.c_void_p, C.c_int64,
                                            C.c_void_p, C.c_void_p, C.c_int32, C.c_void_p]
        L.fcp_table_digest_host.restype = C.c_uint64
        L.fcp_table_digest_host.argtypes = [C.c_void_p, C.c_int32, C.c_int64, C.c_int32, C.c_int64, C.c_int64]
    if hasattr(L, "fcp_table_delta_distinct"):
        L.fcp_table_delta_workspace_bytes.restype = C.c_int64
        L.fcp_table_delta_workspace_bytes.argtypes = [C.c_int64]
        L.fcp_table_delta_distinct.argtypes = [C.c_void_p, C.c_int32, C.c_void_p, C.c_int32, C.c_int64, C.c_int64, C.c_void_p, C.c_void_p,
                                               C.c_void_p, C.c_void_p, C.c_void_p, C.c_int32, C.c_void_p]
    if hasattr(L, "fcp_outputs_compare"):
        L.fcp_outputs_compare_workspace_bytes.restype = C.c_int64
        L.fcp_outputs_compare_workspace_bytes.argtypes = [C.c_int32]
        L.fcp_outputs_compare.argtypes = [C.c_void_p, C.c_void_p, C.c_int32, C.c_void_p, C.c_void_p, C.c_int32, C.c_void_p, C.c_int32,
                                          C.c_void_p, C.c_void_p, C.c_int32, C.c_void_p]
    if L.fcp_abi_version() != FCP_ABI_VERSION:
        raise ImportError("libfcp_hip.so ABI version mismatch; rebuild")
    _lib = L
    return L


def aux_launch_counts(reset: bool = False) -> dict:
    L = load()
    counts = (C.c_int64 * len(AUX_KERNELS))()
    n = L.fcp_aux_launch_counts(counts, len(AUX_KERNELS), 1 if reset else 0)
    if n != len(AUX_KERNELS):
        raise FcpError(-n if n < 0 else FCP_ERR_UNSUPPORTED, "fcp_aux_launch_counts", f"{n} counters")
    return dict(zip(AUX_KERNELS, counts[:]))


def check(status: int, what: str) -> None:
    if status != FCP_OK:
        L = load()
        detail = L.fcp_last_error().decode(errors="replace") or L.fcp_status_string(status).decode()
        raise FcpError(status, what, detail)
```

recom_amd/ops.py:

```python
from __future__ import annotations

import ctypes as C
import os
from dataclasses import dataclass
from typing import List, Optional, Sequence

import numpy as np

from . import lib as _lib
from .plan import (FORM_BATCH_COL_REDUCTION, FORM_GATHER, FORM_GATHER_SCATTER, FORM_PASSTHROUGH, FORM_SEGMENT_REDUCE,
                   IDS_F32_BUCKETIZE, LAYOUT_CONCAT, PlanSpec)


def _host_tensors(inputs):
    arrs = [np.require(np.asarray(a), requirements="C") for a in inputs]
    dims_keep = [np.asarray(a.shape, np.int64) for a in arrs]
    tens = (_lib.HostTensor * max(len(arrs), 1))()
    for i, a in enumerate(arrs):
        tens[i] = _lib.HostTensor(a.ctypes.data, a.dtype.itemsize, a.ndim,
                                  dims_keep[i].ctypes.data_as(C.POINTER(C.c_int64)))
    return arrs, dims_keep, tens


class PackPool:
# ... 157 lines not shown
        _lib.check(self._L.fcp_plan_out_dtype(self.handle, C.byref(v)), "fcp_plan_out_dtype")
        return _lib.OUT_DTYPES[v.value]

    def table_dtype(self) -> str:
        v = C.c_int32()
        _lib.check(self._L.fcp_plan_table_dtype(self.handle, C.byref(v)), "fcp_plan_table_dtype")
        return _lib.PLAN_TABLE_DTYPES[v.value]

    def table_dtypes(self) -> tuple:
        n = C.c_int32()
        _lib.check(self._L.fcp_plan_table_kinds(self.handle, None, 0, C.byref(n)), "fcp_plan_table_kinds")
        kinds = (C.c_int32 * max(1, n.value))()
        _lib.check(self._L.fcp_plan_table_kinds(self.handle, kinds, n.value, None), "fcp_plan_table_kinds")
        return tuple("-" if kinds[t] < 0 else _lib.ALL_TABLE_DTYPES[kinds[t]] for t in range(n.value))

    def table_rows(self) -> tuple:
        n = C.c_int32()
        _lib.check(self._L.fcp_plan_table_rows(self.handle, None, 0, C.byref(n)), "fcp_plan_table_rows")
        rows = (C.c_int64 * max(1, n.value))()
        _lib.check(self._L.fcp_plan_table_rows(self.handle, rows, n.value, None), "fcp_plan_table_rows")
        return tuple(int(rows[t]) for t in range(n.value))

    def traffic_bind(self, counts, skipped=None) -> None:
        import torch
        from . import tables as _tables
        if counts is None:
            _lib.check(self._L.fcp_plan_traffic_bind(self.handle, None, 0, None), "fcp_plan_traffic_bind")
            self._traffic_keep = None
            return
        rows = self.table_rows()
        if len(counts) != len(rows):
            raise ValueError(f"counts names {len(counts)} inputs, the plan has {len(rows)} device inputs")
        for t, c in enumerate(counts):
            if c is None:
                continue
            if _tables._check_counts(torch, c, f"counts[{t}]") != rows[t]:
                raise ValueError(f"counts[{t}] has {c.shape[0]} cells, the plan's table {t} has {rows[t]} rows (Plan.table_rows)")
        for t, c in enumerate(counts):
            if c is None:
                continue
            if not c.is_cuda or (c.device.index or 0) != self.device:
                raise ValueError(f"counts[{t}] is on {c.device}, the plan on cuda:{self.device}")
        if skipped is not None:
            if skipped.dtype != torch.int64 or skipped.numel() != 1 or not skipped.is_cuda or (skipped.device.index or 0) != self.device:
                raise ValueError("skipped is an int64 tensor of one element on the plan's device")
        ptrs = (C.c_void_p * max(1, len(counts)))(*[None if c is None else c.data_ptr() for c in counts])
        _lib.check(self._L.fcp_plan_traffic_bind(self.handle, ptrs, len(counts), None if skipped is None else C.c_void_p(skipped.data_ptr())),
                   "fcp_plan_traffic_bind")
        self._traffic_keep = (list(counts), skipped)

    def traffic_count(self, concated_inputs, concated_offsets, concated_shapes, symbols=None, stream: Optional[int] = None) -> None:
        import torch
        offs = np.ascontiguousarray(concated_offsets, np.int32)
        shps = np.ascontiguousarray(concated_shapes, np.int32)
        sym = None if symbols is None else np.ascontiguousarray(symbols, np.int32)
        if stream is None:
            stream = torch.cuda.current_stream(torch.device("cuda", self.device)).cuda_stream
        a = _lib.ProcessArgs(
            concated_inputs.data_ptr() if concated_inputs is not None and concated_inputs.numel() else None,
            0 if concated_inputs is None else concated_inputs.numel() * concated_inputs.element_size(),
            offs.ctypes.data_as(C.POINTER(C.c_int32)), shps.ctypes.data_as(C.POINTER(C.c_int32)), None, None,
            None if sym is None else sym.ctypes.data_as(C.POINTER(C.c_int32)), stream)
        _lib.check(self._L.fcp_plan_traffic_count(self.handle, C.byref(a)), "fcp_plan_traffic_count")

    def table_bytes(self):
        a, b = C.c_int64(), C.c_int64()
        _lib.check(self._L.fcp_plan_table_bytes(self.handle, C.byref(a), C.byref(b)), "fcp_plan_table_bytes")
        return a.value, b.value

    def counts(self) -> dict:
        v = [C.c_int32() for _ in range(5)]
        _lib.check(self._L.fcp_plan_counts(self.handle, *[C.byref(x) for x in v]), "fcp_plan_counts")
        return dict(zip(("columns", "groups", "host_inputs", "device_inputs", "symbols"), (x.value for x in v)))

    def close(self) -> None:
        if getattr(self, "handle", None):
            self._L.fcp_plan_destroy(self.handle)
            self.handle = None

    def __del__(self) -> None:
        try:
            self.close()
        except Exception:
            pass

    def group_width(self, group: int) -> int:
        w = C.c_int32()
        _lib.check(self._L.fcp_plan_group_width(self.handle, group, C.byref(w)), "fcp_plan_group_width")
        return w.value

    def column_offset(self, column: int) -> int:
        o = C.c_int32()
        _lib.check(self._L.fcp_plan_column_offset(self.handle, column, C.byref(o)), "fcp_plan_column_offset")
        return o.value

    def arena_bytes(self, shapes, symbols=None) -> int:
        shapes = np.ascontiguousarray(shapes, np.int32)
        sym = None if symbols is None else np.ascontiguousarray(symbols, np.int32)
        out = C.c_int64()
        _lib.check(self._L.fcp_plan_arena_bytes(self.handle, shapes.ctypes.data,
                                                None if sym is None else sym.ctypes.data, C.byref(out)),
                   "fcp_plan_arena_bytes")
        return out.value

    def set_private_streams(self, n_streams: int, no_caller_wait: bool = False, always: bool = False, verify: bool = True) -> None:
        _lib.check(self._L.fcp_plan_set_private_streams(self.handle, int(n_streams),
                                                        (1 if no_caller_wait else 0) | (2 if always else 0) | (0 if verify else 4)),
                   "fcp_plan_set_private_streams")
        self.private_streams = int(n_streams)

    def probe_private_streams(self, stream: int, requests: int = 24, spin_us: int = 20, grid_blocks: int = 2048):
        a, b = C.c_double(), C.c_double()
        _lib.check(self._L.fcp_plan_probe_private_streams(self.handle, C.c_void_p(stream), requests, spin_us, grid_blocks,
                                                         C.byref(a), C.byref(b)), "fcp_plan_probe_private_streams")
        return a.value, b.value

    def private_streams_verdict(self, stream: int) -> int:
        v = C.c_int32(-1)
        _lib.check(self._L.fcp_plan_private_streams_verdict(self.handle, C.c_void_p(stream), C.byref(v)), "fcp_plan_private_streams_verdict")
        return int(v.value)

    def verify_private_streams(self, stream: int, budget_ms: int = 0) -> int:
        v = C.c_int32(-1)
        _lib.check(self._L.fcp_plan_verify_private_streams(self.handle, C.c_void_p(stream), int(budget_ms), C.byref(v)),
                   "fcp_plan_verify_private_streams")
        return int(v.value)

    def private_streams_stats(self) -> dict:
        st = _lib.PrivateStreamsStats()
        _lib.check(self._L.fcp_plan_private_streams_stats(self.handle, C.byref(st)), "fcp_plan_private_streams_stats")
        return {k: getattr(st, k) for k, _ in st._fields_}

    def set_inputs_ready(self, on: bool = True) -> None:
        _lib.check(self._L.fcp_plan_set_request_order(self.handle, 1 if on else 0), "fcp_plan_set_request_order")

    def read_bad_ids(self, stream: int = 0) -> int:
        out = C.c_int64()
        _lib.check(self._L.fcp_plan_read_bad_ids(self.handle, stream, C.byref(out)), "fcp_plan_read_bad_ids")
        return out.value

    def last_launch(self) -> dict:
        li = _lib.LaunchInfo()
        _lib.check(self._L.fcp_plan_last_launch(self.handle, C.byref(li)), "fcp_plan_last_launch")
        return dict(kernel=_lib.LAUNCH_KERNELS[li.kernel], vec=li.vec, rows_per_wave=li.rows_per_wave,
                    store=_lib.LAUNCH_STORES[li.store_policy], wide_rows=bool(li.wide_rows), shard_world=li.shard_world,
                    dense_blocks=li.dense_blocks, ragged_blocks=li.ragged_blocks,
                    segment_offsets=_lib.LAUNCH_SEGMENT_OFFSETS[li.segment_offsets])

    def last_dense_front(self) -> str:
        v = C.c_int32()
        _lib.check(self._L.fcp_plan_last_dense_front(self.handle, C.byref(v)), "fcp_plan_last_dense_front")
        return _lib.DENSE_FRONTS[v.value]

    def last_csr(self):
        off = C.c_int64()
        n = self.spec.n_columns
        base = np.empty(max(n, 1), np.int32)
        _lib.check(self._L.fcp_plan_last_csr(self.handle, C.byref(off), base.ctypes.data, n), "fcp_plan_last_csr")
        return off.value, base[:n]


@dataclass
class ProcessOutputs:
    output_ptrs: np.ndarray
    output_shapes: np.ndarray
    output_row_strides: np.ndarray
    buffer: "object"
    groups: list
    group_shapes: np.ndarray

    def wait(self, stream: Optional[int] = None) -> None:
        import torch
        if stream is None:
            stream = torch.cuda.current_stream(self.buffer.device).cuda_stream
        _lib.check(_lib.load().fcp_result_wait(self.buffer.data_ptr(), stream), "fcp_result_wait")

    def column(self, k: int):
        import torch
        rows, dim = int(self.output_shapes[2 * k]), int(self.output_shapes[2 * k + 1])
        dtype = self.groups[0].dtype if self.groups else torch.float32
        f = _typed_arena(torch, self.buffer, dtype)
        off = (int(self.output_ptrs[k]) - self.buffer.data_ptr()) // f.element_size()
        return f.as_strided((rows, dim), (int(self.output_row_strides[k]), 1), off)


def _typed_arena(torch, arena, dtype):
    if dtype == torch.float32:
        return arena.view(torch.float32)
    return arena[:arena.numel() // 2 * 2].view(dtype)


OUTPUT_ERROR_DTYPE = np.dtype([("elems", "<i8"), ("differ", "<i8"), ("nonfinite", "<i8"), ("first_differ_row", "<i8"),
                               ("sum_sq_ref", "<f8"), ("sum_sq_err", "<f8"), ("max_abs_err", "<f4"), ("max_abs_ref", "<f4"),
                               ("reserved", "<i8")])

_compare_workspaces: dict = {}


@dataclass
class OutputErrors:
    columns: np.ndarray
    total: np.record

    def rel_rms(self, k: Optional[int] = None) -> float:
        r = self.total if k is None else self.columns[k]
        if r["sum_sq_ref"] == 0.0:
            return 0.0 if r["sum_sq_err"] == 0.0 else float("inf")
        return float(np.sqrt(r["sum_sq_err"] / r["sum_sq_ref"]))

    @property
    def identical(self) -> bool:
        return int(self.total["differ"]) == 0


def _out_kind(torch, outputs: ProcessOutputs) -> int:
    dtype = outputs.groups[0].dtype if outputs.groups else torch.float32
    return {torch.float32: 0, torch.bfloat16: 1, torch.float16: 2}[dtype]


def _same_request(a: ProcessOutputs, b: ProcessOutputs) -> np.ndarray:
    sa, sb = np.asarray(a.output_shapes, np.int32), np.asarray(b.output_shapes, np.int32)
    if sa.size != sb.size:
        raise ValueError(f"compare_outputs: {sa.size // 2} columns against {sb.size // 2}")
    if not np.array_equal(sa, sb):
        k = int(np.flatnonzero(sa != sb)[0]) // 2
        raise ValueError(f"compare_outputs: column {k} is [{sa[2 * k]}, {sa[2 * k + 1]}] in a and [{sb[2 * k]}, {sb[2 * k + 1]}] in b: "
                         "the two results are not of the same request")
    return sa


def compare_outputs_async(a: ProcessOutputs, b: ProcessOutputs, stream: Optional[int] = None):
    import torch
    sa = _same_request(a, b)
    n = sa.size // 2
    device = a.buffer.device
    if b.buffer.device != device:
        raise ValueError(f"compare_outputs: a lies on {device}, b on {b.buffer.device}")
    L = _lib.load()
    if stream is None:
        stream = torch.cuda.current_stream(device).cuda_stream
    need = int(L.fcp_outputs_compare_workspace_bytes(n))
    key = (device.index or 0, int(stream))
    with torch.cuda.stream(torch.cuda.ExternalStream(stream, device=device)):
        out = torch.empty((n + 1, OUTPUT_ERROR_DTYPE.itemsize // 8), dtype=torch.int64, device=device)
        workspace = _compare_workspaces.get(key)
        if workspace is None or workspace.numel() * 8 < need:
            workspace = _compare_workspaces[key] = torch.empty((need // 8,), dtype=torch.int64, device=device)
    pa, pb = np.ascontiguousarray(a.output_ptrs, np.int64), np.ascontiguousarray(b.output_ptrs, np.int64)
    ta, tb = np.ascontiguousarray(a.output_row_strides, np.int64), np.ascontiguousarray(b.output_row_strides, np.int64)
    shapes = np.ascontiguousarray(sa)
    status = L.fcp_outputs_compare(pa.ctypes.data, ta.ctypes.data, _out_kind(torch, a), pb.ctypes.data, tb.ctypes.data,
                                   _out_kind(torch, b), shapes.ctypes.data, n, out.data_ptr(), workspace.data_ptr(),
                                   device.index or 0, C.c_void_p(stream))
    _lib.check(status, "fcp_outputs_compare")
    return out


def compare_outputs(a: ProcessOutputs, b: ProcessOutputs, stream: Optional[int] = None) -> OutputErrors:
    import torch
    _same_request(a, b)
    if stream is None:
        stream = torch.cuda.current_stream(a.buffer.device).cuda_stream
    out = compare_outputs_async(a, b, stream)
    torch.cuda.ExternalStream(stream, device=a.buffer.device).synchronize()
    records = np.frombuffer(out.cpu().numpy().tobytes(), OUTPUT_ERROR_DTYPE).copy().view(np.recarray)
    return OutputErrors(records[:-1], records[-1])


class FeatureColumnProcess:

    def __init__(self, spec: PlanSpec, device: int = 0, plan: Optional[Plan] = None) -> None:
        import torch
        if not torch.cuda.is_available():
            raise RuntimeError("FeatureColumnProcess needs a GPU (no CPU fallback)")
        self.torch = torch
        self.device = torch.device("cuda", device)
        self.plan = plan if plan is not None else Plan(spec, device)
        self.spec = spec
        self._L = self.plan._L
        self.out_dtype = {"f32": torch.float32, "bf16": torch.bfloat16, "f16": torch.float16}[self.plan.out_dtype()]
        torch_dtypes = {"f32": torch.float32, "bf16": torch.bfloat16, "f16": torch.float16, "q8": torch.uint8}
        self.table_dtype = torch_dtypes.get(self.plan.table_dtype())
        kinds = self.plan.table_dtypes()
        self._input_dtypes = {t: torch_dtypes[k] for t, k in enumerate(kinds) if k != "-"}
        self._q8_shapes = {c.table_input: (int(c.vocab), int(c.dim) + 8) for c in self.plan.spec.columns
                           if c.form in (FORM_GATHER, FORM_SEGMENT_REDUCE, FORM_GATHER_SCATTER) and kinds[c.table_input] == "q8"}
        self._table_inputs = sorted({c.table_input for c in self.plan.spec.columns
                                     if c.form in (FORM_GATHER, FORM_SEGMENT_REDUCE, FORM_GATHER_SCATTER)})

    @classmethod
    def from_plan_file(cls, dlpath: str, device: int = 0) -> "FeatureColumnProcess":
        plan = Plan.from_file(dlpath, device)
        return cls(plan.spec, device, plan)

    def _allocators(self, arena=None):
        torch, dev = self.torch, self.device
        state = {"arena": None, "temps": [], "error": None}

        def _alloc(_ctx, nbytes):
            if arena is None:
                state["arena"] = torch.empty(int(nbytes), dtype=torch.uint8, device=dev)
                return state["arena"].data_ptr()
            have = arena.numel() * arena.element_size()
            if have < int(nbytes):
                state["error"] = ValueError(f"FeatureColumnProcess: caller arena of {have} bytes, the request needs {int(nbytes)} "
                                            "(Plan.arena_bytes)")
# ... 324 lines not shown
```

Baseline: 19.87 million.

## Add plain ragged kernel front fed by precomposed per-span column image

Adds a specialized ragged kernel for plain pooled f32 plans. The host precomputes a per-span image of column records (static plus dynamic fields, lane-to-column map), and each block loads it with wide vector loads straight into LDS. This replaces the generic locate_block, map lookup and per-column staging, and drops the xform pointer path. The cost is extra host-side image filling and upload per slot, more template specialization, and a narrow eligibility check that falls back to the generic path.

Measured after the change: 19.66 million. 0.99x the previous value.

```diff
diff --git a/include/fcp_hip.h b/include/fcp_hip.h
--- a/include/fcp_hip.h
+++ b/include/fcp_hip.h
@@ -314,6 +314,8 @@
 int fcp_plan_last_launch(const fcp_plan_t *plan, fcp_launch_info_t *out);
 enum { FCP_DENSE_FRONT_NONE = 0, FCP_DENSE_FRONT_GENERIC = 1, FCP_DENSE_FRONT_PLAIN = 2 };
 int fcp_plan_last_dense_front(const fcp_plan_t *plan, int32_t *front);
+enum { FCP_RAGGED_FRONT_NONE = 0, FCP_RAGGED_FRONT_GENERIC = 1, FCP_RAGGED_FRONT_PLAIN = 2 };
+int fcp_plan_last_ragged_front(const fcp_plan_t *plan, int32_t *front);
 int fcp_plan_last_csr(const fcp_plan_t *plan, int64_t *csr_arena_off, int32_t *csr_base, int32_t capacity);
 enum {
   FCP_AUX_SEGMENT_OFFSETS = 0,
diff --git a/recom_amd/csrc/fcp_fused_bodies.h b/recom_amd/csrc/fcp_fused_bodies.h
--- a/recom_amd/csrc/fcp_fused_bodies.h
+++ b/recom_amd/csrc/fcp_fused_bodies.h
@@ -931,10 +931,91 @@
   int32_t bound[FCP_WAVE * (FCP_WAVES_PER_BLOCK + 1)];
 };
 
-template <int V, bool SHARDED, FcpVariant X = FCP_VAR_F32>
-__device__ __forceinline__ void ragged_body(const FcpLaunch &L, int bid, char *smem, const int64_t *wts = nullptr, int kind = 0) {
+static_assert(sizeof(FcpRaggedCol) == sizeof(LdsCol) && offsetof(FcpRaggedCol, ids_off) == sizeof(FcpColStatic) &&
+                  offsetof(FcpRaggedCol, nnz) == sizeof(LdsCol) - 4 && sizeof(FcpColStatic) % 16 == 0 &&
+                  sizeof(FcpRaggedSpan) == FCP_RAGGED_COLS_OFF && FCP_RAGGED_COLS_OFF % 16 == 0 &&
+                  sizeof(FcpRaggedSpan) <= sizeof(RaggedLds::bound),
+              "image records: an 80-byte head that fits S.bound, then columns laid out as LdsCol");
+template <int RB>
+__device__ __forceinline__ bool ragged_front_image(const FcpRaggedPlainLaunch &L, int bid, RaggedLds &S, BlockPos &B, int &pre0, int &pre1,
+                                                   uint32_t &col_of_lane) {
+  typedef uint32_t __attribute__((ext_vector_type(4))) U4;
+  typedef uint32_t __attribute__((ext_vector_type(2))) U2;
+  const int tid = threadIdx.x;
+  const int lane = tid & (FCP_WAVE - 1);
+  const int wave = tid >> 6;
+  const int nsp8 = L.nsp8;
+  int idx, tile;
+  if (nsp8 > 0) {
+    const int xcd = bid & 7, j8 = bid >> 3;
+    idx = (j8 % nsp8) * 8 + xcd;
+    tile = j8 / nsp8;
+  } else {
+    idx = bid % (-nsp8);
+    tile = bid / (-nsp8);
+  }
+  B.rows = L.rows;
+  B.nslots = L.nslots;
+  B.q0 = idx * FCP_WAVE;
+  B.row_blk = tile * RB;
+  B.map = nullptr;
+  if (B.q0 >= B.nslots || B.row_blk >= B.rows) return false;
+  const char *rec = L.img + (int64_t)idx * L.img_stride;
+  const int n16 = L.img_stride >> 4;
+  const int i0 = min(tid, n16 - 1), i1 = min(tid + FCP_BLOCK_THREADS, n16 - 1);
+  const FCP_GLOBAL U4 *g = as_global(reinterpret_cast<const U4 *>(rec));
+  U4 r0 = g[i0], r1 = g[i1];
+  asm volatile("" ::: "memory");
+  const U2 head = *(const FCP_CONST U2 *)(rec);
+  B.first_col = head.x;
+  B.ncols = (int)head.y;
+  {
+    const FCP_GLOBAL int32_t *cr = as_global(L.csr_reg) + (int64_t)(B.first_col + (uint32_t)min(lane, B.ncols - 1)) * L.csr_reg_stride +
+                                   min(B.row_blk + wave, B.rows - 1);
+    pre0 = cr[0];
+    pre1 = cr[1];
+  }
+  constexpr int HEAD16 = FCP_RAGGED_COLS_OFF / 16, COL16 = sizeof(LdsCol) / 16, IDS16 = sizeof(FcpColStatic) / 16;
+  const uint64_t blob = (uint64_t)reinterpret_cast<uintptr_t>(L.blob);
+  auto put = [&](int i, U4 r) __attribute__((always_inline)) {
+    const int k = i - HEAD16;
+    const bool ids_piece = k >= 0 && k % COL16 == IDS16;
+    const uint64_t a = (((uint64_t)r.y << 32) | r.x) + (ids_piece ? blob : 0ull);
+    r.x = (uint32_t)a;
+    r.y = (uint32_t)(a >> 32);
+    char *at = k >= 0 ? reinterpret_cast<char *>(S.col) + 16 * k : reinterpret_cast<char *>(S.bound) + 16 * i;
+    *reinterpret_cast<U4 *>(at) = r;
+  };
+  put(i0, r0);
+  put(i1, r1);
+  __syncthreads();
+  col_of_lane = B.first_col + reinterpret_cast<const FcpRaggedSpan *>(S.bound)->lane_col[lane];
+  return true;
+}
+
+__device__ __forceinline__ Hot ragged_hot(const FcpLaunch &L) { return load_hot(L); }
+__device__ __forceinline__ Hot ragged_hot(const FcpRaggedPlainLaunch &L) {
+  Hot h = {};
+  h.blob = L.blob;
+  h.arena = L.arena;
+  h.bad_ids = L.bad_ids;
+  h.zeros = L.zeros;
+  h.n_groups = 1;
+  h.world = 1;
+  h.store_through = L.store_policy;
+  h.g0.csr_reg_stride = 1;
+  return h;
+}
+
+__device__ __forceinline__ const FcpXform *ragged_xform(const FcpLaunch &L, uint32_t first, int p) { return L.xforms + first + p; }
+__device__ __forceinline__ const FcpXform *ragged_xform(const FcpRaggedPlainLaunch &, uint32_t, int) { return nullptr; }
+
+template <int V, bool SHARDED, FcpVariant X = FCP_VAR_F32, typename LT = FcpLaunch>
+__device__ __forceinline__ void ragged_body(const LT &L, int bid, char *smem, const int64_t *wts = nullptr, int kind = 0) {
   constexpr bool WEIGHTED = X == FCP_VAR_WEIGHTED, NARROW = X == FCP_VAR_NARROW, TAB16 = X == FCP_VAR_TAB16, TABQ8 = X == FCP_VAR_TABQ8,
                  TABMIX = X == FCP_VAR_TABMIX;
+  constexpr bool IMG = std::is_same<LT, FcpRaggedPlainLaunch>::value;
+  static_assert(!IMG || (X == FCP_VAR_F32 && !SHARDED && V == 4), "the image front serves plain pooled plans only");
   const int out_kind = kind, tab_kind = kind;
   constexpr int RB = RaggedLds::RB, CAPW = RaggedLds::CAPW;
   RaggedLds &S = *reinterpret_cast<RaggedLds *>(smem);
@@ -942,25 +1023,35 @@
 
   BlockPos B;
   __builtin_amdgcn_s_setprio(3);
-  const Hot H = load_hot(L);
-  if (!locate_block<RB>(L, H, bid, B)) return;
+  int img_pre0 = 0, img_pre1 = 0;
+  uint32_t img_col = 0;
+  const Hot H = ragged_hot(L);
+  if constexpr (IMG) {
+    if (!ragged_front_image<RB>(L, bid, S, B, img_pre0, img_pre1, img_col)) return;
+  } else {
+    if (!locate_block<RB>(L, H, bid, B)) return;
+  }
   const int tid = threadIdx.x;
   const int lane = tid & (FCP_WAVE - 1);
   const int wave = tid >> 6;
   const int q = B.q0 + lane;
-  const uint32_t my_col = B.map[min(q, B.nslots - 1)];
+  const uint32_t my_col = IMG ? img_col : B.map[min(q, B.nslots - 1)];
   const int world = H.world, rank = H.rank;
 
   int pre0 = 0, pre1 = 0;
   const int csr_reg_stride = H.g0.csr_reg_stride;
-  if (csr_reg_stride && lane < B.ncols && B.row_blk + wave < B.rows) {
-    const FCP_GLOBAL int32_t *cr = as_global(L.csr_reg) + (int64_t)(B.first_col + lane) * csr_reg_stride + (B.row_blk + wave);
-    pre0 = cr[0];
-    pre1 = cr[1];
-  }
-  if (tid < B.ncols) stage_col(H, &s_col[tid], H.cols + B.first_col + tid, H.dyn + B.first_col + tid);
-  __syncthreads();
-
+  if constexpr (IMG) {
+    pre0 = img_pre0;
+    pre1 = img_pre1;
+  } else {
+    if (csr_reg_stride && lane < B.ncols && B.row_blk + wave < B.rows) {
+      const FCP_GLOBAL int32_t *cr = as_global(L.csr_reg) + (int64_t)(B.first_col + lane) * csr_reg_stride + (B.row_blk + wave);
+      pre0 = cr[0];
+      pre1 = cr[1];
+    }
+    if (tid < B.ncols) stage_col(H, &s_col[tid], H.cols + B.first_col + tid, H.dyn + B.first_col + tid);
+    __syncthreads();
+  }
   if (H.seg_search) {
     for (int u = tid; u < B.ncols * (RB + 1); u += FCP_BLOCK_THREADS) {
       const LdsCol &c = s_col[u / (RB + 1)];
@@ -1038,7 +1129,7 @@
     const int px = __shfl(offx, p), pl = __shfl(lo, p);
     if (k < limit) {
       bool bad;
-      wi[k] = fetch_slot_offset<V, SHARDED>(s_col[p], L.xforms + B.first_col + p, pl + (k - px), nullptr, rank, world, bad);
+      wi[k] = fetch_slot_offset<V, SHARDED>(s_col[p], ragged_xform(L, B.first_col, p), pl + (k - px), nullptr, rank, world, bad);
       if (bad && H.bad_ids && s_col[p].out_off >= B.q0 * V && FCP_F_FORM(s_col[p].flags) != FCP_FORM_GATHER_SCATTER)
         atomicAdd(H.bad_ids, 1ull);
     }
@@ -1169,7 +1260,7 @@
       const int ptk = __shfl(tk, p), pf = __shfl(from, p);
       if (k < limit && i < ptk) {
         bool bad;
-        wi[k] = fetch_slot_offset<V, SHARDED>(s_col[p], L.xforms + B.first_col + p, pf + i, nullptr, rank, world, bad);
+        wi[k] = fetch_slot_offset<V, SHARDED>(s_col[p], ragged_xform(L, B.first_col, p), pf + i, nullptr, rank, world, bad);
         if (bad && H.bad_ids && s_col[p].out_off >= B.q0 * V && FCP_F_FORM(s_col[p].flags) != FCP_FORM_GATHER_SCATTER)
           atomicAdd(H.bad_ids, 1ull);
       }
diff --git a/recom_amd/csrc/fcp_host.h b/recom_amd/csrc/fcp_host.h
--- a/recom_amd/csrc/fcp_host.h
+++ b/recom_amd/csrc/fcp_host.h
@@ -63,6 +63,7 @@
   int64_t seg_pairs = 0;
   bool seg_search = false;
   bool plain = false;
+  bool ragged_plain = false;
   int64_t work_bytes = 0;
   int32_t csr_reg_mode = 0, csr_reg_stride = 0;
   int64_t csr_reg_base = 0;
@@ -203,6 +204,9 @@
   std::vector<char> plain_tmpl;
   std::vector<std::pair<uint32_t, int32_t>> plain_entries;
   std::atomic<int32_t> last_dense_front{0};
+  bool ragged_plain = false;
+  RaggedImage ragged_img;
+  std::atomic<int32_t> last_ragged_front{0};
   bool wide_rows = false;
   int out_kind = FCP_OUT_F32, out_elem = 4;
   int tab_kind = FCP_TAB_F32, tab_elem = 4;
@@ -281,15 +285,18 @@
 int compute_dyn(const fcp_plan *p, const int32_t *offsets, const int32_t *shapes, const int32_t *symbols, int64_t blob_bytes,
                 FcpColDyn *dyn, DynMeta *m);
 int compute_weights(const fcp_plan *p, const int32_t *offsets, const int32_t *shapes, int64_t *wts);
+inline size_t slot_image_bytes(const fcp_plan *p) {
+  return p->plain_dense ? p->plain_tmpl.size() : p->ragged_plain ? p->ragged_img.tmpl.size() : 0;
+}
 inline size_t slot_dyn_bytes(const fcp_plan *p) {
-  return p->cols.size() * sizeof(FcpColDyn) + (p->has_weights ? p->cols.size() * sizeof(int64_t) : 0) +
-         (p->plain_dense ? p->plain_tmpl.size() : 0);
+  return p->cols.size() * sizeof(FcpColDyn) + (p->has_weights ? p->cols.size() * sizeof(int64_t) : 0) + slot_image_bytes(p);
 }
 inline size_t slot_image_off(const fcp_plan *p) { return p->cols.size() * sizeof(FcpColDyn); }
 inline const int64_t *slot_weights(const fcp_plan *p, const FcpColDyn *dyn) {
   return p->has_weights ? reinterpret_cast<const int64_t *>(dyn + p->cols.size()) : nullptr;
 }
 void build_plain_template(fcp_plan *p);
+void build_ragged_template(fcp_plan *p);
 bool stream_is_capturing(hipStream_t stream);
 int bind_tables(fcp_plan *p, const void *const *input_ptrs, bool capturing);
 void build_key(const fcp_plan *p, const fcp_process_args_t *a, std::vector<int32_t> &key);
diff --git a/recom_amd/csrc/fcp_internal.h b/recom_amd/csrc/fcp_internal.h
--- a/recom_amd/csrc/fcp_internal.h
+++ b/recom_amd/csrc/fcp_internal.h
@@ -123,6 +123,34 @@
   int32_t store_policy;
 };
 
+struct FcpRaggedCol {
+  FcpColStatic s;
+  int64_t ids_off;
+  int64_t csr;
+  int64_t out_base;
+  int32_t out_stride;
+  int32_t nnz;
+};
+struct FcpRaggedSpan {
+  uint32_t first_col;
+  int32_t ncols;
+  int32_t pad_[2];
+  uint8_t lane_col[FCP_WAVE];
+};
+constexpr int FCP_RAGGED_COLS_OFF = 80;
+struct FcpRaggedPlainLaunch {
+  const char *img;
+  const char *blob;
+  char *arena;
+  const int32_t *csr_reg;
+  int32_t rows, nslots, nsp8;
+  int32_t img_stride;
+  int32_t csr_reg_stride;
+  int32_t store_policy;
+  unsigned long long *bad_ids;
+  const float *zeros;
+};
+
 struct FcpSegLaunch {
   const int32_t *seg_cols;
   const FcpColStatic *cols;
@@ -178,6 +206,7 @@
 typedef int FcpFusedLauncher(const FcpFusedWork &W, ihipStream_t *s);
 FcpFusedLauncher fcp_launch_f32, fcp_launch_weighted, fcp_launch_narrow, fcp_launch_tab16, fcp_launch_tabq8, fcp_launch_tabmix;
 int fcp_launch_dense_plain(const FcpPlainLaunch &P, int grid_blocks, ihipStream_t *s);
+int fcp_launch_ragged_plain(const FcpRaggedPlainLaunch &P, int grid_blocks, ihipStream_t *s);
 void fcp_take_launch_extras(void **stop_event, int *flags);
 int fcp_launch_upload(const void *host_mapped_src, void *dst, size_t bytes, ihipStream_t *s);
 int fcp_launch_h2d_copy(const void *host_mapped_src, void *dst, size_t bytes, ihipStream_t *s);
diff --git a/recom_amd/csrc/fcp_plan.hip b/recom_amd/csrc/fcp_plan.hip
--- a/recom_amd/csrc/fcp_plan.hip
+++ b/recom_amd/csrc/fcp_plan.hip
@@ -459,6 +459,27 @@
   p->plain_dense = true;
 }
 
+void build_ragged_template(fcp_plan *p) {
+  p->ragged_plain = false;
+  p->ragged_img = RaggedImage();
+  if (fcp::diag_ll("ragged_generic", 0) != 0) return;
+  if (p->cols.empty() || p->desc.n_groups != 1) return;
+  RaggedPlainFacts f;
+  f.out_elem = p->out_elem;
+  f.tab_elem = p->tab_mixed() ? 0 : p->tab_elem;
+  f.layout = p->desc.layout;
+  f.n_groups = p->desc.n_groups;
+  f.shard_world = p->desc.shard_world;
+  f.vec = p->vec;
+  f.wide_rows = p->wide_rows;
+  f.weighted_kernel = p->weighted_kernel;
+  f.seg_map = p->has_seg_map;
+  f.any_order_scatter = p->has_inverse;
+  f.all_spans_ragged = p->list_n[1][0] == (p->group_nslots[0] + FCP_WAVE - 1) / FCP_WAVE && p->list_n[0][0] == 0;
+  if (!ragged_plain_plan(f, p->h_cols.data(), (int)p->h_cols.size())) return;
+  p->ragged_plain = build_ragged_image(p->h_cols.data(), (int)p->h_cols.size(), p->group_nslots[0], &p->ragged_img);
+}
+
 void destroy_device(fcp_plan *p) {
   if (p->host_only) return;
   for (auto &s : p->slots) {
@@ -582,6 +603,7 @@
     }
   }
   build_plain_template(p);
+  build_ragged_template(p);
   HIP_TRY(hipMalloc(&p->d_cols, nc * sizeof(FcpColStatic)));
   HIP_TRY(hipMemcpy(p->d_cols, p->h_cols.data(), nc * sizeof(FcpColStatic), hipMemcpyHostToDevice));
   if (!h_xforms.empty()) {
@@ -1025,6 +1047,12 @@
   return FCP_OK;
 }
 
+int fcp_plan_last_ragged_front(const fcp_plan_t *p, int32_t *front) {
+  if (!p || !front) return fail(FCP_ERR_INVALID_ARGUMENT, "null argument");
+  *front = p->last_ragged_front.load(std::memory_order_relaxed);
+  return FCP_OK;
+}
+
 int fcp_plan_last_csr(const fcp_plan_t *p, int64_t *csr_arena_off, int32_t *csr_base, int32_t capacity) {
   if (!p || capacity < 0 || (capacity > 0 && !csr_base)) return fail(FCP_ERR_INVALID_ARGUMENT, "null plan / bad capacity");
   const fcp_plan::LastLaunch &ll = p->last_launch;
diff --git a/recom_amd/csrc/fcp_plan_desc.cc b/recom_amd/csrc/fcp_plan_desc.cc
--- a/recom_amd/csrc/fcp_plan_desc.cc
+++ b/recom_amd/csrc/fcp_plan_desc.cc
@@ -439,6 +439,89 @@
   return FCP_OK;
 }
 
+bool ragged_plain_column(const FcpColStatic &s) {
+  const unsigned form = FCP_F_FORM(s.flags), comb = FCP_F_COMBINER(s.flags), ids = FCP_F_IDSRC(s.flags), seg = FCP_F_SEGKIND(s.flags);
+  if (form == FCP_FORM_SEGMENT_REDUCE) {
+    if (comb != FCP_COMBINER_SUM && comb != FCP_COMBINER_MEAN) return false;
+    if (seg != FCP_SEG_IDS_I32 && seg != FCP_SEG_IDS_I64 && seg != FCP_SEG_CSR_I32) return false;
+  } else if (form != FCP_FORM_GATHER) {
+    return false;
+  }
+  if (ids != FCP_IDS_I32 && ids != FCP_IDS_I64) return false;
+  if (s.xform != 0 || FCP_F_TABKIND(s.flags) != FCP_TAB_F32) return false;
+  return s.vocab >= 0 && s.vocab < 0xFFFFFFFDLL && s.dim > 0 && s.dim % 4 == 0 && s.out_off >= 0 && s.out_off % 4 == 0;
+}
+
+bool ragged_plain_plan(const RaggedPlainFacts &f, const FcpColStatic *cols, int nc) {
+  if (f.out_elem != 4 || f.tab_elem != 4 || f.layout != FCP_LAYOUT_CONCAT || f.n_groups != 1 || f.shard_world > 1 || f.vec != 4) return false;
+  if (f.wide_rows || f.weighted_kernel || f.seg_map || f.any_order_scatter || !f.all_spans_ragged || nc <= 0) return false;
+  for (int pos = 0; pos < nc; ++pos)
+    if (!ragged_plain_column(cols[pos])) return false;
+  return true;
+}
+
+bool build_ragged_image(const FcpColStatic *cols, int nc, int nslots, RaggedImage *out) {
+  *out = RaggedImage();
+  if (nc <= 0 || nslots <= 0) return false;
+  const int nspans = (nslots + FCP_WAVE - 1) / FCP_WAVE;
+  std::vector<int> first(nspans, nc), last(nspans, -1);
+  int next_off = 0;
+  for (int pos = 0; pos < nc; ++pos) {
+    const FcpColStatic &s = cols[pos];
+    if (s.out_off != next_off || s.dim <= 0 || s.dim % 4) return false;
+    next_off += s.dim;
+    if (next_off > nslots * 4) return false;
+    for (int sp = s.out_off / 4 / FCP_WAVE; sp <= (s.out_off + s.dim - 1) / 4 / FCP_WAVE; ++sp) {
+      first[sp] = std::min(first[sp], pos);
+      last[sp] = std::max(last[sp], pos);
+    }
+  }
+  if (next_off != nslots * 4) return false;
+  int max_cols = 1;
+  for (int sp = 0; sp < nspans; ++sp) max_cols = std::max(max_cols, last[sp] - first[sp] + 1);
+  out->stride = (int32_t)(FCP_RAGGED_COLS_OFF + (size_t)max_cols * sizeof(FcpRaggedCol));
+  out->spans = nspans;
+  out->tmpl.assign((size_t)nspans * out->stride, 0);
+  for (int sp = 0; sp < nspans; ++sp) {
+    char *rec = out->tmpl.data() + (size_t)sp * out->stride;
+    FcpRaggedSpan head;
+    std::memset(&head, 0, sizeof(head));
+    head.first_col = (uint32_t)first[sp];
+    head.ncols = last[sp] - first[sp] + 1;
+    for (int pos = first[sp]; pos <= last[sp]; ++pos) {
+      const FcpColStatic &s = cols[pos];
+      FcpRaggedCol c;
+      std::memset(&c, 0, sizeof(c));
+      c.s = s;
+      c.s.table = nullptr;
+      const size_t at = (size_t)sp * out->stride + FCP_RAGGED_COLS_OFF + (size_t)(pos - first[sp]) * sizeof(FcpRaggedCol);
+      std::memcpy(out->tmpl.data() + at, &c, sizeof(c));
+      out->entries.emplace_back((uint32_t)at, pos);
+      for (int q = std::max(s.out_off / 4, sp * FCP_WAVE); q < std::min((s.out_off + s.dim) / 4, (sp + 1) * FCP_WAVE); ++q)
+        head.lane_col[q - sp * FCP_WAVE] = (uint8_t)(pos - first[sp]);
+    }
+    for (int q = nslots; q < (sp + 1) * FCP_WAVE; ++q) head.lane_col[q - sp * FCP_WAVE] = (uint8_t)(last[sp] - first[sp]);
+    std::memcpy(rec, &head, sizeof(head));
+  }
+  return true;
+}
+
+void fill_ragged_image(const RaggedImage &I, const FcpColStatic *cols, const FcpColDyn *dyn, char *img) {
+  std::memcpy(img, I.tmpl.data(), I.tmpl.size());
+  for (const auto &e : I.entries) {
+    FcpRaggedCol c;
+    std::memcpy(&c, img + e.first, sizeof(c));
+    const FcpColDyn &d = dyn[e.second];
+    c.s.table = cols[e.second].table;
+    c.ids_off = d.ids_off;
+    c.csr = 0;
+    c.out_base = d.out_base;
+    c.out_stride = d.out_stride;
+    c.nnz = d.nnz;
+    std::memcpy(img + e.first, &c, sizeof(c));
+  }
+}
+
 }
 
 using namespace fcph;
diff --git a/recom_amd/csrc/fcp_plan_desc.h b/recom_amd/csrc/fcp_plan_desc.h
--- a/recom_amd/csrc/fcp_plan_desc.h
+++ b/recom_amd/csrc/fcp_plan_desc.h
@@ -21,4 +21,22 @@
 
 int check_desc(const fcp_plan_desc_t *d, const fcp_column_ext_t *ext, PlanFacts *facts);
 
+struct RaggedPlainFacts {
+  int out_elem = 4, tab_elem = 4;
+  int layout = FCP_LAYOUT_CONCAT, n_groups = 1, shard_world = 1, vec = 4;
+  bool wide_rows = false;
+  bool weighted_kernel = false;
+  bool seg_map = false, any_order_scatter = false;
+  bool all_spans_ragged = false;
+};
+bool ragged_plain_column(const FcpColStatic &s);
+bool ragged_plain_plan(const RaggedPlainFacts &f, const FcpColStatic *cols, int nc);
+struct RaggedImage {
+  int32_t stride = 0, spans = 0;
+  std::vector<char> tmpl;
+  std::vector<std::pair<uint32_t, int32_t>> entries;
+};
+bool build_ragged_image(const FcpColStatic *cols, int nc, int nslots, RaggedImage *out);
+void fill_ragged_image(const RaggedImage &I, const FcpColStatic *cols, const FcpColDyn *dyn, char *img);
+
 }
diff --git a/recom_amd/csrc/fcp_process.hip b/recom_amd/csrc/fcp_process.hip
--- a/recom_amd/csrc/fcp_process.hip
+++ b/recom_amd/csrc/fcp_process.hip
@@ -57,6 +57,15 @@
                         hipMemcpyHostToDevice));
     }
   }
+  if (p->ragged_plain) {
+    for (auto &s : p->slots) {
+      if (!s.img_built) continue;
+      const size_t off = slot_image_off(p);
+      fill_ragged_image(p->ragged_img, p->h_cols.data(), s.h_dyn, reinterpret_cast<char *>(s.h_dyn) + off);
+      HIP_TRY(hipMemcpy(reinterpret_cast<char *>(s.d_dyn) + off, reinterpret_cast<const char *>(s.h_dyn) + off, p->ragged_img.tmpl.size(),
+                        hipMemcpyHostToDevice));
+    }
+  }
   for (int t = 0; t < nt; ++t) p->bound_tables[t] = input_ptrs[t];
   p->tables_bound = true;
   return FCP_OK;
@@ -157,7 +166,15 @@
     s.img_built = s.meta.plain;
     if (!s.meta.plain) image_lock.unlock();
   }
-  const size_t dyn_bytes = s.meta.plain ? slot_dyn_bytes(p) : (slot_dyn_bytes(p) - (p->plain_dense ? p->plain_tmpl.size() : 0));
+  const FcpGroupLaunch &rg = s.meta.geo[1].groups[0];
+  s.meta.ragged_plain = p->ragged_plain && s.meta.geo[0].grid_blocks == 0 && s.meta.geo[1].grid_blocks > 0 && rg.span_list_off < 0 &&
+                        rg.nlist == p->ragged_img.spans && rg.rows > 0 && s.meta.csr_reg_mode != 0 && s.meta.csr_reg_stride > 0;
+  if (s.meta.ragged_plain) {
+    image_lock.lock();
+    fill_ragged_image(p->ragged_img, p->h_cols.data(), s.h_dyn, reinterpret_cast<char *>(s.h_dyn) + slot_image_off(p));
+    s.img_built = true;
+  }
+  const size_t dyn_bytes = (s.meta.plain || s.meta.ragged_plain) ? slot_dyn_bytes(p) : slot_dyn_bytes(p) - slot_image_bytes(p);
   if (p->host_writes_dyn) {
     std::memcpy(s.d_dyn, s.h_dyn, dyn_bytes);
     __builtin_ia32_sfence();
@@ -306,6 +323,7 @@
   FcpLaunch L;
   const int store_policy = store_policy_for(p, arena, m.csr_arena_off);
   fill_launch(p, *slot, 1, a->concated_inputs, arena, store_policy, &L);
+  const bool ragged_plain = m.ragged_plain && L.groups[0].csr_reg_stride > 0;
   {
     fcp_plan::LastLaunch &ll = p->last_launch;
     const int32_t fused = (int32_t)(m.geo[0].grid_blocks > 0) | (int32_t)(m.geo[1].grid_blocks > 0) << 1;
@@ -315,6 +333,10 @@
                               : m.plain                                       ? FCP_DENSE_FRONT_PLAIN
                                                                               : FCP_DENSE_FRONT_GENERIC,
                               std::memory_order_relaxed);
+    p->last_ragged_front.store(m.geo[1].grid_blocks <= 0 ? FCP_RAGGED_FRONT_NONE
+                               : ragged_plain            ? FCP_RAGGED_FRONT_PLAIN
+                                                         : FCP_RAGGED_FRONT_GENERIC,
+                               std::memory_order_relaxed);
     ll.rows_per_wave.store(m.geo[0].rows_per_wave, std::memory_order_relaxed);
     ll.store_policy.store(store_policy, std::memory_order_relaxed);
     ll.dense_blocks.store(m.geo[0].grid_blocks, std::memory_order_relaxed);
@@ -374,6 +396,23 @@
     P.store_policy = store_policy;
     const int e = fcp_launch_dense_plain(P, dense_blocks, stream);
     if (e) return hip_fail("plain dense kernel launch", (hipError_t)e);
+  } else if (ragged_blocks > 0 && ragged_plain) {
+    const FcpGroupLaunch &G = L.groups[0];
+    FcpRaggedPlainLaunch P;
+    P.img = reinterpret_cast<const char *>(slot->d_dyn) + slot_image_off(p);
+    P.blob = L.blob;
+    P.arena = L.arena;
+    P.bad_ids = L.bad_ids;
+    P.csr_reg = L.csr_reg;
+    P.rows = G.rows;
+    P.nslots = G.nslots;
+    P.nsp8 = G.nsp8;
+    P.img_stride = p->ragged_img.stride;
+    P.csr_reg_stride = G.csr_reg_stride;
+    P.store_policy = store_policy;
+    P.zeros = L.zeros;
+    const int e = fcp_launch_ragged_plain(P, ragged_blocks, stream);
+    if (e) return hip_fail("plain ragged kernel launch", (hipError_t)e);
   } else {
     FcpLaunch Ld;
     FcpLaunch *dense = ragged_blocks > 0 ? &Ld : &L;
diff --git a/recom_amd/csrc/fcp_ragged_plain.hip b/recom_amd/csrc/fcp_ragged_plain.hip
--- /dev/null
+++ b/recom_amd/csrc/fcp_ragged_plain.hip
@@ -0,0 +1,32 @@
+#include "fcp_fused_bodies.h"
+
+namespace {
+
+__global__ void __launch_bounds__(FCP_BLOCK_THREADS) __attribute__((amdgpu_waves_per_eu(8, 8)))
+fcp_ragged_kernel_plain(const char *img, const char *blob, char *arena, const int32_t *csr_reg, int rows, int nslots, int nsp8,
+                        int img_stride, int csr_reg_stride, int policy, unsigned long long *bad_ids, const float *zeros) {
+  __shared__ __attribute__((aligned(16))) char smem[sizeof(RaggedLds)];
+  const FcpRaggedPlainLaunch L = {img, blob, arena, csr_reg, rows, nslots, nsp8, img_stride, csr_reg_stride, policy, bad_ids, zeros};
+  ragged_body<4, false, FCP_VAR_F32>(L, blockIdx.x, smem);
+}
+
+}
+
+int fcp_launch_ragged_plain(const FcpRaggedPlainLaunch &P, int grid_blocks, ihipStream_t *s) {
+  if (grid_blocks <= 0) return 0;
+  if (P.img_stride < FCP_RAGGED_COLS_OFF + (int)sizeof(FcpRaggedCol) || (P.img_stride & 15) ||
+      P.img_stride > FCP_RAGGED_COLS_OFF + FCP_WAVE * (int)sizeof(FcpRaggedCol) || !P.csr_reg || P.csr_reg_stride <= 0 || P.rows <= 0 ||
+      P.nslots <= 0)
+    return (int)hipErrorInvalidValue;
+  void *stop = nullptr;
+  int flags = 0;
+  fcp_take_launch_extras(&stop, &flags);
+  const dim3 grid(grid_blocks), block(FCP_BLOCK_THREADS);
+  if (stop || flags)
+    hipExtLaunchKernelGGL(fcp_ragged_kernel_plain, grid, block, 0, s, nullptr, static_cast<hipEvent_t>(stop), flags, P.img, P.blob, P.arena,
+                          P.csr_reg, P.rows, P.nslots, P.nsp8, P.img_stride, P.csr_reg_stride, P.store_policy, P.bad_ids, P.zeros);
+  else
+    hipLaunchKernelGGL(fcp_ragged_kernel_plain, grid, block, 0, s, P.img, P.blob, P.arena, P.csr_reg, P.rows, P.nslots, P.nsp8, P.img_stride,
+                       P.csr_reg_stride, P.store_policy, P.bad_ids, P.zeros);
+  return (int)hipGetLastError();
+}
diff --git a/recom_amd/lib.py b/recom_amd/lib.py
--- a/recom_amd/lib.py
+++ b/recom_amd/lib.py
@@ -34,6 +34,7 @@
                   11: "dense_tabq8", 12: "ragged_tabq8", 13: "hybrid_tabq8",
                   14: "dense_tabmix", 15: "ragged_tabmix", 16: "hybrid_tabmix"}
 DENSE_FRONTS = {0: "none", 1: "generic", 2: "plain"}
+RAGGED_FRONTS = {0: "none", 1: "generic", 2: "plain"}
 LAUNCH_STORES = {0: "nt", 1: "sc1_nt", 4: "plain"}
 LAUNCH_SEGMENT_OFFSETS = {0: "none", 1: "prepass", 2: "search"}
 AUX_KERNELS = ("segment_offsets", "shard_finalize_v4", "shard_finalize_v2", "shard_finalize_v1",
@@ -176,7 +177,7 @@
     "fcp_plan_set_private_streams", "fcp_result_wait", "fcp_result_synchronize", "fcp_plan_set_request_order",
     "fcp_plan_probe_private_streams", "fcp_plan_private_streams_verdict", "fcp_plan_verify_private_streams",
     "fcp_plan_private_streams_stats", "fcp_plan_last_launch", "fcp_plan_last_csr", "fcp_aux_launch_counts",
-    "fcp_plan_out_dtype", "fcp_plan_last_dense_front", "fcp_plan_table_dtype",
+    "fcp_plan_out_dtype", "fcp_plan_last_dense_front", "fcp_plan_last_ragged_front", "fcp_plan_table_dtype",
     "fcp_table_row_bytes", "fcp_table_convert", "fcp_table_update_rows", "fcp_table_read_rows",
     "fcp_plan_table_kinds",
     "fcp_table_audit_workspace_bytes", "fcp_table_audit", "fcp_table_formats_choose",
@@ -326,6 +327,8 @@
         L.fcp_aux_launch_counts.argtypes = [C.c_void_p, C.c_int32, C.c_int32]
     if hasattr(L, "fcp_plan_last_dense_front"):
         L.fcp_plan_last_dense_front.argtypes = [C.c_void_p, C.POINTER(C.c_int32)]
+    if hasattr(L, "fcp_plan_last_ragged_front"):
+        L.fcp_plan_last_ragged_front.argtypes = [C.c_void_p, C.POINTER(C.c_int32)]
     if hasattr(L, "fcp_table_convert"):
         L.fcp_table_row_bytes.restype = C.c_int64
         L.fcp_table_row_bytes.argtypes = [C.c_int32, C.c_int32]
diff --git a/recom_amd/ops.py b/recom_amd/ops.py
--- a/recom_amd/ops.py
+++ b/recom_amd/ops.py
@@ -333,6 +333,11 @@
         _lib.check(self._L.fcp_plan_last_dense_front(self.handle, C.byref(v)), "fcp_plan_last_dense_front")
         return _lib.DENSE_FRONTS[v.value]
 
+    def last_ragged_front(self) -> str:
+        v = C.c_int32()
+        _lib.check(self._L.fcp_plan_last_ragged_front(self.handle, C.byref(v)), "fcp_plan_last_ragged_front")
+        return _lib.RAGGED_FRONTS[v.value]
+
     def last_csr(self):
         off = C.c_int64()
         n = self.spec.n_columns
```
